# PKU-EPIC/HOTrack

Hardware: AMD Instinct MI355X
Metric: HandTrackNet point-cloud frames/sec (N=1024) (higher is better)
Workload: dtype f32; 1 GPU; HandTrackNet forward, batch=64 synthetic 1024-pt clouds per GPU (BASELINE configs[1]); per_gpu_batch=64, global_batch=64, npoints=1024, parallelism=dp1 (independent batches, no collective), world_size=1, resident_batches_rotated=5, dead_attention_elided=True, fused_sa_kernels=True, launch=hipGraph replay, batches_in_flight=4, hip_hw_queues=4, sa_compute_units=256, weights=deterministic random init (no checkpoint available offline)

## Files before the change

hotrack_amd/csrc/ball_query.hip:

```cpp
#include "pn2_common.h"
#include "fps_tie.h"

namespace pn2 {

constexpr int kBqThreads = 256;
constexpr int kBqWaves = kBqThreads / kWave;
constexpr int kBqTile = 4096;

template <int CPW, bool JOINT>
__device__ __forceinline__ void ball_query_body(const int bx, const int by, int n, int m, float radius2, int nsample,
                                                const float *__restrict__ new_xyz_all, const float *__restrict__ xyz_all,
                                                int *__restrict__ idx_all, const int *__restrict__ picks_all,
                                                float *__restrict__ new_xyz_out_all, float *__restrict__ new_xyz_copy, int copy_ld) {
    extern __shared__ __attribute__((aligned(16))) float smem[];
    const int tile_cap = n < kBqTile ? n : kBqTile;
    float *sx = smem, *sy = smem + tile_cap, *sz = smem + 2 * tile_cap;

    const int b = by;
    const float *__restrict__ xyz = xyz_all + (size_t)b * n * 3;
    const float *__restrict__ new_xyz = picks_all ? nullptr : new_xyz_all + (size_t)b * m * 3;
    const int *__restrict__ picks = picks_all ? picks_all + (size_t)b * m : nullptr;
    int *__restrict__ idx = idx_all + (size_t)b * m * nsample;

    const int tid = threadIdx.x;
    const int lane = tid & 63;
    const int w = tid >> 6;
    const int c_base = bx * (kBqWaves * CPW);

    float cx[CPW], cy[CPW], cz[CPW];
    int cnt[CPW], first[CPW];
#pragma unroll
    for (int c = 0; c < CPW; ++c) {
        const int s = c_base + c * kBqWaves + w;
        const bool ok = s < m;
        const float *__restrict__ src = !ok ? nullptr : (picks ? xyz + 3 * (size_t)picks[s] : new_xyz + 3 * (size_t)s);
        cx[c] = ok ? src[0] : 0.f;
        cy[c] = ok ? src[1] : 0.f;
        cz[c] = ok ? src[2] : 0.f;
        if (ok && picks && lane == 0) {
            float *o = new_xyz_out_all + ((size_t)b * m + s) * 3;
            o[0] = cx[c]; o[1] = cy[c]; o[2] = cz[c];
            if (new_xyz_copy) {
                float *o2 = new_xyz_copy + ((size_t)b * m + s) * copy_ld;
                o2[0] = cx[c]; o2[1] = cy[c]; o2[2] = cz[c];
            }
        }
        cnt[c] = ok ? 0 : nsample;
        first[c] = 0;
    }

    for (int t0 = 0; t0 < n; t0 += kBqTile) {
        const int tn = (n - t0) < kBqTile ? (n - t0) : kBqTile;
        if (t0 > 0) __syncthreads();
        for (int i = tid; i < 3 * tn; i += kBqThreads) {
            const float v = xyz[(size_t)3 * t0 + i];
            const int p = i / 3, comp = i - 3 * p;
            (comp == 0 ? sx : comp == 1 ? sy : sz)[p] = v;
        }
        __syncthreads();
        if constexpr (JOINT) {
            int open = 0;
#pragma unroll
            for (int c = 0; c < CPW; ++c) open += cnt[c] < nsample ? 1 : 0;
            for (int base = 0; base < tn && open > 0; base += kWave) {
                const int p = base + lane;
                const bool in = p < tn;
                const float x = in ? sx[p] : 0.f, y = in ? sy[p] : 0.f, z = in ? sz[p] : 0.f;
                float d2[CPW];
                if constexpr (CPW >= 2) {
#pragma unroll
                    for (int c = 0; c < CPW; c += 2) {
                        const pn2_f32x2 d = sqdist2((pn2_f32x2){cx[c], cx[c + 1]}, (pn2_f32x2){cy[c], cy[c + 1]}, (pn2_f32x2){cz[c], cz[c + 1]}, x, y, z);
                        d2[c] = d.x;
                        d2[c + 1] = d.y;
                    }
                } else {
                    d2[0] = sqdist(cx[0], cy[0], cz[0], x, y, z);
                }
#pragma unroll
                for (int c = 0; c < CPW; ++c) {
                    if (cnt[c] >= nsample) continue;
                    const bool hit = in && (d2[c] < radius2);
                    const uint64_t mask = __ballot(hit);
                    if (mask) {
                        int *__restrict__ row = idx + (size_t)(c_base + c * kBqWaves + w) * nsample;
                        if (cnt[c] == 0) first[c] = t0 + base + __builtin_ctzll(mask);
                        const int pos = cnt[c] + prefix_popc(mask);
                        if (hit && pos < nsample) row[pos] = t0 + p;
                        cnt[c] += __builtin_popcountll(mask);
                        if (cnt[c] >= nsample) --open;
                    }
                }
            }
        } else {
#pragma unroll
            for (int c = 0; c < CPW; ++c) {
                const int s = c_base + c * kBqWaves + w;
                int *__restrict__ row = idx + (size_t)s * nsample;
                int mycnt = cnt[c];
                if (mycnt >= nsample) continue;
                for (int base = 0; base < tn; base += kWave) {
                    const int p = base + lane;
                    const bool in = p < tn;
                    const float x = in ? sx[p] : 0.f, y = in ? sy[p] : 0.f, z = in ? sz[p] : 0.f;
                    const float d2 = sqdist(cx[c], cy[c], cz[c], x, y, z);
                    const bool hit = in && (d2 < radius2);
                    const uint64_t mask = __ballot(hit);
                    if (mask) {
                        if (mycnt == 0) first[c] = t0 + base + __builtin_ctzll(mask);
                        const int pos = mycnt + prefix_popc(mask);
                        if (hit && pos < nsample) row[pos] = t0 + p;
                        mycnt += __builtin_popcountll(mask);
                        if (mycnt >= nsample) break;
                    }
                }
                cnt[c] = mycnt;
            }
        }
    }
#pragma unroll
    for (int c = 0; c < CPW; ++c) {
        const int s = c_base + c * kBqWaves + w;
        if (s >= m) continue;
        int *__restrict__ row = idx + (size_t)s * nsample;
        const int fill = cnt[c] > 0 ? first[c] : 0;
        for (int p = cnt[c] + lane; p < nsample; p += kWave) row[p] = fill;
    }
}

template <int CPW, bool JOINT>
__global__ void __launch_bounds__(kBqThreads)
ball_query_kernel(int n, int m, float radius2, int nsample, const float *__restrict__ new_xyz_all,
                  const float *__restrict__ xyz_all, int *__restrict__ idx_all, const int *__restrict__ picks_all,
                  float *__restrict__ new_xyz_out_all, float *__restrict__ new_xyz_copy, int copy_ld) {
    ball_query_body<CPW, JOINT>((int)blockIdx.x, (int)blockIdx.y, n, m, radius2, nsample, new_xyz_all, xyz_all, idx_all, picks_all,
                                new_xyz_out_all, new_xyz_copy, copy_ld);
}

template <int CPW>
__global__ void __launch_bounds__(kBqThreads)
ball_tie_kernel(int nbx_ball, int nb_ball, int nbx_tie, int n, int m, float radius2, int nsample, const float *__restrict__ xyz_all,
                int *__restrict__ idx_all, const int *__restrict__ picks_all, float *__restrict__ new_xyz_out_all,
                float *__restrict__ new_xyz_copy, int copy_ld, int m2, const float *__restrict__ radii_all, int *__restrict__ flags) {
    const int L = (int)blockIdx.x;
    if (L < nb_ball) {
        const int by = L / nbx_ball;
        ball_query_body<CPW, false>(L - by * nbx_ball, by, n, m, radius2, nsample, xyz_all, xyz_all, idx_all, picks_all, new_xyz_out_all,
                                    new_xyz_copy, copy_ld);
    } else {
        const int T = L - nb_ball, by = T / nbx_tie;
        fps_tie_body(T - by * nbx_tie, by, nbx_tie, n, m2, m, xyz_all, picks_all, radii_all, flags);
    }
}

int ball_query_dispatch(int b, int n, int m, float radius, int nsample, const float *new_xyz,
                        const float *xyz, int *idx, hipStream_t st, const int *picks, float *new_xyz_out, float *new_xyz_copy,
                        int copy_ld) {
    if (b == 0 || m == 0) return PN2_OK;
    const float radius2 = radius * radius;
    const int tile_cap = n < kBqTile ? n : kBqTile;
    const size_t lds = (size_t)3 * tile_cap * sizeof(float);
    const long total = (long)b * m;
    int cpw = 1;
    if (total >= 4L * kBqWaves * 4096) cpw = 4;
    else if (total >= 2L * kBqWaves * 2048) cpw = 2;
    const int per_block = kBqWaves * cpw;
    dim3 grid((m + per_block - 1) / per_block, b);
    const bool joint = cpw >= 2 && n >= 4096;
    if (cpw == 4 && joint)
        hipLaunchKernelGGL((ball_query_kernel<4, true>), grid, dim3(kBqThreads), lds, st, n, m, radius2, nsample, new_xyz, xyz, idx, picks, new_xyz_out, new_xyz_copy, copy_ld);
    else if (cpw == 4)
        hipLaunchKernelGGL((ball_query_kernel<4, false>), grid, dim3(kBqThreads), lds, st, n, m, radius2, nsample, new_xyz, xyz, idx, picks, new_xyz_out, new_xyz_copy, copy_ld);
    else if (cpw == 2 && joint)
        hipLaunchKernelGGL((ball_query_kernel<2, true>), grid, dim3(kBqThreads), lds, st, n, m, radius2, nsample, new_xyz, xyz, idx, picks, new_xyz_out, new_xyz_copy, copy_ld);
    else if (cpw == 2)
        hipLaunchKernelGGL((ball_query_kernel<2, false>), grid, dim3(kBqThreads), lds, st, n, m, radius2, nsample, new_xyz, xyz, idx, picks, new_xyz_out, new_xyz_copy, copy_ld);
    else
        hipLaunchKernelGGL((ball_query_kernel<1, false>), grid, dim3(kBqThreads), lds, st, n, m, radius2, nsample, new_xyz, xyz, idx, picks, new_xyz_out, new_xyz_copy, copy_ld);
    return check_launch();
}

constexpr long kBallTieMaxN = (64 * 1024 - 22 * 1024) / 12 / 64 * 64;
bool ball_tie_supported(long b, long n, long m, long m2) {
    return b >= 1 && m >= 1 && n <= kBallTieMaxN && b * n <= 16384 && b * m < 2L * kBqWaves * 2048 && m2 >= 1 && m2 <= m &&
           m2 <= kTieMaxM;
}

int ball_tie_dispatch(int b, int n, int m, float radius, int nsample, const float *xyz, int *idx, const int *picks, float *new_xyz_out,
                      float *new_xyz_copy, int copy_ld, int m2, const float *radii, int *flags, hipStream_t st) {
    if (!ball_tie_supported(b, n, m, m2)) return PN2_ERANGE;
    const float radius2 = radius * radius;
    const int tile_cap = n < kBqTile ? n : kBqTile;
    const size_t lds = (size_t)3 * tile_cap * sizeof(float);
    const int per_block = kBqWaves;
    const int nbx_ball = (m + per_block - 1) / per_block, nbx_tie = (n + kTiePts - 1) / kTiePts;
    const long grid = (long)b * nbx_ball + (long)b * nbx_tie;
    hipLaunchKernelGGL(ball_tie_kernel<1>, dim3((unsigned)grid), dim3(kBqThreads), lds, st, nbx_ball, b * nbx_ball, nbx_tie, n, m, radius2, nsample,
                       xyz, idx, picks, new_xyz_out, new_xyz_copy, copy_ld, m2, radii, flags);
    return check_launch();
}

}
```

hotrack_amd/csrc/capi.hip:

```cpp
#include <stdlib.h>

#include "pn2_common.h"
#include "../../include/pn2_ext.h"

namespace pn2 {
static thread_local int g_last_hip_error = 0;
void set_last_hip_error(int e) { g_last_hip_error = e; }

int fps_dispatch(int b, int n, int m, const float *xyz, float *temp, int *idx, hipStream_t st, int force_threads,
                 const int *skip_flags, int nflags, float *radii);
int fps_tie_check(int b, int n, int m, int m1, const float *xyz, const int *idx, const float *radii, int *flags, hipStream_t st);
bool fps_knn_supported(int n, int nq, int k);
bool ball_tie_supported(long b, long n, long m, long m2);
int ball_tie_dispatch(int b, int n, int m, float radius, int nsample, const float *xyz, int *idx, const int *picks, float *new_xyz_out,
                      float *new_xyz_copy, int copy_ld, int m2, const float *radii, int *flags, hipStream_t st);
bool three_nn_interp_supported(long b, long n, long m, long c, long ldp, long ldo);
int three_nn_interp_dispatch(int b, int n, int m, int c, const float *unknown, const float *known, const float *points, int ldp,
                             float *out, int ldo, hipStream_t st);
int fps_knn_dispatch(int b, int n, int m, const float *xyz, int *idx, float *radii, int nq, int k, int k2, const float *query,
                     int *kidx, int *kidx2, hipStream_t st);
int ball_query_dispatch(int b, int n, int m, float radius, int nsample, const float *new_xyz, const float *xyz,
                        int *idx, hipStream_t st, const int *picks, float *new_xyz_out, float *new_xyz_copy, int copy_ld);
int three_nn_dispatch(int b, int n, int m, const float *unknown, const float *known, float *dist2, int *idx,
                      hipStream_t st, bool weights);
int interp_pm_dispatch(int b, int c, int m, int n, const float *points, int ldp, const int *idx, const float *weight,
                       float *out, int ldo, hipStream_t st);
int knn_dispatch(int b, int n, int m, int k, const float *unknown, const float *known, float *dist2, int *idx,
                 hipStream_t st, int k2, int *idx2);
int group_fwd_dispatch(int b, int c, int n, int npoints, int nsample, const float *points, const int *idx,
                       float *out, hipStream_t st);
int group_bwd_dispatch(int b, int c, int n, int npoints, int nsample, const float *grad_out, const int *idx,
                       float *grad_points, hipStream_t st);
int interp_fwd_dispatch(int b, int c, int m, int n, const float *points, const int *idx, const float *weight,
                        float *out, hipStream_t st);
int interp_bwd_dispatch(int b, int c, int n, int m, const float *grad_out, const int *idx, const float *weight,
                        float *grad_points, hipStream_t st);
}

using namespace pn2;

#define PN2_REQ(cond, code) \
    do {                    \
        if (!(cond)) return (code); \
    } while (0)

static inline bool fits_int(long v) { return v >= 0 && v <= 2147483647L; }

extern "C" {

int pn2_abi_version(void) { return 2; }

int pn2_last_hip_error(void) { return g_last_hip_error; }

const char *pn2_strerror(int code) {
    switch (code) {
        case PN2_OK: return "ok";
        case PN2_EINVAL: return "invalid dimension or parameter";
        case PN2_ENULL: return "required pointer is NULL";
        case PN2_ERANGE: return "size outside the supported range";
        case PN2_ESCRATCH: return "this size needs the scratch buffer (temp) to be provided";
        case PN2_ELAUNCH: return "HIP kernel launch failed";
        default: return "unknown error";
    }
}

int pn2_furthest_point_sampling(int b, int n, int m, const float *xyz, float *temp, int *idx, void *stream) {
    PN2_REQ(b >= 0 && n >= 1 && m >= 0, PN2_EINVAL);
    if (b == 0 || m == 0) return PN2_OK;
    PN2_REQ(xyz && idx, PN2_ENULL);
    PN2_REQ(b <= 65535 * 32768L, PN2_ERANGE);
    PN2_REQ(fits_int((long)n * 3), PN2_ERANGE);
    int force = 0;
    if (const char *e = getenv("PN2_FPS_THREADS")) force = atoi(e);
    return fps_dispatch(b, n, m, xyz, temp, idx, (hipStream_t)stream, force, nullptr, 0, nullptr);
}

int pn2x_furthest_point_sampling_radii(int b, int n, int m, const float *xyz, int *idx, float *radii, void *stream) {
    PN2_REQ(b >= 0 && n >= 1 && m >= 0, PN2_EINVAL);
    if (b == 0 || m == 0) return PN2_OK;
    PN2_REQ(xyz && idx && radii, PN2_ENULL);
    PN2_REQ(fits_int((long)n * 3), PN2_ERANGE);
    return fps_dispatch(b, n, m, xyz, nullptr, idx, (hipStream_t)stream, 0, nullptr, 0, radii);
}

int pn2x_fps_radii_knn_supported(int n, int nq, int k) { return fps_knn_supported(n, nq, k) ? 1 : 0; }

int pn2x_fps_radii_knn(int b, int n, int m, const float *xyz, int *idx, float *radii, int nq, int k, int k2, const float *query,
                       int *knn_idx, int *knn_idx2, void *stream) {
    PN2_REQ(b >= 0 && n >= 1 && m >= 1 && nq >= 1 && k >= 1 && k2 >= 0 && k2 <= k, PN2_EINVAL);
    if (b == 0) return PN2_OK;
    PN2_REQ(xyz && idx && radii && query && knn_idx && (k2 == 0 || knn_idx2), PN2_ENULL);
    PN2_REQ(m <= n && fits_int((long)n * 3) && fits_int((long)b * nq * k), PN2_ERANGE);
    return fps_knn_dispatch(b, n, m, xyz, idx, radii, nq, k, k2, query, knn_idx, k2 ? knn_idx2 : nullptr, (hipStream_t)stream);
}

int pn2x_fps_prefix_ties(int b, int n, int m1, int m2, const float *xyz, const int *idx1, const float *radii, int *flags, void *stream) {
    PN2_REQ(b >= 0 && n >= 1 && m1 >= 1 && m2 >= 1 && m2 <= m1, PN2_EINVAL);
    if (b == 0) return PN2_OK;
    PN2_REQ(xyz && idx1 && radii && flags, PN2_ENULL);
    PN2_REQ(fits_int((long)n * 3) && b <= 65535, PN2_ERANGE);
    return fps_tie_check(b, n, m2, m1, xyz, idx1, radii, flags, (hipStream_t)stream);
}

int pn2x_fps_prefix_flags(int n) { return n < 1 ? PN2_EINVAL : (n + 63) / 64; }

int pn2x_furthest_point_sampling_prefix(int b, int n, int m, const float *xyz, const int *flags, int nflags, int *idx, void *stream) {
    PN2_REQ(b >= 0 && n >= 1 && m >= 0 && m <= n && nflags >= 1, PN2_EINVAL);
    if (b == 0 || m == 0) return PN2_OK;
    PN2_REQ(xyz && idx && flags, PN2_ENULL);
    PN2_REQ(fits_int((long)n * 3), PN2_ERANGE);
    return fps_dispatch(b, n, m, xyz, nullptr, idx, (hipStream_t)stream, 0, flags, nflags, nullptr);
}

int pn2_ball_query(int b, int n, int m, float radius, int nsample, const float *new_xyz, const float *xyz,
                   int *idx, void *stream) {
    PN2_REQ(b >= 0 && n >= 1 && m >= 0 && nsample >= 1, PN2_EINVAL);
    PN2_REQ(radius == radius, PN2_EINVAL);
    if (b == 0 || m == 0) return PN2_OK;
    PN2_REQ(new_xyz && xyz && idx, PN2_ENULL);
    PN2_REQ(b <= 65535, PN2_ERANGE);
    PN2_REQ(fits_int((long)n * 3) && fits_int((long)m * nsample), PN2_ERANGE);
    if (n >= 4096 && (long)m * n >= (1L << 22) && radius > 0.f) {
        const long words = pn2x_ball_query_grid_scratch_words(b, n);
        if (words > 0 && words < (1L << 30)) {
            StreamScratch own;
            int *scratch = own.acquire((size_t)words + 4, (hipStream_t)stream);
            if (scratch) {
                unsigned *aligned = reinterpret_cast<unsigned *>(((uintptr_t)scratch + 15) & ~(uintptr_t)15);
                const int rc = ball_query_grid_dispatch(b, n, m, radius, nsample, new_xyz, xyz, idx, aligned, (size_t)words, (hipStream_t)stream);
                if (rc != PN2_ERANGE) return rc;
            }
        }
    }
    return ball_query_dispatch(b, n, m, radius, nsample, new_xyz, xyz, idx, (hipStream_t)stream, nullptr, nullptr, nullptr, 0);
}

int pn2x_ball_query_picks(int b, int n, int m, float radius, int nsample, const float *xyz, const int *picks, float *new_xyz,
                           int *idx, float *new_xyz_copy, int copy_ld, void *stream) {
    PN2_REQ(!new_xyz_copy || copy_ld >= 3, PN2_EINVAL);
    PN2_REQ(b >= 0 && n >= 1 && m >= 0 && nsample >= 1, PN2_EINVAL);
    PN2_REQ(radius == radius, PN2_EINVAL);
    if (b == 0 || m == 0) return PN2_OK;
    PN2_REQ(xyz && picks && new_xyz && idx, PN2_ENULL);
    PN2_REQ(b <= 65535, PN2_ERANGE);
    PN2_REQ(fits_int((long)n * 3) && fits_int((long)m * nsample), PN2_ERANGE);
    return ball_query_dispatch(b, n, m, radius, nsample, nullptr, xyz, idx, (hipStream_t)stream, picks, new_xyz, new_xyz_copy, copy_ld);
}

int pn2x_ball_query_picks_ties_supported(int b, int n, int m, int m2) { return ball_tie_supported(b, n, m, m2) ? 1 : 0; }

int pn2x_ball_query_picks_ties(int b, int n, int m, float radius, int nsample, const float *xyz, const int *picks, float *new_xyz,
                               int *idx, float *new_xyz_copy, int copy_ld, int m2, const float *radii, int *flags, void *stream) {
    PN2_REQ(!new_xyz_copy || copy_ld >= 3, PN2_EINVAL);
    PN2_REQ(b >= 0 && n >= 1 && m >= 1 && nsample >= 1 && m2 >= 1 && m2 <= m, PN2_EINVAL);
    PN2_REQ(radius == radius, PN2_EINVAL);
    if (b == 0) return PN2_OK;
    PN2_REQ(xyz && picks && new_xyz && idx && radii && flags, PN2_ENULL);
    PN2_REQ(b <= 65535 && fits_int((long)n * 3) && fits_int((long)m * nsample), PN2_ERANGE);
    return ball_tie_dispatch(b, n, m, radius, nsample, xyz, idx, picks, new_xyz, new_xyz_copy, copy_ld, m2, radii, flags, (hipStream_t)stream);
}

int pn2_group_points(int b, int c, int n, int npoints, int nsample, const float *points, const int *idx,
                     float *out, void *stream) {
    PN2_REQ(b >= 0 && c >= 0 && n >= 1 && npoints >= 0 && nsample >= 0, PN2_EINVAL);
    if (b == 0 || c == 0 || npoints == 0 || nsample == 0) return PN2_OK;
    PN2_REQ(points && idx && out, PN2_ENULL);
    PN2_REQ(b <= 65535 && fits_int((long)npoints * nsample), PN2_ERANGE);
    return group_fwd_dispatch(b, c, n, npoints, nsample, points, idx, out, (hipStream_t)stream);
}

int pn2_group_points_grad(int b, int c, int n, int npoints, int nsample, const float *grad_out, const int *idx,
                          float *grad_points, void *stream) {
    PN2_REQ(b >= 0 && c >= 0 && n >= 1 && npoints >= 0 && nsample >= 0, PN2_EINVAL);
    if (b == 0 || c == 0 || npoints == 0 || nsample == 0) return PN2_OK;
    PN2_REQ(grad_out && idx && grad_points, PN2_ENULL);
    PN2_REQ(b <= 65535 && c <= 65535 * 16 && fits_int((long)npoints * nsample), PN2_ERANGE);
    return group_bwd_dispatch(b, c, n, npoints, nsample, grad_out, idx, grad_points, (hipStream_t)stream);
}

int pn2_gather_points(int b, int c, int n, int npoints, const float *points, const int *idx, float *out,
                      void *stream) {
    return pn2_group_points(b, c, n, npoints, 1, points, idx, out, stream);
}

int pn2_gather_points_grad(int b, int c, int n, int npoints, const float *grad_out, const int *idx,
                           float *grad_points, void *stream) {
    return pn2_group_points_grad(b, c, n, npoints, 1, grad_out, idx, grad_points, stream);
}

int pn2_knn(int b, int n, int m, int k, const float *unknown, const float *known, float *dist2, int *idx,
            void *stream) {
    PN2_REQ(b >= 0 && n >= 0 && m >= 0, PN2_EINVAL);
    PN2_REQ(k >= 1, PN2_EINVAL);
    PN2_REQ(k <= PN2_KNN_MAX_K, PN2_ERANGE);
    if (b == 0 || n == 0) return PN2_OK;
    PN2_REQ(unknown && dist2 && idx && (known || m == 0), PN2_ENULL);
    PN2_REQ(b <= 65535 && fits_int((long)n * k) && fits_int((long)m * 3), PN2_ERANGE);
    return knn_dispatch(b, n, m, k, unknown, known, dist2, idx, (hipStream_t)stream, 0, nullptr);
}

int pn2x_knn_indices(int b, int n, int m, int k, int k2, const float *unknown, const float *known, int *idx, int *idx2, void *stream) {
    PN2_REQ(b >= 0 && n >= 0 && m >= 1 && k >= 1 && k2 >= 0 && k2 <= k, PN2_EINVAL);
    PN2_REQ(k <= PN2_KNN_MAX_K, PN2_ERANGE);
    if (b == 0 || n == 0) return PN2_OK;
    PN2_REQ(unknown && known && idx && (idx2 || k2 == 0), PN2_ENULL);
    PN2_REQ(b <= 65535 && fits_int((long)n * k) && fits_int((long)m * 3), PN2_ERANGE);
    return knn_dispatch(b, n, m, k, unknown, known, nullptr, idx, (hipStream_t)stream, k2, k2 > 0 ? idx2 : nullptr);
}

int pn2_three_nn(int b, int n, int m, const float *unknown, const float *known, float *dist2, int *idx,
                 void *stream) {
    PN2_REQ(b >= 0 && n >= 0 && m >= 0, PN2_EINVAL);
    if (b == 0 || n == 0) return PN2_OK;
    PN2_REQ(unknown && dist2 && idx && (known || m == 0), PN2_ENULL);
    PN2_REQ(b <= 65535 && fits_int((long)n * 3) && fits_int((long)m * 3), PN2_ERANGE);
    return three_nn_dispatch(b, n, m, unknown, known, dist2, idx, (hipStream_t)stream, false);
}

int pn2_three_interpolate(int b, int c, int m, int n, const float *points, const int *idx, const float *weight,
                          float *out, void *stream) {
    PN2_REQ(b >= 0 && c >= 0 && m >= 1 && n >= 0, PN2_EINVAL);
    if (b == 0 || c == 0 || n == 0) return PN2_OK;
    PN2_REQ(points && idx && weight && out, PN2_ENULL);
    PN2_REQ(b <= 65535 && fits_int((long)n * 3), PN2_ERANGE);
    return interp_fwd_dispatch(b, c, m, n, points, idx, weight, out, (hipStream_t)stream);
}

int pn2_three_interpolate_grad(int b, int c, int n, int m, const float *grad_out, const int *idx,
                               const float *weight, float *grad_points, void *stream) {
    PN2_REQ(b >= 0 && c >= 0 && m >= 1 && n >= 0, PN2_EINVAL);
    if (b == 0 || c == 0 || n == 0) return PN2_OK;
    PN2_REQ(grad_out && idx && weight && grad_points, PN2_ENULL);
    PN2_REQ(b <= 65535 && c <= 65535 * 16 && fits_int((long)n * 3), PN2_ERANGE);
    return interp_bwd_dispatch(b, c, n, m, grad_out, idx, weight, grad_points, (hipStream_t)stream);
}

int pn2x_three_nn_weights(int b, int n, int m, const float *unknown, const float *known, float *weight, int *idx,
                          void *stream) {
    PN2_REQ(b >= 0 && n >= 0 && m >= 3, PN2_EINVAL);
    if (b == 0 || n == 0) return PN2_OK;
    PN2_REQ(unknown && known && weight && idx, PN2_ENULL);
    PN2_REQ(b <= 65535 && fits_int((long)n * 3) && fits_int((long)m * 3), PN2_ERANGE);
    return three_nn_dispatch(b, n, m, unknown, known, weight, idx, (hipStream_t)stream, true);
}

int pn2x_three_nn_interpolate_pm_supported(int b, int n, int m, int c, int ldp, int ldo) {
    return three_nn_interp_supported(b, n, m, c, ldp, ldo) ? 1 : 0;
}

int pn2x_three_nn_interpolate_pm(int b, int n, int m, int c, const float *unknown, const float *known, const float *points, int ldp,
                                 float *out, int ldo, void *stream) {
    PN2_REQ(b >= 0 && n >= 0 && m >= 3 && c >= 1 && ldp >= c && ldo >= c, PN2_EINVAL);
    if (b == 0 || n == 0) return PN2_OK;
    PN2_REQ(unknown && known && points && out, PN2_ENULL);
    PN2_REQ(b <= 65535 && fits_int((long)n * 3) && fits_int((long)m * 3), PN2_ERANGE);
    return three_nn_interp_dispatch(b, n, m, c, unknown, known, points, ldp, out, ldo, (hipStream_t)stream);
}

int pn2x_three_interpolate_pm(int b, int c, int m, int n, const float *points, int ldp, const int *idx,
                              const float *weight, float *out, int ldo, void *stream) {
    PN2_REQ(b >= 0 && c >= 0 && m >= 1 && n >= 0 && ldp >= c && ldo >= c, PN2_EINVAL);
    if (b == 0 || c == 0 || n == 0) return PN2_OK;
    PN2_REQ(points && idx && weight && out, PN2_ENULL);
    PN2_REQ(fits_int((long)n * 3), PN2_ERANGE);
    return interp_pm_dispatch(b, c, m, n, points, ldp, idx, weight, out, ldo, (hipStream_t)stream);
}

}
```

hotrack_amd/csrc/sa_fused.hip:

```cpp
#include <stdlib.h>

#include "pn2_common.h"
#include "../../include/pn2_ext.h"

#ifndef SA_PAD
#define SA_PAD 4
#endif

#ifndef SA_DEFER_EPILOGUE
#define SA_DEFER_EPILOGUE 0
#endif
#ifndef SA_OVERLAP_WRITEOUT
#define SA_OVERLAP_WRITEOUT 1
#endif
#ifndef SA_SCALAR_L1
#define SA_SCALAR_L1 0
#endif
#ifndef SA_LOADER_PRIO
#define SA_LOADER_PRIO 0
#endif
#ifndef SA_PROBE
#define SA_PROBE 0
#endif
#ifndef SA_PREFETCH
#define SA_PREFETCH 1
#endif
#if SA_PREFETCH
#define SA_SCHED_FENCE() __builtin_amdgcn_sched_barrier(0)
#else
#define SA_SCHED_FENCE() ((void)0)
#endif

namespace pn2 {

typedef float f32x4 __attribute__((ext_vector_type(4)));
typedef float f32x3 __attribute__((ext_vector_type(3)));
__device__ __forceinline__ f32x3 load_xyz(const float *p) {
    f32x3 v;
    __builtin_memcpy(&v, p, 12);
    return v;
}

typedef __amdgpu_buffer_rsrc_t rsrc_t;
__device__ __forceinline__ rsrc_t make_rsrc(const void *base, unsigned bytes) {
    return __builtin_amdgcn_make_buffer_rsrc(const_cast<void *>(base), 0, (int)bytes, 0x00020000);
}
__device__ __forceinline__ unsigned mad24(int a, unsigned b_uniform, unsigned c) {
    unsigned r;
    asm("v_mad_u32_u24 %0, %1, %2, %3" : "=v"(r) : "v"(a), "s"(b_uniform), "v"(c));
    return r;
}
__device__ __forceinline__ unsigned mul24(int a, unsigned b_uniform) {
    unsigned r;
    asm("v_mul_u32_u24 %0, %1, %2" : "=v"(r) : "s"(b_uniform), "v"(a));
    return r;
}
typedef int i32x4 __attribute__((ext_vector_type(4)));
typedef int i32x2 __attribute__((ext_vector_type(2)));
__device__ __forceinline__ float4 ld_b128(rsrc_t r, unsigned voff, int soff) {
    const f32x4 v = __builtin_bit_cast(f32x4, __builtin_amdgcn_raw_buffer_load_b128(r, (int)voff, soff, 0));
    return make_float4(v.x, v.y, v.z, v.w);
}
typedef float f32x2 __attribute__((ext_vector_type(2)));
__device__ __forceinline__ f32x2 pk_fma_lo(f32x2 w, f32x2 d, f32x2 acc) {
    f32x2 r;
    asm("v_pk_fma_f32 %0, %1, %2, %3 op_sel_hi:[1,0,1]" : "=v"(r) : "v"(w), "v"(d), "v"(acc));
    return r;
}
__device__ __forceinline__ f32x2 pk_fma_hi(f32x2 w, f32x2 d, f32x2 acc) {
    f32x2 r;
    asm("v_pk_fma_f32 %0, %1, %2, %3 op_sel:[0,1,0]" : "=v"(r) : "v"(w), "v"(d), "v"(acc));
    return r;
}

struct SaArgs {
    int B, N, S, K, lgK;
    const float *a1f;
    const float *xyz;
    const float *cxyz;
    const float *wx;
    const float *b1;
    const float *cadd;
    int a1f_ld, cadd_ld;
    const int *idx;
    const float *w2, *b2, *w3, *b3;
    const float *w2e;
    float *out;
    long out_b;
    int out_s, out_c;
    int num_tiles, tiles_per_cloud;
    long long *trace;
};

template <int C1, int C2, int C3, int WC, int RTC, int MINW, int NB1, int K, int MODE>
__device__ __forceinline__ void sa_body(const SaArgs &A, const int wg, const int nwg) {
    static_assert(K == 16 || K == 32 || K == 64, "K");
    constexpr bool ROWS = MODE == 4 || MODE == 5, ROWS_EXTRA = MODE == 5;
    static_assert(!ROWS_EXTRA || SA_PAD >= 4, "the extra input columns live in the LDS row padding");
    constexpr bool has_a1f = MODE >= 1, has_xyz = !ROWS, has_cadd = MODE == 2 || MODE == 3;
    const bool p_a1f = MODE == 3 ? A.a1f != nullptr : has_a1f, p_xyz = MODE == 3 ? A.xyz != nullptr : has_xyz;
    const bool p_cadd = MODE == 3 ? A.cadd != nullptr : has_cadd;
    constexpr int lgK = K == 16 ? 4 : K == 32 ? 5 : 6;
    const int N = A.N, S = A.S;
    const float *__restrict__ W2 = A.w2, *__restrict__ b2 = A.b2, *__restrict__ W3 = A.w3, *__restrict__ b3 = A.b3;
    float *__restrict__ out = A.out;
    const int num_tiles = A.num_tiles, tiles_per_cloud = A.tiles_per_cloud;
    constexpr int WP = 4 / WC;
    constexpr int TM = WP * 64;
    constexpr int LD1 = C1 + SA_PAD, LD2 = C2 + SA_PAD;
    constexpr int NT2 = C2 / (16 * WC), NT3 = C3 / (16 * WC);
    static_assert(C2 % (16 * WC) == 0 && C3 % (16 * WC) == 0 && C1 % 16 == 0, "tile geometry");
    extern __shared__ __attribute__((aligned(16))) float smem[];
    float *H1ring = smem;
    float *H2 = smem + NB1 * TM * LD1;

    const int tid = (int)__builtin_amdgcn_workitem_id_x();
    const int lane = tid & 63;
    const int w = tid >> 6;
    const bool compute = w < 4;
    const int wc = (w & 3) % WC, wp = (w & 3) / WC;
    const int li = lane & 15, g = lane >> 4;
    const int SK = S * K;

    constexpr int Q1 = C1 / 4;
    static_assert(256 % Q1 == 0, "a loader thread keeps its channel quad across rows");
    const int lt = tid & 255;
    const int c4 = lt % Q1;
    float wxr[4][3] = {{0.f}};
    float4 b1r = make_float4(0.f, 0.f, 0.f, 0.f);
    if (!compute) {
        if (p_xyz) {
#pragma unroll
            for (int i = 0; i < 4; ++i)
#pragma unroll
                for (int k = 0; k < 3; ++k) wxr[i][k] = A.wx[(4 * c4 + i) * 3 + k];
        }
        if (A.b1) b1r = *reinterpret_cast<const float4 *>(A.b1 + 4 * c4);
    }

    constexpr int RPT = (TM / 2) / (256 / Q1);
    static_assert((TM / 2) % (256 / Q1) == 0, "half tile rows split evenly over the loader threads");
    static_assert(RPT == 1 || RPT == 2 || RPT == 4, "a thread's neighbour indices are ONE 4/8/16-byte load");
    const int row0 = (lt / Q1) * RPT;
    const int cur_db = nwg / tiles_per_cloud, cur_dt = nwg - cur_db * tiles_per_cloud;
    struct Cursor { int tile, b, t; };
    auto cursor_at = [&](int tile) { Cursor c; c.tile = tile; c.b = tile / tiles_per_cloud; c.t = tile - c.b * tiles_per_cloud; return c; };
    auto cursor_next = [&](Cursor c) {
        c.tile += nwg; c.b += cur_db; c.t += cur_dt;
        if (c.t >= tiles_per_cloud) { c.t -= tiles_per_cloud; ++c.b; }
        return c;
    };
    const unsigned c4x16 = 16u * c4, row0x4 = 4u * row0;
    const unsigned a1f_ldb = 4u * (unsigned)A.a1f_ld, cadd_ldb = 4u * (unsigned)A.cadd_ld;
    const unsigned idx_cloud = 4u * (unsigned)SK, a1f_cloud = (unsigned)N * a1f_ldb, xyz_cloud = 12u * (unsigned)N;
    const unsigned cxyz_cloud = 12u * (unsigned)S, cadd_cloud = (unsigned)S * cadd_ldb;
    const rsrc_t ra_all = make_rsrc(A.a1f, p_a1f ? (unsigned)A.B * a1f_cloud : 0u);
    const rsrc_t rx_all = make_rsrc(A.xyz, p_xyz ? (unsigned)A.B * xyz_cloud : 0u);
    struct HalfIdx { int jj[RPT], ss; };
    struct HalfRows { float4 a[RPT], pj[RPT], c, cs, e; };
    auto load_idx = [&](const Cursor &cu, int h, HalfIdx &I) {
        const int b = cu.b < A.B ? cu.b : A.B - 1;
        const int pos0 = cu.t * TM + h * (TM / 2);
        if constexpr (ROWS) {
#pragma unroll
            for (int r = 0; r < RPT; ++r) I.jj[r] = pos0 + row0 + r;
            I.ss = 0;
            return;
        }
        const rsrc_t ri = make_rsrc(reinterpret_cast<const char *>(A.idx) + (size_t)b * idx_cloud, idx_cloud);
        if constexpr (RPT == 4) {
            const i32x4 v = __builtin_bit_cast(i32x4, __builtin_amdgcn_raw_buffer_load_b128(ri, (int)row0x4, 4 * pos0, 0));
            I.jj[0] = v.x; I.jj[1] = v.y; I.jj[2] = v.z; I.jj[3] = v.w;
        } else if constexpr (RPT == 2) {
            const i32x2 v = __builtin_bit_cast(i32x2, __builtin_amdgcn_raw_buffer_load_b64(ri, (int)row0x4, 4 * pos0, 0));
            I.jj[0] = v.x; I.jj[1] = v.y;
        } else {
            I.jj[0] = (int)__builtin_amdgcn_raw_buffer_load_b32(ri, (int)row0x4, 4 * pos0, 0);
        }
        I.ss = (pos0 + row0) >> lgK;
    };
    auto load_rows = [&](const Cursor &cu, const HalfIdx &I, HalfRows &D) {
        const int b = cu.b < A.B ? cu.b : A.B - 1;
        if (has_a1f) {
            const int so = ROWS ? 0 : (int)((unsigned)b * a1f_cloud);
#pragma unroll
            for (int r = 0; r < RPT; ++r) D.a[r] = ld_b128(ra_all, mad24(I.jj[r], a1f_ldb, c4x16), so);
            if (ROWS_EXTRA && lt < TM / 2) D.e = ld_b128(ra_all, mad24(I.jj[0] - row0 + lt, a1f_ldb, 4u * C1), so);
        }
        if (has_cadd) {
            const rsrc_t rd = make_rsrc(reinterpret_cast<const char *>(A.cadd) + (size_t)b * cadd_cloud, p_cadd ? cadd_cloud : 0u);
            D.c = ld_b128(rd, mad24(I.ss, cadd_ldb, c4x16), 0);
        }
        if (has_xyz) {
            const int so = (int)((unsigned)b * xyz_cloud);
            const rsrc_t rc = make_rsrc(reinterpret_cast<const char *>(A.cxyz) + (size_t)b * cxyz_cloud, p_xyz ? cxyz_cloud : 0u);
#pragma unroll
            for (int r = 0; r < RPT; ++r) D.pj[r] = ld_b128(rx_all, mul24(I.jj[r], 12u), so);
            D.cs = ld_b128(rc, mul24(I.ss, 12u), 0);
        }
    };
    auto finish = [&](const HalfRows &D, float *__restrict__ H1, int h) {
#ifdef SA_FINISH_PRIO
        __builtin_amdgcn_s_setprio(SA_FINISH_PRIO);
#endif
        if constexpr (ROWS) {
#pragma unroll
            for (int r = 0; r < RPT; ++r) *reinterpret_cast<float4 *>(H1 + (h * (TM / 2) + row0 + r) * LD1 + 4 * c4) = D.a[r];
            if (ROWS_EXTRA && lt < TM / 2) *reinterpret_cast<float4 *>(H1 + (h * (TM / 2) + lt) * LD1 + C1) = D.e;
            return;
        }
        const f32x2 w0x = {wxr[0][0], wxr[1][0]}, w0y = {wxr[0][1], wxr[1][1]}, w0z = {wxr[0][2], wxr[1][2]};
        const f32x2 w1x = {wxr[2][0], wxr[3][0]}, w1y = {wxr[2][1], wxr[3][1]}, w1z = {wxr[2][2], wxr[3][2]};
#if SA_SCALAR_L1
        float t[4] = {b1r.x, b1r.y, b1r.z, b1r.w};
        if (has_cadd) { t[0] += D.c.x; t[1] += D.c.y; t[2] += D.c.z; t[3] += D.c.w; }
#pragma unroll
        for (int r = 0; r < RPT; ++r) {
            float v[4] = {t[0], t[1], t[2], t[3]};
            if (has_a1f) { v[0] += D.a[r].x; v[1] += D.a[r].y; v[2] += D.a[r].z; v[3] += D.a[r].w; }
            if (has_xyz) {
                const float dx = D.pj[r].x - D.cs.x, dy = D.pj[r].y - D.cs.y, dz = D.pj[r].z - D.cs.z;
#pragma unroll
                for (int i = 0; i < 4; ++i)
                    v[i] = __builtin_fmaf(wxr[i][0], dx, __builtin_fmaf(wxr[i][1], dy, __builtin_fmaf(wxr[i][2], dz, v[i])));
            }
            *reinterpret_cast<float4 *>(H1 + (h * (TM / 2) + row0 + r) * LD1 + 4 * c4) =
                make_float4(fmax_raw(v[0], 0.f), fmax_raw(v[1], 0.f), fmax_raw(v[2], 0.f), fmax_raw(v[3], 0.f));
        }
#else
        f32x2 t0 = {b1r.x, b1r.y}, t1 = {b1r.z, b1r.w};
        if (has_cadd) { t0 += (f32x2){D.c.x, D.c.y}; t1 += (f32x2){D.c.z, D.c.w}; }
        const f32x2 cxy = {D.cs.x, D.cs.y}, czw = {D.cs.z, D.cs.w};
#pragma unroll
        for (int r = 0; r < RPT; ++r) {
            f32x2 v0 = t0, v1 = t1;
            if (has_a1f) { v0 += (f32x2){D.a[r].x, D.a[r].y}; v1 += (f32x2){D.a[r].z, D.a[r].w}; }
            if (has_xyz) {
                const f32x2 dxy = (f32x2){D.pj[r].x, D.pj[r].y} - cxy, dzw = (f32x2){D.pj[r].z, D.pj[r].w} - czw;
                v0 = pk_fma_lo(w0x, dxy, pk_fma_hi(w0y, dxy, pk_fma_lo(w0z, dzw, v0)));
                v1 = pk_fma_lo(w1x, dxy, pk_fma_hi(w1y, dxy, pk_fma_lo(w1z, dzw, v1)));
            }
            *reinterpret_cast<float4 *>(H1 + (h * (TM / 2) + row0 + r) * LD1 + 4 * c4) =
                make_float4(fmax_raw(v0.x, 0.f), fmax_raw(v0.y, 0.f), fmax_raw(v1.x, 0.f), fmax_raw(v1.y, 0.f));
        }
#endif
#ifdef SA_FINISH_PRIO
        __builtin_amdgcn_s_setprio(SA_LOADER_PRIO);
#endif
    };
    auto gather = [&](const Cursor &cu, float *__restrict__ H1, int h) {
        HalfIdx I;
        HalfRows D;
        load_idx(cu, h, I);
        load_rows(cu, I, D);
        finish(D, H1, h);
    };

    float w2r[NT2][C1 / 4], w3r[NT3][C2 / 4];
    f32x4 bias2v[NT2];
    float bias3[NT3];
    f32x4 bias3v[ROWS ? NT3 : 1];
    float w2e[NT2][4][3] = {{{0.f}}};
    if (compute) {
        if constexpr (ROWS_EXTRA) {
#pragma unroll
            for (int ct = 0; ct < NT2; ++ct)
#pragma unroll
                for (int r = 0; r < 4; ++r)
#pragma unroll
                    for (int k = 0; k < 3; ++k) w2e[ct][r][k] = A.w2e[((wc * NT2 + ct) * 16 + 4 * g + r) * 3 + k];
        }
#pragma unroll
        for (int ct = 0; ct < NT2; ++ct) {
            const int oc = (wc * NT2 + ct) * 16 + li;
            {
                const float *bp = b2 + (wc * NT2 + ct) * 16 + 4 * g;
                bias2v[ct] = (f32x4){bp[0], bp[1], bp[2], bp[3]};
            }
#pragma unroll
            for (int tq = 0; tq < C1 / 16; ++tq) {
                const float4 v = *reinterpret_cast<const float4 *>(W2 + (size_t)oc * C1 + 16 * tq + 4 * g);
                w2r[ct][4 * tq + 0] = v.x; w2r[ct][4 * tq + 1] = v.y; w2r[ct][4 * tq + 2] = v.z; w2r[ct][4 * tq + 3] = v.w;
            }
        }
#pragma unroll
        for (int ct = 0; ct < NT3; ++ct) {
            const int oc = (wc * NT3 + ct) * 16 + li;
            bias3[ct] = b3[oc];
            if constexpr (ROWS) {
                const float *bp = b3 + (wc * NT3 + ct) * 16 + 4 * g;
                bias3v[ct] = (f32x4){bp[0], bp[1], bp[2], bp[3]};
            }
#pragma unroll
            for (int tq = 0; tq < C2 / 16; ++tq) {
                const float4 v = *reinterpret_cast<const float4 *>(W3 + (size_t)oc * C2 + 16 * tq + 4 * g);
                w3r[ct][4 * tq + 0] = v.x; w3r[ct][4 * tq + 1] = v.y; w3r[ct][4 * tq + 2] = v.z; w3r[ct][4 * tq + 3] = v.w;
            }
        }
    } else {
        Cursor cu = cursor_at(wg);
        for (int a = 0; a < NB1 - 1; ++a, cu = cursor_next(cu)) {
            if (cu.tile < num_tiles) {
                gather(cu, H1ring + a * TM * LD1, 0);
                gather(cu, H1ring + a * TM * LD1, 1);
            }
        }
    }
    __syncthreads();

    auto stamp = [&](int it, int slot) {
#if defined(SA_TRACE) && SA_TRACE
        if (A.trace && wg == 0 && lane == 0 && (w == 0 || w == 4) && it < 8)
            A.trace[((w >> 2) * 8 + it) * 8 + slot] = (long long)__builtin_readcyclecounter();
#else
        (void)it; (void)slot;
#endif
    };
    if (!compute) {
        __builtin_amdgcn_s_setprio(SA_LOADER_PRIO);
        HalfIdx I0, I1;
        HalfRows D0, D1;
        Cursor nx = cursor_at(wg + (NB1 - 1) * nwg);
        Cursor af = cursor_next(nx);
        load_idx(nx, 0, I0);
        load_idx(nx, 1, I1);
        load_rows(nx, I0, D0);
        int it = 0;
        for (int tile = wg; tile < num_tiles; tile += nwg, ++it) {
            stamp(it, 0);
            float *H1n = H1ring + ((it + NB1 - 1) % NB1) * TM * LD1;
#if !(SA_PROBE & 1)
            load_rows(nx, I1, D1);
#endif
            stamp(it, 7);
#if !(SA_PROBE & 4)
            load_idx(af, 0, I0);
#endif
            stamp(it, 1);
#if !(SA_PROBE & 2)
            if (nx.tile < num_tiles) finish(D0, H1n, 0);
#endif
            stamp(it, 2);
            __syncthreads();
            stamp(it, 3);
#if !(SA_PROBE & 1)
            load_rows(af, I0, D0);
#endif
#if !(SA_PROBE & 4)
            load_idx(af, 1, I1);
#endif
            stamp(it, 4);
#if !(SA_PROBE & 2)
            if (nx.tile < num_tiles) finish(D1, H1n, 1);
#endif
            stamp(it, 5);
            __syncthreads();
            stamp(it, 6);
            nx = af;
            af = cursor_next(af);
        }
        return;
    }
#ifdef SA_COMPUTE_PRIO
    __builtin_amdgcn_s_setprio(SA_COMPUTE_PRIO);
#endif
    int it = 0;
    Cursor cc = cursor_at(wg);
    constexpr int NP = 4 / RTC, NQ2 = C1 / 16, NQ3 = C2 / 16;
    constexpr int rstep = K >> 4;
    const int oc_lane = (wc * NT3 + g) * 16 + li;
    const unsigned out_cloud = 4u * ((unsigned)(S - 1) * (unsigned)A.out_s + (unsigned)(C3 - 1) * (unsigned)A.out_c + 1u);
    const rsrc_t ro_rows = make_rsrc(out, ROWS ? 4u * (unsigned)N * (unsigned)A.out_s : 0u);
    float m[4][NT3];
#pragma unroll
    for (int rt = 0; rt < 4; ++rt)
#pragma unroll
        for (int ct = 0; ct < NT3; ++ct) m[rt][ct] = 0.f;
    int e_b = 0, e_pos0 = 0;
    bool e_pending = false;
    auto epilogue = [&]() {
        if constexpr (K == 32) {
#pragma unroll
            for (int ct = 0; ct < NT3; ++ct) {
                m[0][ct] = fmax_raw(m[0][ct], m[1][ct]);
                m[2][ct] = fmax_raw(m[2][ct], m[3][ct]);
            }
        }
        if constexpr (K == 64) {
#pragma unroll
            for (int ct = 0; ct < NT3; ++ct) m[0][ct] = fmax_raw(fmax3_raw(m[0][ct], m[1][ct], m[2][ct]), m[3][ct]);
        }
        const rsrc_t ro = make_rsrc(out + (size_t)e_b * A.out_b, e_pending ? out_cloud : 0u);
#pragma unroll
        for (int rt = 0; rt < 4; rt += rstep) {
            const int s = ((e_pos0 + wp * 64) >> lgK) + rt / rstep;
#pragma unroll
            for (int ct0 = 0; ct0 < NT3; ct0 += 4) {
                float v = rows_max4(m[rt][ct0]);
#pragma unroll
                for (int j = 1; j < 4; ++j)
                    if (ct0 + j < NT3) {
                        const float vj = rows_max4(m[rt][ct0 + j]);
                        v = g == j ? vj : v;
                    }
                const unsigned off = 4u * ((unsigned)s * (unsigned)A.out_s + (unsigned)(oc_lane + 16 * ct0) * (unsigned)A.out_c);
                const bool ok = ct0 + g < NT3 && s < S;
                __builtin_amdgcn_raw_buffer_store_b32(__builtin_bit_cast(unsigned, fmaxf(v, 0.f)), ro, (int)(ok ? off : 0xffffffffu), 0, 0);
            }
        }
    };
    auto frag2 = [&](const float *H1, int p, int tq, int rt) {
        return *reinterpret_cast<const float4 *>(H1 + (wp * 64 + (p * RTC + rt) * 16 + li) * LD1 + 4 * g + 16 * tq);
    };
    constexpr bool PREFETCH_NEXT = WP == 1 && RTC * 16 <= TM / 2;
    float4 an2[RTC];
#pragma unroll
    for (int rt = 0; rt < RTC; ++rt) an2[rt] = frag2(H1ring, 0, 0, rt);
    for (int tile = wg; tile < num_tiles; tile += nwg, ++it, cc = cursor_next(cc)) {
        stamp(it, 0);
        const float *H1 = H1ring + (it % NB1) * TM * LD1;
        const float *H1next = H1ring + ((it + 1) % NB1) * TM * LD1;
        {
            f32x4 acc[2][RTC][NT2];
            auto writeout2 = [&](int p) {
#pragma unroll
                for (int rt = 0; rt < RTC; ++rt) {
                    float4 e = make_float4(0.f, 0.f, 0.f, 0.f);
                    if constexpr (ROWS_EXTRA) e = *reinterpret_cast<const float4 *>(H1 + (wp * 64 + (p * RTC + rt) * 16 + li) * LD1 + C1);
#pragma unroll
                    for (int ct = 0; ct < NT2; ++ct) {
                        float *dst = H2 + (wp * 64 + (p * RTC + rt) * 16 + li) * LD2 + (wc * NT2 + ct) * 16 + 4 * g;
                        f32x4 v = acc[p & 1][rt][ct];
                        if constexpr (ROWS_EXTRA) {
#pragma unroll
                            for (int r = 0; r < 4; ++r)
                                v[r] = __builtin_fmaf(w2e[ct][r][0], e.x, __builtin_fmaf(w2e[ct][r][1], e.y, __builtin_fmaf(w2e[ct][r][2], e.z, v[r])));
                        }
                        *reinterpret_cast<float4 *>(dst) = make_float4(fmaxf(v.x, 0.f), fmaxf(v.y, 0.f), fmaxf(v.z, 0.f), fmaxf(v.w, 0.f));
                    }
                }
            };
            float4 an[RTC];
#pragma unroll
            for (int rt = 0; rt < RTC; ++rt) an[rt] = PREFETCH_NEXT ? an2[rt] : frag2(H1, 0, 0, rt);
#pragma unroll
            for (int p = 0; p < NP; ++p) {
#pragma unroll
                for (int rt = 0; rt < RTC; ++rt)
#pragma unroll
                    for (int ct = 0; ct < NT2; ++ct) acc[p & 1][rt][ct] = bias2v[ct];
#pragma unroll
                for (int tq = 0; tq < NQ2; ++tq) {
                    float4 a[RTC];
#pragma unroll
                    for (int rt = 0; rt < RTC; ++rt) a[rt] = an[rt];
                    if (tq + 1 < NQ2 || p + 1 < NP) {
#pragma unroll
                        for (int rt = 0; rt < RTC; ++rt) an[rt] = tq + 1 < NQ2 ? frag2(H1, p, tq + 1, rt) : frag2(H1, p + 1, 0, rt);
                        SA_SCHED_FENCE();
                    }
#pragma unroll
                    for (int j = 0; j < 4; ++j)
#pragma unroll
                        for (int rt = 0; rt < RTC; ++rt) {
                            const float av = j == 0 ? a[rt].x : j == 1 ? a[rt].y : j == 2 ? a[rt].z : a[rt].w;
#pragma unroll
                            for (int ct = 0; ct < NT2; ++ct)
                                acc[p & 1][rt][ct] = __builtin_amdgcn_mfma_f32_16x16x4f32(w2r[ct][4 * tq + j], av, acc[p & 1][rt][ct], 0, 0, 0);
                        }
#if SA_DEFER_EPILOGUE
                    if (!ROWS && tq == 0 && p == 0) epilogue();
#endif
#if SA_OVERLAP_WRITEOUT
                    if (tq == 0 && p > 0) writeout2(p - 1);
#endif
                }
#if !SA_OVERLAP_WRITEOUT
                writeout2(p);
#endif
            }
            stamp(it, 1);
#if SA_OVERLAP_WRITEOUT
            writeout2(NP - 1);
#endif
        }
        stamp(it, 2);
        __syncthreads();
        stamp(it, 3);
        {
            auto frag3 = [&](int p, int tq, int rt) {
                return *reinterpret_cast<const float4 *>(H2 + (wp * 64 + (p * RTC + rt) * 16 + li) * LD2 + 4 * g + 16 * tq);
            };
            float4 an[RTC];
#pragma unroll
            for (int rt = 0; rt < RTC; ++rt) an[rt] = frag3(0, 0, rt);
#pragma unroll
            for (int p = 0; p < NP; ++p) {
                f32x4 acc[RTC][NT3];
#pragma unroll
                for (int rt = 0; rt < RTC; ++rt)
#pragma unroll
                    for (int ct = 0; ct < NT3; ++ct) acc[rt][ct] = ROWS ? bias3v[ct] : (f32x4){bias3[ct], bias3[ct], bias3[ct], bias3[ct]};
#pragma unroll
                for (int tq = 0; tq < NQ3; ++tq) {
                    float4 a[RTC];
#pragma unroll
                    for (int rt = 0; rt < RTC; ++rt) a[rt] = an[rt];
                    if (tq + 1 < NQ3 || p + 1 < NP) {
#pragma unroll
                        for (int rt = 0; rt < RTC; ++rt) an[rt] = tq + 1 < NQ3 ? frag3(p, tq + 1, rt) : frag3(p + 1, 0, rt);
                    } else if (PREFETCH_NEXT) {
#pragma unroll
                        for (int rt = 0; rt < RTC; ++rt) an2[rt] = frag2(H1next, 0, 0, rt);
                    }
                    SA_SCHED_FENCE();
#pragma unroll
                    for (int j = 0; j < 4; ++j)
#pragma unroll
                        for (int rt = 0; rt < RTC; ++rt) {
                            const float av = j == 0 ? a[rt].x : j == 1 ? a[rt].y : j == 2 ? a[rt].z : a[rt].w;
#pragma unroll
                            for (int ct = 0; ct < NT3; ++ct) {
                                if constexpr (ROWS) acc[rt][ct] = __builtin_amdgcn_mfma_f32_16x16x4f32(w3r[ct][4 * tq + j], av, acc[rt][ct], 0, 0, 0);
                                else acc[rt][ct] = __builtin_amdgcn_mfma_f32_16x16x4f32(av, w3r[ct][4 * tq + j], acc[rt][ct], 0, 0, 0);
                            }
                        }
                }
                if constexpr (ROWS) {
#pragma unroll
                    for (int rt = 0; rt < RTC; ++rt)
#pragma unroll
                        for (int ct = 0; ct < NT3; ++ct) {
                            const int row = cc.t * TM + wp * 64 + (p * RTC + rt) * 16 + li;
                            const unsigned off = 4u * ((unsigned)row * (unsigned)A.out_s + (unsigned)((wc * NT3 + ct) * 16 + 4 * g));
                            f32x4 v = acc[rt][ct];
                            v.x = fmaxf(v.x, 0.f); v.y = fmaxf(v.y, 0.f); v.z = fmaxf(v.z, 0.f); v.w = fmaxf(v.w, 0.f);
                            typedef unsigned u32x4 __attribute__((ext_vector_type(4)));
                            __builtin_amdgcn_raw_buffer_store_b128(__builtin_bit_cast(u32x4, v), ro_rows, (int)off, 0, 0);
                        }
                } else {
#pragma unroll
                    for (int rt = 0; rt < RTC; ++rt)
#pragma unroll
                        for (int ct = 0; ct < NT3; ++ct)
                            m[p * RTC + rt][ct] = fmax_raw(fmax3_raw(acc[rt][ct][0], acc[rt][ct][1], acc[rt][ct][2]), acc[rt][ct][3]);
                }
            }
            stamp(it, 4);
            if constexpr (!ROWS) {
                e_b = cc.b;
                e_pos0 = cc.t * TM;
                e_pending = true;
#if !SA_DEFER_EPILOGUE
                epilogue();
#endif
            }
        }
        stamp(it, 5);
        __syncthreads();
        stamp(it, 6);
    }
#if SA_DEFER_EPILOGUE
    if (!ROWS) epilogue();
#endif
}

template <int C1, int C2, int C3, int WC, int RTC, int MINW, int NB1, int K, int MODE>
__global__ void __launch_bounds__(512, MINW)
sa_mlp_max_kernel(const SaArgs A, const int grid) {
    sa_body<C1, C2, C3, WC, RTC, MINW, NB1, K, MODE>(A, (int)__builtin_amdgcn_workgroup_id_x(), grid);
}

template <int C1, int C2, int C3, int WC, int RTC, int MINW, int NB1, int K0, int K1, int MODE>
__global__ void __launch_bounds__(512, MINW)
sa_mlp_max_pair_kernel(const SaArgs A0, const SaArgs A1, const int n0, const int n1) {
    const int wg = (int)__builtin_amdgcn_workgroup_id_x();
    if (wg < n0)
        sa_body<C1, C2, C3, WC, RTC, MINW, NB1, K0, MODE>(A0, wg, n0);
    else
        sa_body<C1, C2, C3, WC, RTC, MINW, NB1, K1, MODE>(A1, wg - n0, n1);
}

static int g_sa_cus = -1;
static int sa_compute_units() {
    if (g_sa_cus < 0) {
        const char *e = getenv("PN2_SA_CUS");
        g_sa_cus = e ? atoi(e) : 0;
    }
    const int all = num_compute_units();
    return (g_sa_cus > 0 && g_sa_cus < all) ? g_sa_cus : all;
}

template <int C1, int C2, int C3, int WC, int RTC, int MINW, int NB1, int K, int MODE>
static int launch_sa_km(int b, SaArgs a, hipStream_t st) {
    constexpr int WP = 4 / WC, TM = WP * 64;
    const int sk = a.S * a.K;
    a.tiles_per_cloud = (sk + TM - 1) / TM;
    const long num_tiles_l = (long)b * a.tiles_per_cloud;
    if (num_tiles_l > 2147483647L) return PN2_ERANGE;
    a.num_tiles = (int)num_tiles_l;
    a.B = b;
    a.lgK = 0;
    while ((1 << a.lgK) < a.K) ++a.lgK;
    const size_t lds = (size_t)TM * (NB1 * (C1 + SA_PAD) + C2 + SA_PAD) * sizeof(float);
    auto kfn = sa_mlp_max_kernel<C1, C2, C3, WC, RTC, MINW, NB1, K, MODE>;
    static PerDeviceOnce raised;
    if (lds > 64 * 1024 && raised.first_use())
        (void)hipFuncSetAttribute((const void *)kfn, hipFuncAttributeMaxDynamicSharedMemorySize, (int)lds);
    const int wg_per_cu = (int)((160 * 1024) / lds) < MINW / 2 ? (int)((160 * 1024) / lds) : MINW / 2;
    const int max_wg = sa_compute_units() * (wg_per_cu < 1 ? 1 : wg_per_cu);
    const int rounds = (a.num_tiles + max_wg - 1) / max_wg;
    const int grid = (a.num_tiles + rounds - 1) / rounds;
    hipLaunchKernelGGL(kfn, dim3(grid), dim3(512), lds, st, a, grid);
    return check_launch();
}

template <int C1, int C2, int C3, int WC, int RTC, int MINW, int NB1>
static void sa_tiles(int b, SaArgs &a) {
    constexpr int WP = 4 / WC, TM = WP * 64;
    a.tiles_per_cloud = (a.S * a.K + TM - 1) / TM;
    a.num_tiles = b * a.tiles_per_cloud;
    a.B = b;
    a.lgK = 0;
    while ((1 << a.lgK) < a.K) ++a.lgK;
}

template <int C1, int C2, int C3, int WC, int RTC, int MINW, int NB1, int K0, int K1, int MODE>
static int launch_sa_pair(int b, SaArgs a0, SaArgs a1, hipStream_t st) {
    constexpr int WP = 4 / WC, TM = WP * 64;
    if ((long)b * ((a0.S * a0.K + TM - 1) / TM) + (long)b * ((a1.S * a1.K + TM - 1) / TM) > 2147483647L) return PN2_ERANGE;
    sa_tiles<C1, C2, C3, WC, RTC, MINW, NB1>(b, a0);
    sa_tiles<C1, C2, C3, WC, RTC, MINW, NB1>(b, a1);
    const size_t lds = (size_t)TM * (NB1 * (C1 + SA_PAD) + C2 + SA_PAD) * sizeof(float);
    auto kfn = sa_mlp_max_pair_kernel<C1, C2, C3, WC, RTC, MINW, NB1, K0, K1, MODE>;
    static PerDeviceOnce raised;
    if (lds > 64 * 1024 && raised.first_use())
        (void)hipFuncSetAttribute((const void *)kfn, hipFuncAttributeMaxDynamicSharedMemorySize, (int)lds);
    const int wg_per_cu = (int)((160 * 1024) / lds) < MINW / 2 ? (int)((160 * 1024) / lds) : MINW / 2;
    const int max_wg = sa_compute_units() * (wg_per_cu < 1 ? 1 : wg_per_cu);
    const int total = a0.num_tiles + a1.num_tiles;
    int rounds = (total + max_wg - 1) / max_wg;
    int n0, n1;
    for (;; ++rounds) {
        n0 = (a0.num_tiles + rounds - 1) / rounds;
        n1 = (a1.num_tiles + rounds - 1) / rounds;
        if (n0 + n1 <= max_wg || rounds > total) break;
    }
    hipLaunchKernelGGL(kfn, dim3(n0 + n1), dim3(512), lds, st, a0, a1, n0, n1);
    return check_launch();
}

template <int C1, int C2, int C3, int WC, int RTC, int MINW, int NB1, int K>
static int launch_sa_k(int b, const SaArgs &a, hipStream_t st) {
    const bool fa = a.a1f != nullptr, fx = a.xyz != nullptr, fc = a.cadd != nullptr;
    if (!fa && fx && !fc) return launch_sa_km<C1, C2, C3, WC, RTC, MINW, NB1, K, 0>(b, a, st);
    if (fa && fx && !fc) return launch_sa_km<C1, C2, C3, WC, RTC, MINW, NB1, K, 1>(b, a, st);
    if (fa && fx && fc) return launch_sa_km<C1, C2, C3, WC, RTC, MINW, NB1, K, 2>(b, a, st);
    return launch_sa_km<C1, C2, C3, WC, RTC, MINW, NB1, K, 3>(b, a, st);
}

template <int C1, int C2, int C3, int WC, int RTC, int MINW, int NB1>
static int launch_sa(int b, const SaArgs &a, hipStream_t st) {
    switch (a.K) {
        case 16: return launch_sa_k<C1, C2, C3, WC, RTC, MINW, NB1, 16>(b, a, st);
        case 32: return launch_sa_k<C1, C2, C3, WC, RTC, MINW, NB1, 32>(b, a, st);
        case 64: return launch_sa_k<C1, C2, C3, WC, RTC, MINW, NB1, 64>(b, a, st);
    }
    return PN2_ERANGE;
}

#ifndef SA_RTC128
#define SA_RTC128 2
#endif
#ifndef SA_NB1
#define SA_NB1 2
#endif
static long long *g_sa_trace = nullptr;
static bool sa_ranges_ok(long b, long n, long s, long k, long a1f_ld, long cadd_ld, long c3, long out_s, long out_c) {
    const long lim = 0xffffffffL;
    if (out_s < 0 || out_c < 0 || 4 * ((s - 1) * out_s + (c3 - 1) * out_c + 1) >= lim) return false;
    return n < (1L << 24) && s < (1L << 24) && 4 * a1f_ld < (1L << 24) && 4 * cadd_ld < (1L << 24) &&
           4 * b * n * (a1f_ld > 3 ? a1f_ld : 3) <= lim && 4 * s * (cadd_ld > 3 ? cadd_ld : 3) <= lim && 4 * s * k <= lim;
}
}

extern "C" int pn2x_sa_set_compute_units(int n) {
    if (n < 0) return PN2_EINVAL;
    pn2::g_sa_cus = n;
    return PN2_OK;
}

extern "C" void pn2x_debug_set_sa_trace(void *device_buffer_2x8x8_int64) { pn2::g_sa_trace = (long long *)device_buffer_2x8x8_int64; }

extern "C" int pn2x_sa_mlp_max(int b, int n, int s, int k, int c1, int c2, int c3, const float *a1f, int a1f_ld,
                               const float *xyz, const float *cxyz, const float *wx, const float *b1, const float *cadd,
                               int cadd_ld, const int *idx,
                               const float *w2, const float *b2, const float *w3, const float *b3, float *out,
                               long out_b, int out_s, int out_c, void *stream) {
    using namespace pn2;
    if (b < 0 || n < 1 || s < 0 || k < 1) return PN2_EINVAL;
    if (b == 0 || s == 0) return PN2_OK;
    if (!idx || !w2 || !b2 || !w3 || !b3 || !out) return PN2_ENULL;
    if (!a1f && !xyz) return PN2_ENULL;
    if (xyz && (!cxyz || !wx)) return PN2_ENULL;
    if ((a1f && (a1f_ld < c1 || a1f_ld % 4)) || (cadd && (cadd_ld < c1 || cadd_ld % 4))) return PN2_EINVAL;
    if (!(k == 16 || k == 32 || k == 64)) return PN2_ERANGE;
    if (!sa_ranges_ok(b, n, s, k, a1f ? a1f_ld : 0, cadd ? cadd_ld : 0, c3, out_s, out_c)) return PN2_ERANGE;
    if (((uintptr_t)a1f | (uintptr_t)cadd | (uintptr_t)b1 | (uintptr_t)w2 | (uintptr_t)w3) % 16 != 0) return PN2_EINVAL;
    SaArgs a;
    a.B = b; a.N = n; a.S = s; a.K = k; a.lgK = 0;
    a.a1f = a1f; a.a1f_ld = a1f_ld; a.cadd_ld = cadd_ld; a.xyz = xyz; a.cxyz = cxyz; a.wx = wx; a.b1 = b1; a.cadd = cadd; a.idx = idx;
    a.w2 = w2; a.b2 = b2; a.w3 = w3; a.b3 = b3; a.w2e = nullptr; a.out = out; a.out_b = out_b; a.out_s = out_s; a.out_c = out_c;
    a.num_tiles = 0; a.tiles_per_cloud = 0; a.trace = g_sa_trace;
    hipStream_t st = (hipStream_t)stream;
    if (c1 == 32 && c2 == 32 && c3 == 64) return launch_sa<32, 32, 64, 2, 4, 4, SA_NB1>(b, a, st);
    if (c1 == 64 && c2 == 64 && c3 == 128) return launch_sa<64, 64, 128, 4, 2, 4, SA_NB1>(b, a, st);
    if (c1 == 128 && c2 == 128 && c3 == 192) return launch_sa<128, 128, 192, 4, SA_RTC128, 2, SA_NB1>(b, a, st);
    return PN2_ERANGE;
}

namespace pn2 {
static int fill_sa_args(int b, const pn2x_sa_problem &p, int c1, int c3, SaArgs &a) {
    if (p.n < 1 || p.s < 1 || p.k < 1) return PN2_EINVAL;
    if (!p.idx || !p.w2 || !p.b2 || !p.w3 || !p.b3 || !p.out) return PN2_ENULL;
    if (!p.a1f && !p.xyz) return PN2_ENULL;
    if (p.xyz && (!p.cxyz || !p.wx)) return PN2_ENULL;
    if ((p.a1f && (p.a1f_ld < c1 || p.a1f_ld % 4)) || (p.cadd && (p.cadd_ld < c1 || p.cadd_ld % 4))) return PN2_EINVAL;
    if (((uintptr_t)p.a1f | (uintptr_t)p.cadd | (uintptr_t)p.b1 | (uintptr_t)p.w2 | (uintptr_t)p.w3) % 16 != 0) return PN2_EINVAL;
    if (!sa_ranges_ok(b, p.n, p.s, p.k, p.a1f ? p.a1f_ld : 0, p.cadd ? p.cadd_ld : 0, c3, p.out_s, p.out_c)) return PN2_ERANGE;
    a.B = 0; a.N = p.n; a.S = p.s; a.K = p.k; a.lgK = 0;
    a.a1f = p.a1f; a.a1f_ld = p.a1f_ld; a.cadd_ld = p.cadd_ld; a.xyz = p.xyz; a.cxyz = p.cxyz; a.wx = p.wx; a.b1 = p.b1;
    a.cadd = p.cadd; a.idx = p.idx; a.w2 = p.w2; a.b2 = p.b2; a.w3 = p.w3; a.b3 = p.b3; a.w2e = nullptr; a.out = p.out; a.out_b = p.out_b;
    a.out_s = p.out_s; a.out_c = p.out_c; a.num_tiles = 0; a.tiles_per_cloud = 0; a.trace = nullptr;
    return PN2_OK;
}
}

extern "C" int pn2x_sa_mlp_max_pair_supported(int k0, int k1, int c1, int c2, int c3) {
    return (c1 == 128 && c2 == 128 && c3 == 192 && ((k0 == 16 && k1 == 64) || (k0 == 64 && k1 == 16))) ? 1 : 0;
}

extern "C" int pn2x_sa_mlp_max_pair(int b, int c1, int c2, int c3, const pn2x_sa_problem *p0, const pn2x_sa_problem *p1, void *stream) {
    using namespace pn2;
    if (b < 0 || !p0 || !p1) return b < 0 ? PN2_EINVAL : PN2_ENULL;
    if (b == 0) return PN2_OK;
    if (!pn2x_sa_mlp_max_pair_supported(p0->k, p1->k, c1, c2, c3)) return PN2_ERANGE;
    if (p0->k > p1->k) { const pn2x_sa_problem *t = p0; p0 = p1; p1 = t; }
    SaArgs a0, a1;
    int rc = fill_sa_args(b, *p0, c1, c3, a0);
    if (rc != PN2_OK) return rc;
    rc = fill_sa_args(b, *p1, c1, c3, a1);
    if (rc != PN2_OK) return rc;
    const bool fa = a0.a1f && a1.a1f, fx = a0.xyz && a1.xyz, fc0 = a0.cadd != nullptr, fc1 = a1.cadd != nullptr;
    if (!fa || !fx || fc0 != fc1 || (a0.a1f == nullptr) != (a1.a1f == nullptr)) return PN2_ERANGE;
    hipStream_t st = (hipStream_t)stream;
    if (fc0) return launch_sa_pair<128, 128, 192, 4, SA_RTC128, 2, SA_NB1, 16, 64, 2>(b, a0, a1, st);
    return launch_sa_pair<128, 128, 192, 4, SA_RTC128, 2, SA_NB1, 16, 64, 1>(b, a0, a1, st);
}

extern "C" int pn2x_mlp2_rows_supported(int c1, int c2, int c3) { return (c1 == 128 && c2 == 128 && c3 == 128) ? 1 : 0; }

extern "C" int pn2x_mlp2_rows(long rows, int c1, int c2, int c3, const float *x, int ldx, const float *w2, const float *w2e, const float *b2,
                              const float *w3, const float *b3, float *out, int ldo, void *stream) {
    using namespace pn2;
    if (rows < 0 || ldx < c1 + (w2e ? 4 : 0) || ldo < c3 || ldx % 4 || ldo % 4) return PN2_EINVAL;
    if (rows == 0) return PN2_OK;
    if (!x || !w2 || !b2 || !w3 || !b3 || !out) return PN2_ENULL;
    if (!pn2x_mlp2_rows_supported(c1, c2, c3)) return PN2_ERANGE;
    if (((uintptr_t)x | (uintptr_t)w2 | (uintptr_t)w3 | (uintptr_t)out) % 16 != 0) return PN2_EINVAL;
    if (rows >= (1L << 24) - 64 || 4L * ldx >= (1L << 24) || 4L * rows * ldx > 0xffffffffL || 4L * rows * ldo > 0xffffffffL) return PN2_ERANGE;
    SaArgs a;
    a.B = 1; a.N = (int)rows; a.K = 16; a.S = (int)((rows + 15) / 16); a.lgK = 4;
    a.a1f = x; a.a1f_ld = ldx; a.cadd_ld = 0; a.xyz = nullptr; a.cxyz = nullptr; a.wx = nullptr; a.b1 = nullptr; a.cadd = nullptr; a.idx = nullptr;
    a.w2 = w2; a.b2 = b2; a.w3 = w3; a.b3 = b3; a.w2e = w2e; a.out = out; a.out_b = 0; a.out_s = ldo; a.out_c = 1;
    a.num_tiles = 0; a.tiles_per_cloud = 0; a.trace = nullptr;
    if (w2e) return launch_sa_km<128, 128, 128, 4, 2, 2, SA_NB1, 16, 5>(1, a, (hipStream_t)stream);
    return launch_sa_km<128, 128, 128, 4, 2, 2, SA_NB1, 16, 4>(1, a, (hipStream_t)stream);
}

extern "C" int pn2x_sa_mlp_max_supported(int k, int c1, int c2, int c3) {
    const bool kk = (k == 16 || k == 32 || k == 64);
    const bool cc = (c1 == 32 && c2 == 32 && c3 == 64) || (c1 == 64 && c2 == 64 && c3 == 128) ||
                    (c1 == 128 && c2 == 128 && c3 == 192);
    return (kk && cc) ? 1 : 0;
}
```

hotrack_amd/ext.py:

```python
from __future__ import annotations

import ctypes
import os

import torch

from . import pointnet2_hip as _native

_lib = _native._lib
_vp, _ci = ctypes.c_void_p, ctypes.c_int
_lib.pn2x_kabsch.argtypes = [_ci, _ci, _ci, _vp, _vp, _vp, _vp, _vp]
_lib.pn2x_kabsch.restype = _ci


def kabsch(x: torch.Tensor, y: torch.Tensor):
    x = x.float().contiguous()
    y = y.float().contiguous()
    if x.dim() == 2:
        x = x.unsqueeze(0)
    B, num, _ = y.shape
    xb = x.shape[0]
    if xb not in (1, B) or x.shape[1] != num:
        raise ValueError(f"kabsch: x {tuple(x.shape)} does not match y {tuple(y.shape)}")
    px = _native._ptr(x, "x", torch.float32, xb * num * 3)
    py = _native._ptr(y, "y", torch.float32, B * num * 3)
    R = torch.empty((B, 3, 3), dtype=torch.float32, device=y.device)
    t = torch.empty((B, 3, 1), dtype=torch.float32, device=y.device)
    with torch.cuda.device(y.device):
        _native._check(_lib.pn2x_kabsch(B, xb, num, px, py, R.data_ptr(), t.data_ptr(), _native._stream(y)), "kabsch")
    return R, t


_lib.pn2x_kabsch_backward.argtypes = [_ci, _ci, _ci, _vp, _vp, _vp, _vp, _vp, _vp, _vp]
_lib.pn2x_kabsch_backward.restype = _ci


def kabsch_backward(x: torch.Tensor, y: torch.Tensor, R: torch.Tensor, grad_R, grad_t) -> torch.Tensor:
    x = x.float().contiguous()
    y = y.float().contiguous()
    if x.dim() == 2:
        x = x.unsqueeze(0)
    B, num, _ = y.shape
    f32 = torch.float32
    gR = None if grad_R is None else _native._ptr(grad_R.contiguous(), "grad_R", f32, B * 9)
    gt = None if grad_t is None else _native._ptr(grad_t.contiguous(), "grad_t", f32, B * 3)
    dy = torch.empty_like(y)
    with torch.cuda.device(y.device):
        _native._check(_lib.pn2x_kabsch_backward(B, x.shape[0], num, _native._ptr(x, "x", f32, x.shape[0] * num * 3),
                                                 _native._ptr(y, "y", f32, B * num * 3), _native._ptr(R.contiguous(), "R", f32, B * 9),
                                                 gR, gt, dy.data_ptr(), _native._stream(y)), "kabsch_backward")
    return dy


class KabschFit(torch.autograd.Function):

    @staticmethod
    def forward(ctx, x, y):
        R, t = kabsch(x, y)
        ctx.save_for_backward(x, y, R)
        return R, t

    @staticmethod
    def backward(ctx, grad_R, grad_t):
        x, y, R = ctx.saved_tensors
        return None, kabsch_backward(x, y, R, grad_R, grad_t)


_cl = ctypes.c_long
_lib.pn2x_sa_mlp_max.argtypes = [_ci] * 7 + [_vp, _ci, _vp, _vp, _vp, _vp, _vp, _ci, _vp, _vp, _vp, _vp, _vp, _vp, _cl, _ci, _ci, _vp]
_lib.pn2x_sa_mlp_max.restype = _ci
_lib.pn2x_sa_mlp_max_supported.argtypes = [_ci] * 4
_lib.pn2x_sa_mlp_max_supported.restype = _ci
_lib.pn2x_three_nn_weights.argtypes = [_ci, _ci, _ci, _vp, _vp, _vp, _vp, _vp]
_lib.pn2x_three_nn_weights.restype = _ci
_lib.pn2x_three_interpolate_pm.argtypes = [_ci, _ci, _ci, _ci, _vp, _ci, _vp, _vp, _vp, _ci, _vp]
_lib.pn2x_three_interpolate_pm.restype = _ci
_lib.pn2x_gather_rows.argtypes = [_ci, _ci, _ci, _ci, _vp, _vp, _vp, _vp]
_lib.pn2x_gather_rows.restype = _ci
_lib.pn2x_bias_act_pm.argtypes = [_cl, _ci, _vp, _ci, _vp, _cl, _ci, _vp]
_lib.pn2x_bias_act_pm.restype = _ci


def sa_mlp_max_supported(k: int, c1: int, c2: int, c3: int) -> bool:
    return bool(_lib.pn2x_sa_mlp_max_supported(k, c1, c2, c3))


def _rows(t: torch.Tensor, name: str, cols: int):
    if not t.is_cuda or t.dtype != torch.float32 or t.dim() != 3:
        raise TypeError(f"{name}: expected a 3-D float32 GPU tensor")
    B, R, C = t.shape
    if C < cols or t.stride(2) != 1 or (R > 1 and B > 1 and t.stride(0) != R * t.stride(1)):
        raise ValueError(f"{name}: unsupported layout shape={tuple(t.shape)} strides={t.stride()}")
    return t.data_ptr(), t.stride(1)


def sa_mlp_max(idx: torch.Tensor, w2, b2, w3, b3, *, a1f=None, xyz=None, cxyz=None, wx=None, b1=None, cadd=None,
               out=None, point_major=False) -> torch.Tensor:
    B, S, K = idx.shape
    C1, C2, C3 = w2.shape[1], w2.shape[0], w3.shape[0]
    f32 = torch.float32
    N = a1f.shape[1] if a1f is not None else xyz.shape[1]
    pa, lda = (None, 0) if a1f is None else _rows(a1f, "a1f", C1)
    pc, ldc = (None, 0) if cadd is None else _rows(cadd, "cadd", C1)
    px = None if xyz is None else _native._ptr(xyz, "xyz", f32, B * N * 3)
    pcx = None if cxyz is None else _native._ptr(cxyz, "cxyz", f32, B * S * 3)
    pwx = None if wx is None else _native._ptr(wx, "wx", f32, C1 * 3)
    pb1 = None if b1 is None else _native._ptr(b1, "b1", f32, C1)
    pi = _native._ptr(idx, "idx", torch.int32, B * S * K)
    pw2, pb2 = _native._ptr(w2, "w2", f32, C2 * C1), _native._ptr(b2, "b2", f32, C2)
    pw3, pb3 = _native._ptr(w3, "w3", f32, C3 * C2), _native._ptr(b3, "b3", f32, C3)
    if out is None:
        out = torch.empty((B, S, C3) if point_major else (B, C3, S), dtype=f32, device=idx.device)
        ob, os_, oc = (S * C3, C3, 1) if point_major else (C3 * S, 1, S)
        po = out.data_ptr()
    else:
        po, ld = _rows(out, "out", C3)
        ob, os_, oc = out.stride(0), ld, 1
    with torch.cuda.device(idx.device):
        _native._check(_native._call(_lib.pn2x_sa_mlp_max, "sa_mlp_max_kernel", None, B, N, S, K, C1, C2, C3, pa, lda, px, pcx,
                                     pwx, pb1, pc, ldc, pi, pw2, pb2, pw3, pb3, po, ob, os_, oc, _native._stream(idx)),
                       "sa_mlp_max")
    return out


class _SaProblem(ctypes.Structure):
    _fields_ = [("n", _ci), ("s", _ci), ("k", _ci), ("a1f", _vp), ("a1f_ld", _ci), ("xyz", _vp), ("cxyz", _vp), ("wx", _vp),
                ("b1", _vp), ("cadd", _vp), ("cadd_ld", _ci), ("idx", _vp), ("w2", _vp), ("b2", _vp), ("w3", _vp), ("b3", _vp),
                ("out", _vp), ("out_b", _cl), ("out_s", _ci), ("out_c", _ci)]


_lib.pn2x_sa_mlp_max_pair.argtypes = [_ci] * 4 + [ctypes.POINTER(_SaProblem)] * 2 + [_vp]
_lib.pn2x_sa_mlp_max_pair.restype = _ci
_lib.pn2x_sa_mlp_max_pair_supported.argtypes = [_ci] * 5
_lib.pn2x_sa_mlp_max_pair_supported.restype = _ci


def _sa_problem(idx, w2, b2, w3, b3, a1f, xyz, cxyz, wx, b1, cadd, out) -> _SaProblem:
    B, S, K = idx.shape
    C1, C2, C3 = w2.shape[1], w2.shape[0], w3.shape[0]
    f32 = torch.float32
    N = a1f.shape[1] if a1f is not None else xyz.shape[1]
    pa, lda = (None, 0) if a1f is None else _rows(a1f, "a1f", C1)
    pc, ldc = (None, 0) if cadd is None else _rows(cadd, "cadd", C1)
    po, ld = _rows(out, "out", C3)
    return _SaProblem(
        N, S, K, pa, lda, None if xyz is None else _native._ptr(xyz, "xyz", f32, B * N * 3),
        None if cxyz is None else _native._ptr(cxyz, "cxyz", f32, B * S * 3), None if wx is None else _native._ptr(wx, "wx", f32, C1 * 3),
        None if b1 is None else _native._ptr(b1, "b1", f32, C1), pc, ldc, _native._ptr(idx, "idx", torch.int32, B * S * K),
        _native._ptr(w2, "w2", f32, C2 * C1), _native._ptr(b2, "b2", f32, C2), _native._ptr(w3, "w3", f32, C3 * C2),
        _native._ptr(b3, "b3", f32, C3), po, out.stride(0), ld, 1)


def sa_mlp_max_pair(p0: dict, p1: dict) -> None:
    keys = ("idx", "w2", "b2", "w3", "b3", "a1f", "xyz", "cxyz", "wx", "b1", "cadd", "out")
    a = [{k: p.get(k) for k in keys} for p in (p0, p1)]
    C1, C2, C3 = a[0]["w2"].shape[1], a[0]["w2"].shape[0], a[0]["w3"].shape[0]
    same = all(tuple(a[1][k].shape) == tuple(a[0][k].shape) for k in ("w2", "w3"))
    modes = [(p["a1f"] is not None, p["xyz"] is not None, p["cadd"] is not None) for p in a]
    if not (same and modes[0] == modes[1] and modes[0][0] and modes[0][1]
            and _lib.pn2x_sa_mlp_max_pair_supported(a[0]["idx"].shape[2], a[1]["idx"].shape[2], C1, C2, C3)):
        for p in a:
            sa_mlp_max(p["idx"], p["w2"], p["b2"], p["w3"], p["b3"], a1f=p["a1f"], xyz=p["xyz"], cxyz=p["cxyz"], wx=p["wx"], b1=p["b1"],
                       cadd=p["cadd"], out=p["out"])
        return
    B = a[0]["idx"].shape[0]
    q0, q1 = (_sa_problem(**p) for p in a)
    with torch.cuda.device(a[0]["idx"].device):
        _native._check(_native._call(_lib.pn2x_sa_mlp_max_pair, "sa_mlp_max_pair_kernel", None, B, C1, C2, C3, ctypes.byref(q0),
                                     ctypes.byref(q1), _native._stream(a[0]["idx"])), "sa_mlp_max_pair")


_lib.pn2x_mlp2_rows.argtypes = [_cl] + [_ci] * 3 + [_vp, _ci, _vp, _vp, _vp, _vp, _vp, _vp, _ci, _vp]
_lib.pn2x_mlp2_rows.restype = _ci
_lib.pn2x_mlp2_rows_supported.argtypes = [_ci] * 3
_lib.pn2x_mlp2_rows_supported.restype = _ci


_lib.pn2x_sa_set_compute_units.argtypes = [_ci]
_lib.pn2x_sa_set_compute_units.restype = _ci


def sa_set_compute_units(n: int) -> None:
    _native._check(_lib.pn2x_sa_set_compute_units(int(n)), "sa_set_compute_units")


def mlp2_rows_supported(c1: int, c2: int, c3: int) -> bool:
    return bool(_lib.pn2x_mlp2_rows_supported(c1, c2, c3))


def mlp2_rows(x: torch.Tensor, w2, b2, w3, b3, out: torch.Tensor = None, w2e=None) -> torch.Tensor:
    if x.dim() != 2 or not x.is_cuda or x.dtype != torch.float32 or x.stride(1) != 1:
        raise TypeError("mlp2_rows: x must be a 2-D float32 GPU tensor with a contiguous last dimension")
    R = x.shape[0]
    C1, C2, C3 = w2.shape[1], w2.shape[0], w3.shape[0]
    f32 = torch.float32
    ldx = x.stride(0) if R > 1 else x.shape[1]
    if x.shape[1] < C1 + (3 if w2e is not None else 0) or (w2e is not None and ldx < C1 + 4):
        raise ValueError("mlp2_rows: x has too few columns")
    if out is None:
        out = torch.empty((R, C3), dtype=f32, device=x.device)
    if out.dim() != 2 or out.shape[0] != R or out.shape[1] < C3 or out.stride(1) != 1 or out.dtype != f32 or out.device != x.device:
        raise ValueError("mlp2_rows: out must be (rows, >= c3) float32 on the same device")
    if (R > 1 and out.stride(0) % 4) or out.data_ptr() % 16:
        raise ValueError("mlp2_rows: out needs a row stride that is a multiple of 4 floats and a 16-byte aligned first element")
    with torch.cuda.device(x.device):
        _native._check(_native._call(_lib.pn2x_mlp2_rows, "mlp2_rows_kernel", None, R, C1, C2, C3, x.data_ptr(), ldx,
                                     _native._ptr(w2, "w2", f32, C2 * C1), None if w2e is None else _native._ptr(w2e, "w2e", f32, C2 * 3),
                                     _native._ptr(b2, "b2", f32, C2), _native._ptr(w3, "w3", f32, C3 * C2),
                                     _native._ptr(b3, "b3", f32, C3), out.data_ptr(), out.stride(0) if R > 1 else out.shape[1], _native._stream(x)),
                       "mlp2_rows")
    return out


def three_nn_weights(unknown: torch.Tensor, known: torch.Tensor):
    B, n, _ = unknown.shape
    m = known.shape[1]
    f32 = torch.float32
    w = torch.empty((B, n, 3), dtype=f32, device=unknown.device)
    idx = torch.empty((B, n, 3), dtype=torch.int32, device=unknown.device)
    with torch.cuda.device(unknown.device):
        _native._check(_lib.pn2x_three_nn_weights(B, n, m, _native._ptr(unknown, "unknown", f32, B * n * 3),
                                                  _native._ptr(known, "known", f32, B * m * 3), w.data_ptr(), idx.data_ptr(),
                                                  _native._stream(unknown)), "three_nn_weights")
    return w, idx


def three_interpolate_pm(points: torch.Tensor, idx: torch.Tensor, weight: torch.Tensor, out: torch.Tensor) -> torch.Tensor:
    B, M, C = points.shape
    n = idx.shape[1]
    pp, ldp = _rows(points, "points", C)
    po, ldo = _rows(out, "out", C)
    with torch.cuda.device(points.device):
        _native._check(_lib.pn2x_three_interpolate_pm(B, C, M, n, pp, ldp, _native._ptr(idx, "idx", torch.int32, B * n * 3),
                                                      _native._ptr(weight, "weight", torch.float32, B * n * 3), po, ldo,
                                                      _native._stream(points)), "three_interpolate_pm")
    return out


_lib.pn2x_three_nn_interpolate_pm.argtypes = [_ci, _ci, _ci, _ci, _vp, _vp, _vp, _ci, _vp, _ci, _vp]
_lib.pn2x_three_nn_interpolate_pm.restype = _ci
_lib.pn2x_three_nn_interpolate_pm_supported.argtypes = [_ci] * 6
_lib.pn2x_three_nn_interpolate_pm_supported.restype = _ci


def three_nn_interpolate_pm(unknown: torch.Tensor, known: torch.Tensor, points: torch.Tensor, out: torch.Tensor) -> torch.Tensor:
    B, n, _ = unknown.shape
    m, C = known.shape[1], points.shape[2]
    pp, ldp = _rows(points, "points", C)
    po, ldo = _rows(out, "out", C)
    f32 = torch.float32
    if _lib.pn2x_three_nn_interpolate_pm_supported(B, n, m, C, ldp, ldo) and pp % 16 == 0 and po % 16 == 0:
        with torch.cuda.device(points.device):
            _native._check(_native._call(_lib.pn2x_three_nn_interpolate_pm, "three_nn_interp_kernel", None, B, n, m, C,
                                         _native._ptr(unknown, "unknown", f32, B * n * 3), _native._ptr(known, "known", f32, B * m * 3),
                                         pp, ldp, po, ldo, _native._stream(points)), "three_nn_interpolate_pm")
        return out
    w, i3 = three_nn_weights(unknown, known)
    return three_interpolate_pm(points, i3, w, out)


def gather_rows(src: torch.Tensor, idx: torch.Tensor) -> torch.Tensor:
    B, N, C = src.shape
    M = idx.shape[1]
    out = torch.empty((B, M, C), dtype=torch.float32, device=src.device)
    with torch.cuda.device(src.device):
        _native._check(_lib.pn2x_gather_rows(B, N, M, C, _native._ptr(src, "src", torch.float32, B * N * C),
                                             _native._ptr(idx, "idx", torch.int32, B * M), out.data_ptr(),
                                             _native._stream(src)), "gather_rows")
    return out

# ... 50 lines not shown
        palm_template = palm_template.unsqueeze(0)
    palm_template, kp, points = palm_template.float().contiguous(), kp.float().contiguous(), points.float().contiguous()
    B, N, _ = points.shape
    J = kp.shape[1]
    xb, num = palm_template.shape[0], palm_template.shape[1]
    f32 = torch.float32
    R = torch.empty((B, 3, 3), dtype=f32, device=points.device)
    t = torch.empty((B, 3, 1), dtype=f32, device=points.device)
    xyz2 = torch.empty((B, N, 3), dtype=f32, device=points.device)
    xyz1 = torch.empty((B, J, 3), dtype=f32, device=points.device)
    pc, ldc = (None, 0) if xyz2_copy is None else _xyz_cols(xyz2_copy, "xyz2_copy", B, N)
    with torch.cuda.device(points.device):
        _native._check(_lib.pn2x_hand_frame(B, xb, num, N, J, _native._ptr(palm_template, "palm_template", f32, xb * num * 3),
                                             _native._ptr(kp, "kp", f32, B * J * 3), _native._ptr(palm_idx, "palm_idx", torch.int32, num),
                                             _native._ptr(points, "points", f32, B * N * 3), float(scale), R.data_ptr(), t.data_ptr(),
                                             xyz2.data_ptr(), xyz1.data_ptr(), pc, ldc,
                                             None if nonfinite is None else _native._ptr(nonfinite, "nonfinite", torch.int32, B),
                                             _native._stream(points)), "hand_frame")
    return R, t, xyz2, xyz1


_cf = ctypes.c_float
_lib.pn2x_add_layernorm.argtypes = [_cl, _ci, _vp, _vp, _vp, _vp, _vp, _cf, _vp, _vp, _cf, _vp, _vp]
_lib.pn2x_add_layernorm.restype = _ci
_lib.pn2x_pose_head.argtypes = [_ci, _ci, _ci, _vp, _vp, _vp, _vp, _vp, _vp, _cf, _vp, _vp, _vp, _vp]
_lib.pn2x_pose_head.restype = _ci


def add_layernorm(x: torch.Tensor, ln1, y: torch.Tensor = None, bias: torch.Tensor = None, ln2=None) -> torch.Tensor:
    rows, C = x.shape
    f32 = torch.float32
    px = _native._ptr(x, "x", f32, rows * C)
    py = None if y is None else _native._ptr(y, "y", f32, rows * C)
    pb = None if bias is None else _native._ptr(bias, "bias", f32, C)
    for ln in (ln1, ln2):
        if ln is not None and (tuple(ln.normalized_shape) != (C,) or ln.weight is None or ln.bias is None):
            raise ValueError("add_layernorm: LayerNorm over the last dimension with affine parameters expected")
    g1, b1 = _native._ptr(ln1.weight, "ln1.weight", f32, C), _native._ptr(ln1.bias, "ln1.bias", f32, C)
    g2 = b2 = None
    eps2 = 0.0
    if ln2 is not None:
        g2, b2, eps2 = _native._ptr(ln2.weight, "ln2.weight", f32, C), _native._ptr(ln2.bias, "ln2.bias", f32, C), ln2.eps
    out = torch.empty_like(x)
    with torch.cuda.device(x.device):
        _native._check(_lib.pn2x_add_layernorm(rows, C, px, py, pb, g1, b1, ln1.eps, g2, b2, eps2, out.data_ptr(), _native._stream(x)),
                       "add_layernorm")
    return out


def pose_head(h: torch.Tensor, w: torch.Tensor, bias: torch.Tensor, xyz1: torch.Tensor, R: torch.Tensor, t: torch.Tensor, scale: float,
              nonfinite: torch.Tensor = None):
    B, J, _ = xyz1.shape
    C = h.shape[1]
    f32 = torch.float32
    ptrs = (_native._ptr(h, "h", f32, B * J * C), _native._ptr(w, "w", f32, 3 * C), _native._ptr(bias, "bias", f32, 3),
            _native._ptr(xyz1, "xyz1", f32, B * J * 3), _native._ptr(R, "R", f32, B * 9), _native._ptr(t, "t", f32, B * 3))
    kp_hand = torch.empty((B, J, 3), dtype=f32, device=h.device)
    kp_cam = torch.empty((B, J, 3), dtype=f32, device=h.device)
    with torch.cuda.device(h.device):
        _native._check(_lib.pn2x_pose_head(B, J, C, *ptrs, float(scale), kp_hand.data_ptr(), kp_cam.data_ptr(),
                                            None if nonfinite is None else _native._ptr(nonfinite, "nonfinite", torch.int32, B),
                                            _native._stream(h)), "pose_head")
    return kp_hand, kp_cam


_lib.pn2x_linear_small.argtypes = [_ci, _ci, _ci, _vp, _ci, _vp, _ci, _vp, _ci, _vp, _ci, _vp]
_lib.pn2x_linear_small.restype = _ci
LINEAR_SMALL_MAX_ROWS = 512
LINEAR_SMALL_MAX_K, LINEAR_SMALL_MAX_N = 384, 512


def linear(x: torch.Tensor, w: torch.Tensor, bias: torch.Tensor = None, relu: bool = False) -> torch.Tensor:
    M, K = x.shape
    N = w.shape[0]
    if (M > LINEAR_SMALL_MAX_ROWS or M < 2 or K > LINEAR_SMALL_MAX_K or N > LINEAR_SMALL_MAX_N or not x.is_cuda or x.dtype != torch.float32 or w.dtype != torch.float32 or x.stride(1) != 1
            or w.stride(1) != 1 or (bias is not None and not bias.is_contiguous()) or torch.is_grad_enabled() and (x.requires_grad or w.requires_grad)):
        if relu and bias is not None:
            return torch._addmm_activation(bias, x, w.t())
        y = torch.nn.functional.linear(x, w, bias)
        return torch.relu_(y) if relu else y
    y = torch.empty((M, N), dtype=torch.float32, device=x.device)
    with torch.cuda.device(x.device):
        _native._check(_lib.pn2x_linear_small(M, K, N, x.data_ptr(), x.stride(0), w.data_ptr(), w.stride(0),
                                              None if bias is None else bias.data_ptr(), 1 if relu else 0, y.data_ptr(), N,
                                              _native._stream(x)), "linear_small")
    return y


_lib.pn2x_ln_linear_small.argtypes = [_ci, _ci, _ci, _vp, _vp, _vp, _vp, _vp, _cf, _vp, _vp, _cf, _vp, _vp, _ci, _vp, _ci, _vp, _ci, _vp]
_lib.pn2x_ln_linear_small.restype = _ci
LN_LINEAR_MAX_ROWS = 256


def ln_linear_supported(rows: int, c: int) -> bool:
    return 0 < rows <= LN_LINEAR_MAX_ROWS and c <= 384


def ln_linear(x: torch.Tensor, ln1, w: torch.Tensor, bias: torch.Tensor = None, relu: bool = False, y: torch.Tensor = None,
              ybias: torch.Tensor = None, ln2=None):
    rows, C = x.shape
    N = w.shape[0]
    f32 = torch.float32
    for ln in (ln1, ln2):
        if ln is not None and (tuple(ln.normalized_shape) != (C,) or ln.weight is None or ln.bias is None):
            raise ValueError("ln_linear: LayerNorm over the last dimension with affine parameters expected")
    if x.dtype != f32 or not x.is_cuda or not x.is_contiguous() or w.dtype != f32 or w.stride(1) != 1 or w.shape[1] != C:
        raise TypeError("ln_linear: contiguous float32 GPU rows and a (N, C) float32 weight expected")
    if y is not None and (y.shape != x.shape or not y.is_contiguous() or y.dtype != f32):
        raise TypeError("ln_linear: y must match x")
    xn = torch.empty_like(x)
    out = torch.empty((rows, N), dtype=f32, device=x.device)
    with torch.cuda.device(x.device):
        _native._check(_lib.pn2x_ln_linear_small(
            rows, C, N, x.data_ptr(), None if y is None else y.data_ptr(), None if ybias is None else _native._ptr(ybias, "ybias", f32, C),
            _native._ptr(ln1.weight, "ln1.weight", f32, C), _native._ptr(ln1.bias, "ln1.bias", f32, C), ln1.eps,
            None if ln2 is None else _native._ptr(ln2.weight, "ln2.weight", f32, C), None if ln2 is None else _native._ptr(ln2.bias, "ln2.bias", f32, C),
            0.0 if ln2 is None else ln2.eps, xn.data_ptr(), w.data_ptr(), w.stride(0), None if bias is None else _native._ptr(bias, "bias", f32, N),
            1 if relu else 0, out.data_ptr(), N, _native._stream(x)), "ln_linear_small")
    return xn, out


_lib.pn2x_knn_indices.argtypes = [_ci, _ci, _ci, _ci, _ci, _vp, _vp, _vp, _vp, _vp]
_lib.pn2x_knn_indices.restype = _ci


def knn_indices(k: int, unknown: torch.Tensor, known: torch.Tensor, k2: int = 0):
    B, n, _ = unknown.shape
    m = known.shape[1]
    pu, pk = _native._ptr(unknown, "unknown", torch.float32, B * n * 3), _native._ptr(known, "known", torch.float32, B * m * 3)
    idx = torch.empty((B, n, k), dtype=torch.int32, device=unknown.device)
    idx2 = torch.empty((B, n, k2), dtype=torch.int32, device=unknown.device) if k2 else None
    with torch.cuda.device(unknown.device):
        _native._check(_lib.pn2x_knn_indices(B, n, m, k, k2, pu, pk, idx.data_ptr(), None if idx2 is None else idx2.data_ptr(),
                                             _native._stream(unknown)), "knn_indices")
    return (idx, idx2) if k2 else idx


_lib.pn2x_furthest_point_sampling_radii.argtypes = [_ci, _ci, _ci, _vp, _vp, _vp, _vp]
_lib.pn2x_furthest_point_sampling_radii.restype = _ci
_lib.pn2x_fps_radii_knn.argtypes = [_ci, _ci, _ci, _vp, _vp, _vp, _ci, _ci, _ci, _vp, _vp, _vp, _vp]
_lib.pn2x_fps_radii_knn.restype = _ci
_lib.pn2x_fps_radii_knn_supported.argtypes = [_ci, _ci, _ci]
_lib.pn2x_fps_radii_knn_supported.restype = _ci
_lib.pn2x_fps_prefix_ties.argtypes = [_ci, _ci, _ci, _ci, _vp, _vp, _vp, _vp, _vp]
_lib.pn2x_fps_prefix_ties.restype = _ci
_lib.pn2x_fps_prefix_flags.argtypes = [_ci]
_lib.pn2x_fps_prefix_flags.restype = _ci
_lib.pn2x_furthest_point_sampling_prefix.argtypes = [_ci, _ci, _ci, _vp, _vp, _ci, _vp, _vp]
_lib.pn2x_furthest_point_sampling_prefix.restype = _ci


_lib.pn2x_ball_query_picks.argtypes = [_ci, _ci, _ci, ctypes.c_float, _ci, _vp, _vp, _vp, _vp, _vp, _ci, _vp]
_lib.pn2x_ball_query_picks.restype = _ci


def ball_query_picks(radius: float, nsample: int, xyz: torch.Tensor, picks: torch.Tensor, xyz_copy: torch.Tensor = None):
    B, N, _ = xyz.shape
    S = picks.shape[1]
    px = _native._ptr(xyz, "xyz", torch.float32, B * N * 3)
    pp = _native._ptr(picks, "picks", torch.int32, B * S)
    idx = torch.empty((B, S, nsample), dtype=torch.int32, device=xyz.device)
    new_xyz = torch.empty((B, S, 3), dtype=torch.float32, device=xyz.device)
    pc, ldc = (None, 0) if xyz_copy is None else _xyz_cols(xyz_copy, "xyz_copy", B, S)
    with torch.cuda.device(xyz.device):
        _native._check(_lib.pn2x_ball_query_picks(B, N, S, float(radius), nsample, px, pp, new_xyz.data_ptr(), idx.data_ptr(),
                                                   pc, ldc, _native._stream(xyz)), "ball_query_picks")
    return idx, new_xyz


FPS_KNN_COLAUNCH = True
BALL_TIE_COLAUNCH = True
_lib.pn2x_ball_query_picks_ties.argtypes = [_ci, _ci, _ci, ctypes.c_float, _ci, _vp, _vp, _vp, _vp, _vp, _ci, _ci, _vp, _vp, _vp]
_lib.pn2x_ball_query_picks_ties.restype = _ci
_lib.pn2x_ball_query_picks_ties_supported.argtypes = [_ci] * 4
_lib.pn2x_ball_query_picks_ties_supported.restype = _ci


def fps_two_level(xyz: torch.Tensor, m1: int, m2: int, query=None, knn=None):
    from . import pointnet2_utils as ops
    B, N, _ = xyz.shape
    if not 1 <= m2 <= m1:
        raise ValueError("fps_two_level: need 1 <= m2 <= m1")
    xyz = xyz.contiguous()

    def knn_alone():
        r = knn_indices(knn[1], knn[0], xyz, k2=knn[2])
        return r if knn[2] else (r, None)
    if m2 > 1024 or N > 16384:
        i1 = ops.furthest_point_sample(xyz, m1)
        l1 = gather_rows(xyz, i1)
        i2 = ops.furthest_point_sample(l1, m2)
        res = (i1, l1, i2) if query is None else (i1, l1, i2, ops.ball_query(query[0], query[1], xyz, l1))
        return res if knn is None else res + (knn_alone(),)
    px = _native._ptr(xyz, "xyz", torch.float32, B * N * 3)
    nf = _lib.pn2x_fps_prefix_flags(N)
    i1 = torch.empty((B, m1), dtype=torch.int32, device=xyz.device)
    radii = torch.empty((B, m1), dtype=torch.float32, device=xyz.device)
    flags = torch.empty((B, nf), dtype=torch.int32, device=xyz.device)
    i2 = torch.empty((B, m2), dtype=torch.int32, device=xyz.device)
    with torch.cuda.device(xyz.device):
        st = _native._stream(xyz)
        lists = None
        if knn is not None and FPS_KNN_COLAUNCH and _lib.pn2x_fps_radii_knn_supported(N, knn[0].shape[1], knn[1]):
            pts, k, k2 = knn
            nq = pts.shape[1]
            gi = torch.empty((B, nq, k), dtype=torch.int32, device=xyz.device)
            gi2 = torch.empty((B, nq, k2), dtype=torch.int32, device=xyz.device) if k2 else None
            _native._check(_native._call(_lib.pn2x_fps_radii_knn, "fps_knn_kernel", None, B, N, m1, px, i1.data_ptr(), radii.data_ptr(),
                                         nq, k, k2, _native._ptr(pts, "knn points", torch.float32, B * nq * 3), gi.data_ptr(),
                                         None if gi2 is None else gi2.data_ptr(), st), "fps_two_level/1+knn")
            lists = (gi, gi2)
        else:
            _native._check(_native._call(_lib.pn2x_furthest_point_sampling_radii, "fps_kernel", None, B, N, m1, px, i1.data_ptr(),
                                         radii.data_ptr(), st), "fps_two_level/1")
        if query is not None and BALL_TIE_COLAUNCH and _lib.pn2x_ball_query_picks_ties_supported(B, N, m1, m2):
            idx1 = torch.empty((B, m1, query[1]), dtype=torch.int32, device=xyz.device)
            l1 = torch.empty((B, m1, 3), dtype=torch.float32, device=xyz.device)
            _native._check(_native._call(_lib.pn2x_ball_query_picks_ties, "ball_tie_kernel", None, B, N, m1, float(query[0]), query[1], px,
                                         i1.data_ptr(), l1.data_ptr(), idx1.data_ptr(), None, 0, m2, radii.data_ptr(), flags.data_ptr(), st),
                           "fps_two_level/query+ties")
        else:
            if query is None:
                l1 = gather_rows(xyz, i1)
            else:
                idx1, l1 = ball_query_picks(query[0], query[1], xyz, i1)
            _native._check(_lib.pn2x_fps_prefix_ties(B, N, m1, m2, px, i1.data_ptr(), radii.data_ptr(), flags.data_ptr(), st), "fps_two_level/ties")
        _native._check(_native._call(_lib.pn2x_furthest_point_sampling_prefix, "fps_prefix_kernel", None, B, m1, m2, l1.data_ptr(),
                                     flags.data_ptr(), nf, i2.data_ptr(), st), "fps_two_level/2")
    res = (i1, l1, i2) if query is None else (i1, l1, i2, idx1)
    if knn is None:
        return res
    return res + (lists if lists is not None else knn_alone(),)


_lib.pn2x_hand_losses.argtypes = [_ci, _ci, _vp, _vp, _vp, _vp, _vp, _vp, ctypes.c_float, _vp, _vp, _vp, _vp, _vp]
_lib.pn2x_hand_losses.restype = _ci
_lib.pn2x_hand_losses_backward.argtypes = [_ci, _ci, _vp, ctypes.c_float, _vp, _vp, _vp, _vp, _vp, _vp, _vp]
_lib.pn2x_hand_losses_backward.restype = _ci
HAND_LOSS_NAMES = ("hand_pred_kp_loss", "hand_pred_r_loss", "hand_pred_t_loss", "hand_pred_kp_diff", "hand_init_kp_diff",
                   "hand_init_r_diff", "hand_init_t_diff", "hand_pred_r_diff", "hand_pred_t_diff")


class HandLosses(torch.autograd.Function):

    @staticmethod
    def forward(ctx, pred_hf, init_hf, gt_kp, pred_kp, R, t, scale, palm, weights=None):
        f32 = torch.float32
        B = pred_hf.shape[0]
        ctx.set_materialize_grads(False)
        pred_hf = pred_hf.contiguous()
        palm = palm.contiguous().float()
        if palm.dim() == 2:
            palm = palm.unsqueeze(0)
        args = [x.detach().contiguous().float() for x in (init_hf, gt_kp, pred_kp, R, t)]
        out = torch.empty(10, dtype=f32, device=pred_hf.device)
        saved = torch.empty((B, 87), dtype=f32, device=pred_hf.device)
        wptr = None if weights is None else _native._ptr(weights, "weights", f32, 9)
        with torch.cuda.device(pred_hf.device):
            _native._check(_lib.pn2x_hand_losses(B, palm.shape[0], _native._ptr(pred_hf, "pred_hf", f32, B * 63), _native._ptr(args[0], "init_hf", f32, B * 63),
                                                  _native._ptr(args[1], "gt_kp", f32, B * 63), _native._ptr(args[2], "pred_kp", f32, B * 63),
                                                  _native._ptr(args[3], "R", f32, B * 9), _native._ptr(args[4], "t", f32, B * 3), float(scale),
                                                  _native._ptr(palm, "palm", f32, palm.shape[0] * 18), out.data_ptr(), saved.data_ptr(), wptr,
                                                  _native._stream(pred_hf)), "hand_losses")
        ctx.save_for_backward(pred_hf, palm, saved, *([weights] if weights is not None else []))
        ctx.scale = float(scale)
        ctx.set_materialize_grads(False)
        if weights is None:
            return out[:9]
        return out[:9], out[9]

    @staticmethod
    def backward(ctx, grad, grad_total=None):
        pred_hf, palm, saved = ctx.saved_tensors[:3]
        weights = ctx.saved_tensors[3] if len(ctx.saved_tensors) > 3 else None
        B = pred_hf.shape[0]
        if grad is None and grad_total is None:
            return (None,) * 9
        g3 = None if grad is None else grad[:3].contiguous().float()
        gt = None if grad_total is None else grad_total.contiguous().float()
        d = torch.empty_like(pred_hf)
        with torch.cuda.device(pred_hf.device):
            _native._check(_lib.pn2x_hand_losses_backward(B, palm.shape[0], pred_hf.data_ptr(), ctx.scale, palm.data_ptr(), saved.data_ptr(),
                                                           None if g3 is None else g3.data_ptr(), None if gt is None else gt.data_ptr(),
                                                           None if weights is None else weights.data_ptr(), d.data_ptr(),
                                                           _native._stream(pred_hf)), "hand_losses_backward")
        return d, None, None, None, None, None, None, None, None


_lib.pn2x_copy_multi_max.argtypes = []
_lib.pn2x_copy_multi_max.restype = _ci
_lib.pn2x_copy_multi.argtypes = [_ci, ctypes.POINTER(_vp), ctypes.POINTER(_vp), ctypes.POINTER(ctypes.c_long), _vp]
_lib.pn2x_copy_multi.restype = _ci


def copy_multi(dsts, srcs) -> None:
    n = len(dsts)
    if n == 0:
        return
    cap = int(_lib.pn2x_copy_multi_max())
    dev = dsts[0].device
    for d, s_ in zip(dsts, srcs):
        if (not d.is_cuda or d.device != dev or s_.device != dev or d.dtype != s_.dtype or d.shape != s_.shape
                or not d.is_contiguous() or not s_.is_contiguous()):
            raise ValueError("copy_multi: same-shaped contiguous tensors of one dtype on one GPU")
    with torch.cuda.device(dev):
        for i0 in range(0, n, cap):
            k = min(cap, n - i0)
            D, S, Bn = (_vp * k)(), (_vp * k)(), (ctypes.c_long * k)()
            for j in range(k):
                D[j], S[j], Bn[j] = dsts[i0 + j].data_ptr(), srcs[i0 + j].data_ptr(), dsts[i0 + j].numel() * dsts[i0 + j].element_size()
            _native._check(_lib.pn2x_copy_multi(k, D, S, Bn, _native._stream(dsts[0])), "copy_multi")


_lib.pn2x_row_lists.argtypes = [_ci] * 5 + [_vp] * 5
_lib.pn2x_row_lists.restype = _ci
_lib.pn2x_row_chain_supported.argtypes = [_ci] * 4
_lib.pn2x_row_chain_supported.restype = _ci
_lib.pn2x_row_chain.argtypes = [_ci, _ci, _vp, _ci, _vp, _vp] + [_vp] * 7 + [_vp, _ci, _ci, _vp]
_lib.pn2x_row_chain.restype = _ci
ROW_CHAIN_MAX_B = 1024


def row_lists(gi: torch.Tensor, gi_small, n: int):
    if gi.dim() != 3 or gi.dtype != torch.int32 or not gi.is_cuda:
        raise TypeError("row_lists: gi must be a (B,J,K) int32 GPU tensor")
    gi = gi.contiguous()
    B, J, KL = gi.shape
    if gi_small is not None:
        if gi_small.dim() != 3 or gi_small.shape[:2] != (B, J) or gi_small.dtype != torch.int32 or gi_small.device != gi.device:
            raise ValueError("row_lists: gi_small must be (B,J,K2) int32 on gi's device")
        gi_small = gi_small.contiguous()
    KS = gi_small.shape[2] if gi_small is not None else KL
    lst = torch.empty((B, n), dtype=torch.int32, device=gi.device)
    counts = torch.empty((B, 2), dtype=torch.int32, device=gi.device)
    with torch.cuda.device(gi.device):
        _native._check(_native._call(_lib.pn2x_row_lists, "row_lists_kernel", None, B, n, J, KL, KS, gi.data_ptr(),
                                     None if gi_small is None else gi_small.data_ptr(), lst.data_ptr(), counts.data_ptr(),
                                     _native._stream(gi)), "row_lists")
    return lst, counts


def row_chain_supported(c_in: int, c_h: int, c_conv: int, c_q: int) -> bool:
    return bool(_lib.pn2x_row_chain_supported(c_in, c_h, c_conv, c_q))


def row_chain_pack(W: torch.Tensor) -> torch.Tensor:
    n_out, k = W.shape
    kp = (k + 15) // 16 * 16
    Wp = torch.zeros((n_out, kp), dtype=torch.float32, device=W.device)
    Wp[:, :k] = W
    return Wp.view(n_out // 16, 16, kp // 16, 4, 4).permute(0, 2, 3, 1, 4).contiguous()


def row_chain(x: torch.Tensor, lst: torch.Tensor, counts: torch.Tensor, wa, ba, wb, bb, wc, bc, wq, out: torch.Tensor = None,
              grid: int = 0) -> torch.Tensor:
    if x.dim() != 3 or not x.is_cuda or x.dtype != torch.float32 or x.stride(2) != 1 or x.stride(0) != x.shape[1] * x.stride(1):
        raise TypeError("row_chain: x must be a (B,N,C) float32 GPU tensor with contiguous rows")
    B, N, _ = x.shape
    f32 = torch.float32
    if out is None:
        out = torch.empty((B, N, 512), dtype=f32, device=x.device)
    if out.shape[:2] != (B, N) or out.shape[2] < 512 or out.stride(2) != 1 or out.stride(0) != N * out.stride(1) or out.dtype != f32:
        raise ValueError("row_chain: out must be (B,N,>=512) float32 with contiguous rows")
    if lst.shape != (B, N) or counts.shape != (B, 2) or lst.dtype != torch.int32 or counts.dtype != torch.int32:
        raise ValueError("row_chain: list (B,N) / counts (B,2) int32 from row_lists")
    with torch.cuda.device(x.device):
        _native._check(_native._call(_lib.pn2x_row_chain, "row_chain_kernel", None, B, N, x.data_ptr(), x.stride(1), lst.data_ptr(),
                                     counts.data_ptr(), _native._ptr(wa, "wa", f32, 128 * 144), _native._ptr(ba, "ba", f32, 128),
                                     _native._ptr(wb, "wb", f32, 128 * 128), _native._ptr(bb, "bb", f32, 128),
                                     _native._ptr(wc, "wc", f32, 384 * 128), _native._ptr(bc, "bc", f32, 384),
                                     _native._ptr(wq, "wq", f32, 512 * 384), out.data_ptr(), out.stride(1), int(grid),
                                     _native._stream(x)), "row_chain")
    return out


_lib.pn2x_sa3_chain_supported.argtypes = [_ci] * 5
_lib.pn2x_sa3_chain_supported.restype = _ci
_lib.pn2x_sa3_chain.argtypes = [_ci, _ci, _vp, _ci] + [_vp] * 7 + [_vp]
_lib.pn2x_sa3_chain.restype = _ci
_lib.pn2x_fp3_chain_supported.argtypes = [_ci] * 5
_lib.pn2x_fp3_chain_supported.restype = _ci
_lib.pn2x_fp3_chain.argtypes = [_ci, _ci, _vp, _ci] + [_vp] * 6 + [_vp, _ci, _vp]
# ... 268 lines not shown
```

include/pn2_ext.h:

```cpp
#ifndef PN2_EXT_H
#define PN2_EXT_H

#include "pn2_hip.h"

#ifdef __cplusplus
extern "C" {
#endif

int pn2x_kabsch(int b, int xb, int num, const float *x, const float *y, float *R, float *t, void *stream);
int pn2x_kabsch_backward(int b, int xb, int num, const float *x, const float *y, const float *R, const float *grad_R,
                         const float *grad_t, float *grad_y, void *stream);

int pn2x_hand_frame(int b, int xb, int num, int n, int j, const float *palm_template, const float *kp,
                    const int *palm_idx, const float *points, float scale, float *R, float *t, float *xyz2,
                    float *xyz1, float *xyz2_copy, int copy_ld, int *nonfinite, void *stream);

int pn2x_sa_mlp_max(int b, int n, int s, int k, int c1, int c2, int c3, const float *a1f, int a1f_ld,
                    const float *xyz, const float *cxyz, const float *wx, const float *b1, const float *cadd,
                    int cadd_ld, const int *idx,
                    const float *w2, const float *b2, const float *w3, const float *b3, float *out,
                    long out_b, int out_s, int out_c, void *stream);
int pn2x_sa_mlp_max_supported(int k, int c1, int c2, int c3);

int pn2x_bias_act(int b, int c, int n, float *y, const float *bias, int relu, void *stream);

int pn2x_three_nn_weights(int b, int n, int m, const float *unknown, const float *known, float *weight, int *idx,
                          void *stream);

int pn2x_three_nn_interpolate_pm_supported(int b, int n, int m, int c, int ldp, int ldo);
int pn2x_three_nn_interpolate_pm(int b, int n, int m, int c, const float *unknown, const float *known, const float *points, int ldp,
                                 float *out, int ldo, void *stream);
int pn2x_three_interpolate_pm(int b, int c, int m, int n, const float *points, int ldp, const int *idx,
                              const float *weight, float *out, int ldo, void *stream);

int pn2x_furthest_point_sampling_radii(int b, int n, int m, const float *xyz, int *idx, float *radii, void *stream);
int pn2x_fps_radii_knn_supported(int n, int nq, int k);
int pn2x_fps_radii_knn(int b, int n, int m, const float *xyz, int *idx, float *radii, int nq, int k, int k2, const float *query,
                       int *knn_idx, int *knn_idx2, void *stream);
int pn2x_fps_prefix_ties(int b, int n, int m1, int m2, const float *xyz, const int *idx1, const float *radii, int *flags, void *stream);
int pn2x_ball_query_picks_ties_supported(int b, int n, int m, int m2);
int pn2x_ball_query_picks_ties(int b, int n, int m, float radius, int nsample, const float *xyz, const int *picks, float *new_xyz,
                               int *idx, float *new_xyz_copy, int copy_ld, int m2, const float *radii, int *flags, void *stream);
int pn2x_fps_prefix_flags(int n);
int pn2x_furthest_point_sampling_prefix(int b, int n, int m, const float *xyz, const int *flags, int nflags, int *idx, void *stream);

int pn2x_knn_indices(int b, int n, int m, int k, int k2, const float *unknown, const float *known, int *idx, int *idx2, void *stream);

int pn2x_ball_query_picks(int b, int n, int m, float radius, int nsample, const float *xyz, const int *picks, float *new_xyz,
                          int *idx, float *new_xyz_copy, int copy_ld, void *stream);

long pn2x_ball_query_grid_scratch_words(int b, int n);
int pn2x_ball_query_grid(int b, int n, int m, float radius, int nsample, const float *new_xyz, const float *xyz, int *idx,
                         void *scratch, long scratch_words, void *stream);

int pn2x_gather_rows(int b, int n, int m, int c, const float *src, const int *idx, float *out, void *stream);

int pn2x_bias_act_pm(long rows, int c, float *y, int ldy, const float *bias, long rows_per_bias, int relu, void *stream);

int pn2x_max_rows(int b, int r, int c, const float *x, float *out, void *stream);

int pn2x_copy_multi_max(void);
int pn2x_copy_multi(int n, void *const *dst, const void *const *src, const long *bytes, void *stream);

int pn2x_add_layernorm(long rows, int c, const float *x, const float *y, const float *bias, const float *g1,
                       const float *b1, float eps1, const float *g2, const float *b2, float eps2, float *out, void *stream);

int pn2x_pose_head(int b, int j, int c, const float *h, const float *w, const float *bias, const float *xyz1,
                   const float *R, const float *t, float scale, float *kp_hand, float *kp_cam, const int *nonfinite,
                   void *stream);

typedef struct pn2x_sa_problem {
    int n, s, k;
    const float *a1f;
    int a1f_ld;
    const float *xyz, *cxyz, *wx, *b1, *cadd;
    int cadd_ld;
    const int *idx;
    const float *w2, *b2, *w3, *b3;
    float *out;
    long out_b;
    int out_s, out_c;
} pn2x_sa_problem;
int pn2x_sa_set_compute_units(int n);
int pn2x_mlp2_rows_supported(int c1, int c2, int c3);
int pn2x_mlp2_rows(long rows, int c1, int c2, int c3, const float *x, int ldx, const float *w2, const float *w2e, const float *b2,
                   const float *w3, const float *b3, float *out, int ldo, void *stream);
int pn2x_sa_mlp_max_pair_supported(int k0, int k1, int c1, int c2, int c3);
int pn2x_sa_mlp_max_pair(int b, int c1, int c2, int c3, const pn2x_sa_problem *p0, const pn2x_sa_problem *p1, void *stream);

int pn2x_row_lists(int b, int n, int j, int k_large, int k_small, const int *gi, const int *gi_small, int *list, int *counts,
                   void *stream);
int pn2x_row_chain_supported(int c_in, int c_h, int c_conv, int c_q);
int pn2x_row_chain(int b, int n, const float *x, int ldx, const int *list, const int *counts, const float *wa, const float *ba,
                   const float *wb, const float *bb, const float *wc, const float *bc, const float *wq, float *out, int ldo,
                   int grid, void *stream);

int pn2x_sa3_chain_supported(int s, int c_in, int c1, int c2, int c3);
int pn2x_sa3_chain(int b, int s, const float *x, int ldx, const float *w1, const float *b1, const float *w2, const float *b2,
                   const float *w3, const float *b3, float *part, void *stream);
int pn2x_fp3_chain_supported(int s, int c_l2, int c_l3, int c1, int c2);
int pn2x_fp3_chain(int b, int s, const float *x, int ldx, const float *part, const float *wgt, const float *bg, const float *wa,
                   const float *wf, const float *bf, float *out, int ldo, void *stream);

int pn2x_hand_shape_opt_supported(int p, int d, int t);
int pn2x_hand_shape_opt(int p, int d, int t, int iterations, const float *k0, const float *k, const float *pre,
                        const float *targets, const float *initial_scale, double scaling_coefficient2, double beta, float *out,
                        float *trace, void *stream);

int pn2x_hand_pose_opt_supported(int p, int v, int j, int k, int d_pose, int res);
long pn2x_hand_pose_opt_work_floats(int p);
int pn2x_hand_pose_energy(int p, int v, int j, int k, const int *parents, const int *pose_block, const float *rest_joints,
                          const float *rest_verts, const int *skin_pack, const float *skin_w, const float *comps, float theta_scale,
                          const float *pre, const float *pred_kp, const float *last_kp, const unsigned char *vis_mask,
                          const float *obj_r, const float *obj_t, const void *vol, int vol_f16, int res, float voxel_scale,
                          const unsigned char *mask, int h, int w, float fx, float fy, float cx, float cy, float w_sil, float w_pen,
                          float w_vis, float w_invis, float w_temporal, float w_attr, const float *state, float *work, float *energy,
                          float *out_verts, float *out_kp, void *stream);
int pn2x_hand_pose_opt(int p, int v, int j, int k, const int *parents, const int *pose_block, const float *rest_joints,
                       const float *rest_verts, const int *skin_pack, const float *skin_w, const float *comps, float theta_scale,
                       const float *pre, const float *pred_kp, const float *last_kp, const unsigned char *vis_mask,
                       const float *obj_r, const float *obj_t, const void *vol, int vol_f16, int res, float voxel_scale,
                       const unsigned char *mask, int h, int w, float fx, float fy, float cx, float cy, float w_sil, float w_pen,
                       float w_vis, float w_invis, float w_temporal, float w_attr, int iterations, double scaling_coefficient2,
                       double beta, float *state, float *work, float *trace, void *stream);

int pn2x_iknet_supported(int m, int k_in, int hidden, int layers, int n_out);
long pn2x_iknet_work_floats(void);
int pn2x_iknet_forward(int m, int frame, const float *kp, const float *R, const float *t, const float *w1, const float *b1,
                       const float *wh, const float *bh, const float *wo, const float *bo, float *work, float *kp_hf,
                       float *raw_quat, float *theta, void *stream);

int pn2x_bn_sums_doubles(int c);
int pn2x_bn_stats(long rows, int c, const float *y, int ldy, double *sums, void *stream);
int pn2x_bn_relu_apply(long rows, int c, const float *y, int ldy, const double *sums, const float *gamma, const float *beta,
                       const float *conv_bias, float eps, float momentum, float *running_mean, float *running_var,
                       long long *num_batches_tracked, float *save_mean, float *save_invstd, float *h, int ldh, int relu,
                       void *stream);
int pn2x_bn_relu_bwd(long rows, int c, const float *dh, int ldd, const float *y, int ldy, const float *mean,
                     const float *invstd, const float *gamma, const float *beta, int relu, double *sums, float *dy, int ldo,
                     float *dgamma, float *dbeta, float *dbias, void *stream);
int pn2x_sa_layer1(int b, int n, int s, int k, int c1, const float *a1f, int a1f_ld, const float *xyz, const float *cxyz,
                   const float *wx, int wx_ld, const float *cadd, int cadd_ld, const int *idx, float *out, float *rel_out,
                   void *stream);
int pn2x_sa_layer1_stats(int b, int n, int s, int k, int c1, const float *a1f, int a1f_ld, const float *xyz, const float *cxyz,
                         const float *wx, int wx_ld, const float *cadd, int cadd_ld, const int *idx, float *out, float *rel_out,
                         double *sums, void *stream);
int pn2x_sa_layer1_stats_pair(int b, int n, int s, const float *xyz, const float *cxyz, int k_a, int c1_a, const float *a1f_a, int a1f_ld_a,
                              const float *wx_a, int wx_ld_a, const float *cadd_a, int cadd_ld_a, const int *idx_a, float *out_a,
                              float *rel_out_a, double *sums_a, int k_b, int c1_b, const float *a1f_b, int a1f_ld_b, const float *wx_b,
                              int wx_ld_b, const float *cadd_b, int cadd_ld_b, const int *idx_b, float *out_b, float *rel_out_b,
                              double *sums_b, void *stream);
int pn2x_scatter_add_rows(int b, int n, int m, int c, const float *dout, int ldo, const int *idx, float *din, int ldi,
                          void *stream);
int pn2x_three_interpolate_pm_grad(int b, int c, int m, int n, const float *dout, int ldo, const int *idx,
                                   const float *weight, float *dpoints, int ldp, void *stream);

int pn2x_inverse_index(int b, int n_dst, int l, const int *idx, int *offsets, int *order, void *stream);
int pn2x_rows_segment_sum(int b, int n_dst, int m_src, int t, int c, const float *dout, int ldo, const int *offsets,
                          const int *order, const float *weight, float *din, int ldi, int accumulate, void *stream);
int pn2x_rows_segment_sum_pair(int b, int n_dst, int m_a, int c_a, const float *dout_a, int ldo_a, const int *offsets_a, const int *order_a,
                               float *din_a, int ldi_a, int m_b, int c_b, const float *dout_b, int ldo_b, const int *offsets_b,
                               const int *order_b, float *din_b, int ldi_b, int accumulate, void *stream);

long pn2x_scatter_cm_scratch_ints(int t, int b, int n_dst, int m_src);
int pn2x_scatter_cm(int t, int b, int c, int n_dst, int m_src, const float *grad_out, const int *idx, const float *weight,
                    float *grad_points, int *scratch, long scratch_ints, void *stream);

int pn2x_bn_relu_max(long groups, int k, int c, const float *y, int ldy, const double *sums, const float *gamma, const float *beta,
                     const float *conv_bias, float eps, float momentum, float *running_mean, float *running_var,
                     long long *num_batches_tracked, float *save_mean, float *save_invstd, float *out, int *arg, void *stream);
int pn2x_bn_relu_max_ld(long groups, int k, int c, const float *y, int ldy, const double *sums, const float *gamma, const float *beta,
                        const float *conv_bias, float eps, float momentum, float *running_mean, float *running_var,
                        long long *num_batches_tracked, float *save_mean, float *save_invstd, float *out, int ldo, int *arg, void *stream);
int pn2x_bn_relu_max_pair(long groups_a, int k_a, int c_a, const float *y_a, int ldy_a, const double *sums_a, const float *gamma_a,
                          const float *beta_a, const float *conv_bias_a, float eps_a, float momentum_a, float *running_mean_a,
                          float *running_var_a, long long *nbt_a, float *save_mean_a, float *save_invstd_a, float *out_a, int ldo_a,
                          int *arg_a, long groups_b, int k_b, int c_b, const float *y_b, int ldy_b, const double *sums_b,
                          const float *gamma_b, const float *beta_b, const float *conv_bias_b, float eps_b, float momentum_b,
                          float *running_mean_b, float *running_var_b, long long *nbt_b, float *save_mean_b, float *save_invstd_b,
                          float *out_b, int ldo_b, int *arg_b, void *stream);
int pn2x_bn_relu_max_bwd(long groups, int k, int c, const float *dout, const int *arg, const float *y, int ldy, const float *mean,
                         const float *invstd, const float *gamma, const float *beta, double *sums, float *dy, int ldo, float *dgamma,
                         float *dbeta, float *dbias, void *stream);

int pn2x_bn_bwd_reduce(long rows, int c, const float *dh, int ldd, const int *arg, int k, const float *y, int ldy, const float *mean,
                       const float *invstd, const float *gamma, const float *beta, int relu, double *sums, float *g_out, int ldg,
                       void *stream);
int pn2x_bn_bwd_reduce_routed(long groups, int k, int c, const float *dout, int ldd, const int *arg, int lda, const float *y, int ldy,
                              const float *mean, const float *invstd, const float *gamma, const float *beta, double *sums, void *stream);
int pn2x_bn_bwd_reduce_routed_pair(long groups_a, int k_a, int c_a, const float *dout_a, int ldd_a, const int *arg_a, int lda_a,
                                   const float *y_a, int ldy_a, const float *mean_a, const float *invstd_a, const float *gamma_a,
                                   const float *beta_a, double *sums_a, long groups_b, int k_b, int c_b, const float *dout_b, int ldd_b,
                                   const int *arg_b, int lda_b, const float *y_b, int ldy_b, const float *mean_b, const float *invstd_b,
                                   const float *gamma_b, const float *beta_b, double *sums_b, void *stream);
long pn2x_rows_outer3_scratch_floats(long rows, int c);
int pn2x_rows_outer3(long rows, int c, const float *dy, int ldy, const float *rel, float *out, float *scratch, long scratch_floats,
                     void *stream);
int pn2x_bn_bwd_apply(long rows, int c, const float *g, int ldg, const float *y, int ldy, const float *mean, const float *invstd,
                      const float *gamma, const float *beta, int relu, const double *sums, float *dy, int ldo, float *dgamma,
                      float *dbeta, float *dbias, void *stream);

long pn2x_bn_bwd_apply_rel_scratch_floats(long rows, int c);
// ... 113 lines not shown
```

network/models/fast_eval.py:

```python
from __future__ import annotations

import torch
import torch.nn.functional as F



def _lin_relu(x2d: torch.Tensor, W: torch.Tensor, b: torch.Tensor) -> torch.Tensor:
    from hotrack_amd import ext
    return ext.linear(x2d, W, b, relu=True)


def _lin(x2d: torch.Tensor, W: torch.Tensor, b: torch.Tensor = None) -> torch.Tensor:
    from hotrack_amd import ext
    return ext.linear(x2d, W, b)


class FastEval:
    MAX_POINTS = 16384

    def __init__(self, net):
        self.net = net
        self._shapes_seen = set()
        self._key = None
        self.P = None
        self._consts = {}
        self._idents = {}
        self.row_chain = True

    def _palm_idx(self, device):
        key = ("palm", str(device))
        if key not in self._consts:
            self._consts[key] = torch.tensor([0, 1, 5, 9, 13, 17], dtype=torch.int32, device=device)
        return self._consts[key]

    def _scale(self, device):
        key = ("scale", str(device))
        if key not in self._consts:
            self._consts[key] = 0.2 * torch.ones(1, dtype=torch.float32, device=device)
        return self._consts[key]

    def _versions(self):
        return tuple((t._version, t.data_ptr(), t.device) for t in list(self.net.parameters()) + list(self.net.buffers()))

    @staticmethod
    def supported(net) -> bool:
        from hotrack_amd import ext
        bh = net.bhand
        if net.handframe != "kp" or not net.elide_dead_attention:
            return False

        def scales_ok(mod, n_scales):
            if len(mod.conv_blocks) != n_scales or len(mod.nsample_list) != n_scales:
                return False
            for convs, K in zip(mod.conv_blocks, mod.nsample_list):
                if len(convs) != 3 or not ext.sa_mlp_max_supported(int(K), *(int(c.weight.shape[0]) for c in convs)):
                    return False
            return True

        if not (scales_ok(bh.sa1, 1) and scales_ok(bh.sa2, 1) and scales_ok(net.q1, 2) and scales_ok(net.q2, 2)):
            return False
        if getattr(bh.sa1, "knn", False) or getattr(bh.sa2, "knn", False) or not (net.q1.knn and net.q2.knn):
            return False
        if bh.in_dim != 0 or not bh.sa3.group_all:
            return False
        if list(net.q1.nsample_list) != list(net.q2.nsample_list):
            return False
        w = [tuple(int(c.weight.shape[0]) for c in convs) for mod in (net.q1, net.q2) for convs in mod.conv_blocks]
        return len(set(w)) == 1

    def prepare(self, force: bool = False):
        key = self._versions()
        if not force and self._key == key:
            return self.P
        with torch.no_grad():
            ts = [t for t in list(self.net.parameters()) + list(self.net.buffers()) if t.is_floating_point()]
            self.finite_weights = bool(torch.stack([torch.isfinite(t).all() for t in ts]).all().item()) if ts else True
        if not self.finite_weights:
            self.P, self._key = None, key
            return None
        from hotrack_amd import gemm_tuning
        from hotrack_amd.fused import fold_conv_bn as fold
        gemm_tuning.enable()
        net, bh = self.net, self.net.bhand
        P = {}

        def msg(mod, i):
            return [fold(c, n) for c, n in zip(mod.conv_blocks[i], mod.bn_blocks[i])]

        (W1, b1), l2, l3 = msg(bh.sa1, 0)
        P["sa1"] = dict(wx=W1.contiguous(), b1=b1, l2=l2, l3=l3)
        (W1, b1), l2, l3 = msg(bh.sa2, 0)
        D = W1.shape[1] - 3
        P["sa2"] = dict(w1f=W1[:, :D].contiguous(), wx=W1[:, D:].contiguous(), b1=b1, l2=l2, l3=l3)
        sa3 = [fold(c, n) for c, n in zip(bh.sa3.mlp_convs, bh.sa3.mlp_bns)]
        W = sa3[0][0]
        sa3[0] = (torch.cat([W[:, 3:], W[:, :3]], dim=1).contiguous(), sa3[0][1])
        P["sa3"] = sa3
        fp3 = [fold(c, n) for c, n in zip(bh.fp3.mlp_convs, bh.fp3.mlp_bns)]
        c_l2 = bh.sa2.out_channel
        P["fp3"] = dict(wa=fp3[0][0][:, :c_l2].contiguous(), wb=fp3[0][0][:, c_l2:].contiguous(), b=fp3[0][1], rest=fp3[1:])
        P["fp2"] = [fold(c, n) for c, n in zip(bh.fp2.mlp_convs, bh.fp2.mlp_bns)]
        fp1 = [fold(c, n) for c, n in zip(bh.fp1.mlp_convs, bh.fp1.mlp_bns)]
        W = fp1[0][0]
        fp1[0] = (torch.cat([W[:, 3:], W[:, :3]], dim=1).contiguous(), fp1[0][1])
        P["fp1"] = fp1
        import os
        from hotrack_amd import ext
        P["fp1_fused"] = None
        c_in = fp1[0][0].shape[1] - 3
        if os.environ.get("HOTRACK_MLP2", "1") != "0" and len(fp1) == 2 and c_in == P["fp2"][-1][0].shape[0] and ext.mlp2_rows_supported(c_in, fp1[0][0].shape[0], fp1[1][0].shape[0]):
            P["fp1_fused"] = dict(w2=fp1[0][0][:, :c_in].contiguous(), w2e=fp1[0][0][:, c_in:].contiguous(), b2=fp1[0][1],
                                  w3=fp1[1][0].contiguous(), b3=fp1[1][1])
        P["conv1"] = fold(bh.conv1, bh.bn1)
        C = bh.out_dim
        wq, q = [], {}
        for name, mod in (("q1", net.q1), ("q2", net.q2)):
            for i in range(2):
                (W1, b1), l2, l3 = msg(mod, i)
                wq.append(W1[:, :C])
                q[(name, i)] = dict(wx=W1[:, C:C + 3].contiguous(), b1=b1, l2=l2, l3=l3, K=mod.nsample_list[i],
                                    wc=W1[:, C + 3:] if W1.shape[1] > C + 3 else None)
        P["q"] = q
        Ks = [q[("q1", i)]["K"] for i in range(2)]
        i_s = Ks.index(min(Ks))
        P["wq_order"] = (i_s, 1 - i_s)
        P["wq"] = torch.cat([torch.cat([wq[i], wq[2 + i]], dim=0) for i in P["wq_order"]], dim=0)
        P["row_chain"] = None
        Wc = P["conv1"][0]
        if (len(fp1) == 2 and c_in == P["fp2"][-1][0].shape[0] and Ks[0] != Ks[1] and fp1[0][0].shape[1] == c_in + 3
                and ext.row_chain_supported(c_in, fp1[0][0].shape[0], Wc.shape[0], 4 * wq[0].shape[0])
                and fp1[1][0].shape == (c_in, c_in) and Wc.shape[1] == c_in and C == Wc.shape[0]):
            P["row_chain"] = dict(wa=ext.row_chain_pack(fp1[0][0]), ba=fp1[0][1].contiguous(),
                                  wb=ext.row_chain_pack(fp1[1][0]), bb=fp1[1][1].contiguous(),
                                  wc=ext.row_chain_pack(Wc), bc=P["conv1"][1].contiguous(), wq=ext.row_chain_pack(P["wq"]))
        P["mid_chain"] = None
        S2 = bh.sa2.npoint
        pf = P["fp3"]
        if (len(sa3) == 3 and len(pf["rest"]) == 1 and sa3[0][0].shape[1] == c_l2 + 3
                and ext.sa3_chain_supported(S2, c_l2, sa3[0][0].shape[0], sa3[1][0].shape[0], sa3[2][0].shape[0])
                and sa3[1][0].shape[1] == sa3[0][0].shape[0] and sa3[2][0].shape[1] == sa3[1][0].shape[0]
                and ext.fp3_chain_supported(S2, pf["wa"].shape[1], pf["wb"].shape[1], pf["wa"].shape[0], pf["rest"][0][0].shape[0])
                and pf["wb"].shape[1] == sa3[2][0].shape[0] and pf["rest"][0][0].shape[1] == pf["wa"].shape[0]):
            P["mid_chain"] = dict(sa3=[t for W, b in sa3 for t in (ext.row_chain_pack(W), b.contiguous())],
                                  wgt=pf["wb"].t().contiguous(), bg=pf["b"].contiguous(), wa=ext.row_chain_pack(pf["wa"]),
                                  wf=ext.row_chain_pack(pf["rest"][0][0]), bf=pf["rest"][0][1].contiguous())
        P["wc2"] = torch.cat([q[("q2", 0)]["wc"], q[("q2", 1)]["wc"]], dim=0).contiguous()
        P["head_w"] = net.final_mlp[2].weight.detach().squeeze(-1).contiguous()
        P["r1"] = (net.r1.linear.weight.detach().squeeze(-1), net.r1.linear.bias.detach(), net.r1._perm.t().contiguous())
        P["r2"] = (net.r2.linear.weight.detach().squeeze(-1), net.r2.linear.bias.detach(), net.r2._perm.t().contiguous())
        self.P, self._key = P, key
        return P

    def _large_batch(self, B, N) -> bool:
        from hotrack_amd import ext
        return self.row_chain and B * N >= 32768 and B <= ext.ROW_CHAIN_MAX_B

    def _perm_idx(self, perm, B):
        key = ("perm", B, str(perm.device))
        if key not in self._idents:
            self._idents[key] = perm.reshape(1, -1).to(torch.int32).expand(B, -1).contiguous()
        return self._idents[key]

    @staticmethod
    def _q_scales(ext, name, plan, q, xyz1, c1q, a_col, cadd, out, c_q):
        probs = []
        for i, (idx, a, nb_xyz) in enumerate(plan):
            p = q[(name, i)]
            probs.append(dict(idx=idx, w2=p["l2"][0], b2=p["l2"][1], w3=p["l3"][0], b3=p["l3"][1], a1f=a[:, :, a_col:a_col + c1q],
                              xyz=nb_xyz, cxyz=xyz1, wx=p["wx"], b1=p["b1"],
                              cadd=None if cadd is None else cadd[:, :, i * c1q:(i + 1) * c1q], out=out[:, :, i * c_q:(i + 1) * c_q]))
        if len(probs) == 2:
            ext.sa_mlp_max_pair(*probs)
        else:
            for p in probs:
                ext.sa_mlp_max(p.pop("idx"), p.pop("w2"), p.pop("b2"), p.pop("w3"), p.pop("b3"), **p)

    def forward(self, input, flag_dict):
        from hotrack_amd import gemm_tuning
        shape = tuple(input["hand_points"].shape[:2])
        first = shape not in self._shapes_seen
        self._shapes_seen.add(shape)
        with gemm_tuning.scope(tune=first):
            return self._forward(input, flag_dict)

    def _forward(self, input, flag_dict):
        G = self._geometry(input, flag_dict)
        return None if G is None else self._dense(G, flag_dict)

    def _geometry(self, input, flag_dict):
        from hotrack_amd import ext
        net = self.net
        P = self.prepare()
        if P is None:
            return None
        dev = net.device
        if flag_dict["track_flag"]:
            palm = input["pred_palm_template"]
        else:
            palm = input["gt_hand_pose"]["palm_template"]
        palm = palm.to(dev).float()
        kp = input["jittered_hand_kp"].to(dev).float()
        pts = input["hand_points"].to(dev).float()
        B, N, _ = pts.shape
        J = kp.shape[1]
        f32 = dict(dtype=torch.float32, device=pts.device)

        if net.handframe != "kp":
            raise NotImplementedError("fast path covers handframe='kp' (HandTrackNet's configuration)")
        if kp.shape[1] != 21:
            raise NotImplementedError("fast path covers the 21-keypoint hand")
        palm_idx = self._palm_idx(pts.device)
        c_i = P["fp2"][-1][0].shape[0]
        fp1_in = torch.empty((B, N, c_i + 4), **f32)
        nonfinite = torch.empty(B, dtype=torch.int32, device=pts.device)
        R, t, xyz2, xyz1 = ext.hand_frame(palm.contiguous(), kp.contiguous(), palm_idx, pts.contiguous(), 0.2,
                                          xyz2_copy=fp1_in[:, :, c_i:c_i + 3], nonfinite=nonfinite)
        scale = self._scale(pts.device)
        canon = {"scale": scale, "rotation": R, "translation": t}
        tt = t.transpose(1, 2)

        bh = net.bhand
        p = P["sa1"]
        S1, K1 = bh.sa1.npoint, bh.sa1.nsample_list[0]
        qK = [P["q"][("q1", i)]["K"] for i in range(2)]
        knn_req = (xyz1, max(qK), min(qK) if min(qK) < max(qK) else 0)
        _, l1_xyz, i_l2, idx1, knn_lists = ext.fps_two_level(xyz2, S1, bh.sa2.npoint, query=(bh.sa1.radius_list[0], K1), knn=knn_req)
        return dict(P=P, pts=pts, B=B, N=N, J=J, c_i=c_i, fp1_in=fp1_in, nonfinite=nonfinite, R=R, t=t, xyz2=xyz2, xyz1=xyz1,
                    canon=canon, S1=S1, K1=K1, l1_xyz=l1_xyz, i_l2=i_l2, idx1=idx1, knn_lists=knn_lists)

    def _dense(self, G, flag_dict):
        from hotrack_amd import ext
        from hotrack_amd import pointnet2_utils as ops
        net, bh = self.net, self.net.bhand
        P, pts, B, N, J, c_i, fp1_in, nonfinite = G["P"], G["pts"], G["B"], G["N"], G["J"], G["c_i"], G["fp1_in"], G["nonfinite"]
        R, t, xyz2, xyz1, canon, S1, K1 = G["R"], G["t"], G["xyz2"], G["xyz1"], G["canon"], G["S1"], G["K1"]
        l1_xyz, i_l2, idx1, knn_lists = G["l1_xyz"], G["i_l2"], G["idx1"], G["knn_lists"]
        f32 = dict(dtype=torch.float32, device=pts.device)
        dev = net.device
        p = P["sa1"]
        c_l1 = p["l3"][0].shape[0]
        fp2_w = P["fp2"][0][0].shape[1]
        fp2_in = torch.empty((B, S1, fp2_w), **f32)
        l1_feat = fp2_in[:, :, :c_l1]
        ext.sa_mlp_max(idx1, *p["l2"], *p["l3"], xyz=xyz2, cxyz=l1_xyz, wx=p["wx"], b1=p["b1"], out=l1_feat)

        p = P["sa2"]
        S2, K2 = bh.sa2.npoint, bh.sa2.nsample_list[0]
        c_l2 = p["l3"][0].shape[0]
        sa3_in = torch.empty((B, S2, c_l2 + 4), **f32)
        idx2, l2_xyz = ext.ball_query_picks(bh.sa2.radius_list[0], K2, l1_xyz, i_l2, xyz_copy=sa3_in[:, :, c_l2:c_l2 + 3])
        a1f = _lin(l1_feat.reshape(B * S1, c_l1), p["w1f"]).view(B, S1, -1)
        l2_feat = sa3_in[:, :, :c_l2]
        ext.sa_mlp_max(idx2, *p["l2"], *p["l3"], a1f=a1f, xyz=l1_xyz, cxyz=l2_xyz, wx=p["wx"], b1=p["b1"], out=l2_feat)

        large = self._large_batch(B, N)
        mc = P["mid_chain"]
        if large and mc is not None:
            part = ext.sa3_chain(sa3_in, *mc["sa3"])
            l2_out = ext.fp3_chain(sa3_in, part, mc["wgt"], mc["bg"], mc["wa"], mc["wf"], mc["bf"])
        else:
            x = sa3_in.view(B * S2, c_l2 + 4)[:, :c_l2 + 3]
            for W, b in P["sa3"]:
                x = _lin_relu(x, W, b)
            l3 = ext.max_rows(x.view(B, S2, -1))

            p = P["fp3"]
            g = _lin(l3, p["wb"], p["b"])
            if B == 1:
                h = _lin_relu(sa3_in.view(S2, c_l2 + 4)[:, :c_l2], p["wa"], g.view(-1)).view(B, S2, -1)
            else:
                h = _lin(sa3_in.view(B * S2, c_l2 + 4)[:, :c_l2], p["wa"]).view(B, S2, -1)
                ext.bias_act_pm_(h, g, rows_per_bias=S2, relu=True)
            x = h.view(B * S2, -1)
            for W, b in p["rest"]:
                x = _lin_relu(x, W, b)
            l2_out = x.view(B, S2, -1)

        ext.three_nn_interpolate_pm(l1_xyz, l2_xyz, l2_out, fp2_in[:, :, c_l1:])
        x = fp2_in.view(B * S1, fp2_w)
        for W, b in P["fp2"]:
            x = _lin_relu(x, W, b)
        l1_out = x.view(B, S1, -1)

        assert c_i == l1_out.shape[2]
        ext.three_nn_interpolate_pm(xyz2, l1_xyz, l1_out, fp1_in[:, :, :c_i])
        q = P["q"]
        Ks = [q[("q1", i)]["K"] for i in range(2)]
        kmin, kmax = min(Ks), max(Ks)
        gi, gi_small = knn_lists
        c_q = q[("q1", 0)]["l3"][0].shape[0]
        c1q = q[("q1", 0)]["l2"][0].shape[1]
        rc = P["row_chain"]
        if large and rc is not None and gi_small is not None:
            lst, counts = ext.row_lists(gi, gi_small, N)
            a_all = torch.empty((B, N, 4 * c1q), **f32)
            ext.row_chain(fp1_in, lst, counts, rc["wa"], rc["ba"], rc["wb"], rc["bb"], rc["wc"], rc["bc"], rc["wq"], out=a_all)
        else:
            f = P["fp1_fused"]
            if f is not None:
                x = ext.mlp2_rows(fp1_in.view(B * N, c_i + 4), f["w2"], f["b2"], f["w3"], f["b3"], w2e=f["w2e"])
            else:
                x = fp1_in.view(B * N, c_i + 4)[:, :c_i + 3]
                for W, b in P["fp1"]:
                    x = _lin_relu(x, W, b)
            src2 = _lin_relu(x, *P["conv1"])
            a_all = _lin(src2, P["wq"]).view(B, N, -1)
        plan = []
        for i, K in enumerate(Ks):
            j = P["wq_order"].index(i)
            idx = gi if K == kmax else (gi_small if K == kmin and gi_small is not None else gi[:, :, :K].contiguous())
            plan.append((idx, a_all[:, :, 2 * c1q * j:2 * c1q * (j + 1)], xyz2))
        f11 = torch.empty((B, J, 2 * c_q), **f32)
        self._q_scales(ext, "q1", plan, q, xyz1, c1q, 0, None, f11, c_q)
        Wr, br, perm = P["r1"]
        f12 = _lin(ext.gather_rows(f11, self._perm_idx(perm, B)).view(B * J, -1), Wr, br)
        cadd = _lin(f12, P["wc2"]).view(B, J, -1)
        f13 = torch.empty((B, J, 2 * c_q), **f32)
        self._q_scales(ext, "q2", plan, q, xyz1, c1q, c1q, cadd, f13, c_q)
        Wr, br, perm = P["r2"]
        f14 = _lin(ext.gather_rows(f13, self._perm_idx(perm, B)).view(B * J, -1), Wr, br)

        s11, c11, c3 = net.transt.s11, net.transt.c11, net.c3
        wf, bf = net.final_mlp[0].weight.squeeze(-1), net.final_mlp[0].bias
        if ext.ln_linear_supported(f14.shape[0], f14.shape[1]):
            x, hdn = ext.ln_linear(f14, s11.norm1, c11.linear1.weight, c11.linear1.bias, relu=True, ln2=c11.norm1)
            y = _lin(hdn, c11.linear2.weight)
            x, hdn = ext.ln_linear(x, c11.norm2, c3.linear1.weight, c3.linear1.bias, relu=True, y=y, ybias=c11.linear2.bias, ln2=c3.norm1)
            y = _lin(hdn, c3.linear2.weight)
            x, hdn = ext.ln_linear(x, c3.norm2, wf, bf, relu=True, y=y, ybias=c3.linear2.bias)
        else:
            x = ext.add_layernorm(f14, s11.norm1, ln2=c11.norm1)
            for blk, nxt in ((c11, c3.norm1), (c3, None)):
                hdn = _lin_relu(x, blk.linear1.weight, blk.linear1.bias)
                x = ext.add_layernorm(x, blk.norm2, y=_lin(hdn, blk.linear2.weight), bias=blk.linear2.bias, ln2=nxt)
            hdn = _lin_relu(x, wf, bf)
        pred_hf, pred_kp = ext.pose_head(hdn, P["head_w"], net.final_mlp[2].bias, xyz1, R, t, 0.2, nonfinite=nonfinite)

        ret = {"canon_pose": canon}
        ret["pred_kp_handframe"] = pred_hf.transpose(1, 2)
        ret["init_kp_handframe"] = xyz1.transpose(1, 2)
        ret["points_handframe"] = xyz2.transpose(1, 2)
        ret["pred_kp"] = pred_kp
        if flag_dict.get("IKNet_flag", False):
            d4, _ = ops.knn(4, ret["pred_kp"].contiguous(), pts.contiguous())
            d4 = d4.mean(dim=-1)
            d4[:, 0] -= 0.01
            d4[:, 1] -= 0.01
            ret["pred_kp_vis_mask"] = (d4 < 0.02).bool()
        return ret
```

Baseline: 87980 frames/s.

## Group SA centroids by neighbour count so fused MLP skips duplicate padded rows

Ball query now optionally writes each centroid's distinct-neighbour count. A class-list kernel buckets centroids into classes of 32/16/8 effective rows. A new class-walk mode of the fused SA MLP+max kernel processes only those rows instead of always K padded neighbours, since padding duplicates the first hit and cannot change the max. This aims to cut MLP work for sparse neighbourhoods, at the cost of an extra list-building launch and more complex tile scheduling.

```diff
diff --git a/hotrack_amd/csrc/ball_query.hip b/hotrack_amd/csrc/ball_query.hip
--- a/hotrack_amd/csrc/ball_query.hip
+++ b/hotrack_amd/csrc/ball_query.hip
@@ -11,7 +11,8 @@
 __device__ __forceinline__ void ball_query_body(const int bx, const int by, int n, int m, float radius2, int nsample,
                                                 const float *__restrict__ new_xyz_all, const float *__restrict__ xyz_all,
                                                 int *__restrict__ idx_all, const int *__restrict__ picks_all,
-                                                float *__restrict__ new_xyz_out_all, float *__restrict__ new_xyz_copy, int copy_ld) {
+                                                float *__restrict__ new_xyz_out_all, float *__restrict__ new_xyz_copy, int copy_ld,
+                                                int *__restrict__ counts_all) {
     extern __shared__ __attribute__((aligned(16))) float smem[];
     const int tile_cap = n < kBqTile ? n : kBqTile;
     float *sx = smem, *sy = smem + tile_cap, *sz = smem + 2 * tile_cap;
@@ -125,6 +126,7 @@
         int *__restrict__ row = idx + (size_t)s * nsample;
         const int fill = cnt[c] > 0 ? first[c] : 0;
         for (int p = cnt[c] + lane; p < nsample; p += kWave) row[p] = fill;
+        if (counts_all && lane == 0) counts_all[(size_t)b * m + s] = cnt[c] < 1 ? 1 : (cnt[c] < nsample ? cnt[c] : nsample);
     }
 }
 
@@ -132,21 +134,22 @@
 __global__ void __launch_bounds__(kBqThreads)
 ball_query_kernel(int n, int m, float radius2, int nsample, const float *__restrict__ new_xyz_all,
                   const float *__restrict__ xyz_all, int *__restrict__ idx_all, const int *__restrict__ picks_all,
-                  float *__restrict__ new_xyz_out_all, float *__restrict__ new_xyz_copy, int copy_ld) {
+                  float *__restrict__ new_xyz_out_all, float *__restrict__ new_xyz_copy, int copy_ld, int *__restrict__ counts_all) {
     ball_query_body<CPW, JOINT>((int)blockIdx.x, (int)blockIdx.y, n, m, radius2, nsample, new_xyz_all, xyz_all, idx_all, picks_all,
-                                new_xyz_out_all, new_xyz_copy, copy_ld);
+                                new_xyz_out_all, new_xyz_copy, copy_ld, counts_all);
 }
 
 template <int CPW>
 __global__ void __launch_bounds__(kBqThreads)
 ball_tie_kernel(int nbx_ball, int nb_ball, int nbx_tie, int n, int m, float radius2, int nsample, const float *__restrict__ xyz_all,
                 int *__restrict__ idx_all, const int *__restrict__ picks_all, float *__restrict__ new_xyz_out_all,
-                float *__restrict__ new_xyz_copy, int copy_ld, int m2, const float *__restrict__ radii_all, int *__restrict__ flags) {
+                float *__restrict__ new_xyz_copy, int copy_ld, int m2, const float *__restrict__ radii_all, int *__restrict__ flags,
+                int *__restrict__ counts_all) {
     const int L = (int)blockIdx.x;
     if (L < nb_ball) {
         const int by = L / nbx_ball;
         ball_query_body<CPW, false>(L - by * nbx_ball, by, n, m, radius2, nsample, xyz_all, xyz_all, idx_all, picks_all, new_xyz_out_all,
-                                    new_xyz_copy, copy_ld);
+                                    new_xyz_copy, copy_ld, counts_all);
     } else {
         const int T = L - nb_ball, by = T / nbx_tie;
         fps_tie_body(T - by * nbx_tie, by, nbx_tie, n, m2, m, xyz_all, picks_all, radii_all, flags);
@@ -155,7 +158,7 @@
 
 int ball_query_dispatch(int b, int n, int m, float radius, int nsample, const float *new_xyz,
                         const float *xyz, int *idx, hipStream_t st, const int *picks, float *new_xyz_out, float *new_xyz_copy,
-                        int copy_ld) {
+                        int copy_ld, int *counts) {
     if (b == 0 || m == 0) return PN2_OK;
     const float radius2 = radius * radius;
     const int tile_cap = n < kBqTile ? n : kBqTile;
@@ -168,15 +171,15 @@
     dim3 grid((m + per_block - 1) / per_block, b);
     const bool joint = cpw >= 2 && n >= 4096;
     if (cpw == 4 && joint)
-        hipLaunchKernelGGL((ball_query_kernel<4, true>), grid, dim3(kBqThreads), lds, st, n, m, radius2, nsample, new_xyz, xyz, idx, picks, new_xyz_out, new_xyz_copy, copy_ld);
+        hipLaunchKernelGGL((ball_query_kernel<4, true>), grid, dim3(kBqThreads), lds, st, n, m, radius2, nsample, new_xyz, xyz, idx, picks, new_xyz_out, new_xyz_copy, copy_ld, counts);
     else if (cpw == 4)
-        hipLaunchKernelGGL((ball_query_kernel<4, false>), grid, dim3(kBqThreads), lds, st, n, m, radius2, nsample, new_xyz, xyz, idx, picks, new_xyz_out, new_xyz_copy, copy_ld);
+        hipLaunchKernelGGL((ball_query_kernel<4, false>), grid, dim3(kBqThreads), lds, st, n, m, radius2, nsample, new_xyz, xyz, idx, picks, new_xyz_out, new_xyz_copy, copy_ld, counts);
     else if (cpw == 2 && joint)
-        hipLaunchKernelGGL((ball_query_kernel<2, true>), grid, dim3(kBqThreads), lds, st, n, m, radius2, nsample, new_xyz, xyz, idx, picks, new_xyz_out, new_xyz_copy, copy_ld);
+        hipLaunchKernelGGL((ball_query_kernel<2, true>), grid, dim3(kBqThreads), lds, st, n, m, radius2, nsample, new_xyz, xyz, idx, picks, new_xyz_out, new_xyz_copy, copy_ld, counts);
     else if (cpw == 2)
-        hipLaunchKernelGGL((ball_query_kernel<2, false>), grid, dim3(kBqThreads), lds, st, n, m, radius2, nsample, new_xyz, xyz, idx, picks, new_xyz_out, new_xyz_copy, copy_ld);
+        hipLaunchKernelGGL((ball_query_kernel<2, false>), grid, dim3(kBqThreads), lds, st, n, m, radius2, nsample, new_xyz, xyz, idx, picks, new_xyz_out, new_xyz_copy, copy_ld, counts);
     else
-        hipLaunchKernelGGL((ball_query_kernel<1, false>), grid, dim3(kBqThreads), lds, st, n, m, radius2, nsample, new_xyz, xyz, idx, picks, new_xyz_out, new_xyz_copy, copy_ld);
+        hipLaunchKernelGGL((ball_query_kernel<1, false>), grid, dim3(kBqThreads), lds, st, n, m, radius2, nsample, new_xyz, xyz, idx, picks, new_xyz_out, new_xyz_copy, copy_ld, counts);
     return check_launch();
 }
 
@@ -187,7 +190,7 @@
 }
 
 int ball_tie_dispatch(int b, int n, int m, float radius, int nsample, const float *xyz, int *idx, const int *picks, float *new_xyz_out,
-                      float *new_xyz_copy, int copy_ld, int m2, const float *radii, int *flags, hipStream_t st) {
+                      float *new_xyz_copy, int copy_ld, int m2, const float *radii, int *flags, hipStream_t st, int *counts) {
     if (!ball_tie_supported(b, n, m, m2)) return PN2_ERANGE;
     const float radius2 = radius * radius;
     const int tile_cap = n < kBqTile ? n : kBqTile;
@@ -196,7 +199,7 @@
     const int nbx_ball = (m + per_block - 1) / per_block, nbx_tie = (n + kTiePts - 1) / kTiePts;
     const long grid = (long)b * nbx_ball + (long)b * nbx_tie;
     hipLaunchKernelGGL(ball_tie_kernel<1>, dim3((unsigned)grid), dim3(kBqThreads), lds, st, nbx_ball, b * nbx_ball, nbx_tie, n, m, radius2, nsample,
-                       xyz, idx, picks, new_xyz_out, new_xyz_copy, copy_ld, m2, radii, flags);
+                       xyz, idx, picks, new_xyz_out, new_xyz_copy, copy_ld, m2, radii, flags, counts);
     return check_launch();
 }
 
diff --git a/hotrack_amd/csrc/capi.hip b/hotrack_amd/csrc/capi.hip
--- a/hotrack_amd/csrc/capi.hip
+++ b/hotrack_amd/csrc/capi.hip
@@ -13,14 +13,14 @@
 bool fps_knn_supported(int n, int nq, int k);
 bool ball_tie_supported(long b, long n, long m, long m2);
 int ball_tie_dispatch(int b, int n, int m, float radius, int nsample, const float *xyz, int *idx, const int *picks, float *new_xyz_out,
-                      float *new_xyz_copy, int copy_ld, int m2, const float *radii, int *flags, hipStream_t st);
+                      float *new_xyz_copy, int copy_ld, int m2, const float *radii, int *flags, hipStream_t st, int *counts);
 bool three_nn_interp_supported(long b, long n, long m, long c, long ldp, long ldo);
 int three_nn_interp_dispatch(int b, int n, int m, int c, const float *unknown, const float *known, const float *points, int ldp,
                              float *out, int ldo, hipStream_t st);
 int fps_knn_dispatch(int b, int n, int m, const float *xyz, int *idx, float *radii, int nq, int k, int k2, const float *query,
                      int *kidx, int *kidx2, hipStream_t st);
 int ball_query_dispatch(int b, int n, int m, float radius, int nsample, const float *new_xyz, const float *xyz,
-                        int *idx, hipStream_t st, const int *picks, float *new_xyz_out, float *new_xyz_copy, int copy_ld);
+                        int *idx, hipStream_t st, const int *picks, float *new_xyz_out, float *new_xyz_copy, int copy_ld, int *counts);
 int three_nn_dispatch(int b, int n, int m, const float *unknown, const float *known, float *dist2, int *idx,
                       hipStream_t st, bool weights);
 int interp_pm_dispatch(int b, int c, int m, int n, const float *points, int ldp, const int *idx, const float *weight,
@@ -132,11 +132,16 @@
             }
         }
     }
-    return ball_query_dispatch(b, n, m, radius, nsample, new_xyz, xyz, idx, (hipStream_t)stream, nullptr, nullptr, nullptr, 0);
+    return ball_query_dispatch(b, n, m, radius, nsample, new_xyz, xyz, idx, (hipStream_t)stream, nullptr, nullptr, nullptr, 0, nullptr);
 }
 
 int pn2x_ball_query_picks(int b, int n, int m, float radius, int nsample, const float *xyz, const int *picks, float *new_xyz,
                            int *idx, float *new_xyz_copy, int copy_ld, void *stream) {
+    return pn2x_ball_query_picks_counts(b, n, m, radius, nsample, xyz, picks, new_xyz, idx, new_xyz_copy, copy_ld, nullptr, stream);
+}
+
+int pn2x_ball_query_picks_counts(int b, int n, int m, float radius, int nsample, const float *xyz, const int *picks, float *new_xyz,
+                                  int *idx, float *new_xyz_copy, int copy_ld, int *counts, void *stream) {
     PN2_REQ(!new_xyz_copy || copy_ld >= 3, PN2_EINVAL);
     PN2_REQ(b >= 0 && n >= 1 && m >= 0 && nsample >= 1, PN2_EINVAL);
     PN2_REQ(radius == radius, PN2_EINVAL);
@@ -144,20 +149,27 @@
     PN2_REQ(xyz && picks && new_xyz && idx, PN2_ENULL);
     PN2_REQ(b <= 65535, PN2_ERANGE);
     PN2_REQ(fits_int((long)n * 3) && fits_int((long)m * nsample), PN2_ERANGE);
-    return ball_query_dispatch(b, n, m, radius, nsample, nullptr, xyz, idx, (hipStream_t)stream, picks, new_xyz, new_xyz_copy, copy_ld);
+    return ball_query_dispatch(b, n, m, radius, nsample, nullptr, xyz, idx, (hipStream_t)stream, picks, new_xyz, new_xyz_copy, copy_ld, counts);
 }
 
 int pn2x_ball_query_picks_ties_supported(int b, int n, int m, int m2) { return ball_tie_supported(b, n, m, m2) ? 1 : 0; }
 
 int pn2x_ball_query_picks_ties(int b, int n, int m, float radius, int nsample, const float *xyz, const int *picks, float *new_xyz,
                                int *idx, float *new_xyz_copy, int copy_ld, int m2, const float *radii, int *flags, void *stream) {
+    return pn2x_ball_query_picks_ties_counts(b, n, m, radius, nsample, xyz, picks, new_xyz, idx, new_xyz_copy, copy_ld, m2, radii, flags,
+                                             nullptr, stream);
+}
+
+int pn2x_ball_query_picks_ties_counts(int b, int n, int m, float radius, int nsample, const float *xyz, const int *picks, float *new_xyz,
+                                      int *idx, float *new_xyz_copy, int copy_ld, int m2, const float *radii, int *flags, int *counts,
+                                      void *stream) {
     PN2_REQ(!new_xyz_copy || copy_ld >= 3, PN2_EINVAL);
     PN2_REQ(b >= 0 && n >= 1 && m >= 1 && nsample >= 1 && m2 >= 1 && m2 <= m, PN2_EINVAL);
     PN2_REQ(radius == radius, PN2_EINVAL);
     if (b == 0) return PN2_OK;
     PN2_REQ(xyz && picks && new_xyz && idx && radii && flags, PN2_ENULL);
     PN2_REQ(b <= 65535 && fits_int((long)n * 3) && fits_int((long)m * nsample), PN2_ERANGE);
-    return ball_tie_dispatch(b, n, m, radius, nsample, xyz, idx, picks, new_xyz, new_xyz_copy, copy_ld, m2, radii, flags, (hipStream_t)stream);
+    return ball_tie_dispatch(b, n, m, radius, nsample, xyz, idx, picks, new_xyz, new_xyz_copy, copy_ld, m2, radii, flags, (hipStream_t)stream, counts);
 }
 
 int pn2_group_points(int b, int c, int n, int npoints, int nsample, const float *points, const int *idx,
diff --git a/hotrack_amd/csrc/sa_fused.hip b/hotrack_amd/csrc/sa_fused.hip
--- a/hotrack_amd/csrc/sa_fused.hip
+++ b/hotrack_amd/csrc/sa_fused.hip
@@ -71,6 +71,12 @@
     f32x2 r;
     asm("v_pk_fma_f32 %0, %1, %2, %3 op_sel:[0,1,0]" : "=v"(r) : "v"(w), "v"(d), "v"(acc));
     return r;
+}
+
+__device__ __forceinline__ float rows_max2(float v) {
+    const unsigned u = __builtin_bit_cast(unsigned, v);
+    auto a = __builtin_amdgcn_permlane16_swap(u, u, false, false);
+    return fmax_raw(__builtin_bit_cast(float, (unsigned)a[0]), __builtin_bit_cast(float, (unsigned)a[1]));
 }
 
 struct SaArgs {
@@ -90,11 +96,14 @@
     int out_s, out_c;
     int num_tiles, tiles_per_cloud;
     long long *trace;
+    const int *cls_list;
+    const int *cls_sizes;
 };
 
 template <int C1, int C2, int C3, int WC, int RTC, int MINW, int NB1, int K, int MODE>
 __device__ __forceinline__ void sa_body(const SaArgs &A, const int wg, const int nwg) {
-    static_assert(K == 16 || K == 32 || K == 64, "K");
+    static_assert(K == 0 || K == 16 || K == 32 || K == 64, "K");
+    constexpr bool CLS = K == 0;
     constexpr bool ROWS = MODE == 4 || MODE == 5, ROWS_EXTRA = MODE == 5;
     static_assert(!ROWS_EXTRA || SA_PAD >= 4, "the extra input columns live in the LDS row padding");
     constexpr bool has_a1f = MODE >= 1, has_xyz = !ROWS, has_cadd = MODE == 2 || MODE == 3;
@@ -142,10 +151,39 @@
     static_assert((TM / 2) % (256 / Q1) == 0, "half tile rows split evenly over the loader threads");
     static_assert(RPT == 1 || RPT == 2 || RPT == 4, "a thread's neighbour indices are ONE 4/8/16-byte load");
     const int row0 = (lt / Q1) * RPT;
-    const int cur_db = nwg / tiles_per_cloud, cur_dt = nwg - cur_db * tiles_per_cloud;
+    int first = wg, step = nwg, end = num_tiles;
+    int cls_n0 = 0, cls_n1 = 0, cls_n2 = 0, cls_t0 = 0, cls_t1 = 0;
+    if constexpr (CLS) {
+        constexpr int lgTM = TM == 64 ? 6 : 7;
+        static_assert(TM == 64 || TM == 128, "class walk: tile of 64 or 128 positions");
+        cls_n0 = A.cls_sizes[0]; cls_n1 = A.cls_sizes[1]; cls_n2 = A.cls_sizes[2];
+        cls_t0 = (int)(((unsigned)cls_n0 * 32u + (TM - 1)) >> lgTM);
+        cls_t1 = (int)(((unsigned)cls_n1 * 16u + (TM - 1)) >> lgTM);
+        const unsigned total = (unsigned)cls_t0 + (unsigned)cls_t1 + (((unsigned)cls_n2 * 8u + (TM - 1)) >> lgTM);
+        const unsigned q = total / (unsigned)nwg, r = total - q * (unsigned)nwg;
+        first = (int)((unsigned)wg * q + ((unsigned)wg < r ? (unsigned)wg : r));
+        end = first + (int)q + ((unsigned)wg < r ? 1 : 0);
+        step = 1;
+    }
+    auto sel3 = [](int c, int v0, int v1, int v2) { return c == 0 ? v0 : c == 1 ? v1 : v2; };
+    const int cur_db = CLS ? 0 : nwg / tiles_per_cloud, cur_dt = CLS ? 0 : nwg - cur_db * tiles_per_cloud;
     struct Cursor { int tile, b, t; };
-    auto cursor_at = [&](int tile) { Cursor c; c.tile = tile; c.b = tile / tiles_per_cloud; c.t = tile - c.b * tiles_per_cloud; return c; };
+    auto cursor_at = [&](int tile) {
+        Cursor c;
+        c.tile = tile;
+        if constexpr (CLS) {
+            c.b = 0; c.t = tile;
+            if (c.t >= cls_t0) {
+                c.t -= cls_t0; c.b = 1;
+                if (c.t >= cls_t1) { c.t -= cls_t1; c.b = 2; }
+            }
+        } else {
+            c.b = tile / tiles_per_cloud; c.t = tile - c.b * tiles_per_cloud;
+        }
+        return c;
+    };
     auto cursor_next = [&](Cursor c) {
+        if constexpr (CLS) return cursor_at(c.tile + 1);
         c.tile += nwg; c.b += cur_db; c.t += cur_dt;
         if (c.t >= tiles_per_cloud) { c.t -= tiles_per_cloud; ++c.b; }
         return c;
@@ -156,7 +194,8 @@
     const unsigned cxyz_cloud = 12u * (unsigned)S, cadd_cloud = (unsigned)S * cadd_ldb;
     const rsrc_t ra_all = make_rsrc(A.a1f, p_a1f ? (unsigned)A.B * a1f_cloud : 0u);
     const rsrc_t rx_all = make_rsrc(A.xyz, p_xyz ? (unsigned)A.B * xyz_cloud : 0u);
-    struct HalfIdx { int jj[RPT], ss; };
+    struct HalfIdx { int jj[RPT], ss, bn; };
+    struct HalfCid { int cid, bn; };
     struct HalfRows { float4 a[RPT], pj[RPT], c, cs, e; };
     auto load_idx = [&](const Cursor &cu, int h, HalfIdx &I) {
         const int b = cu.b < A.B ? cu.b : A.B - 1;
@@ -179,7 +218,49 @@
         }
         I.ss = (pos0 + row0) >> lgK;
     };
+    const rsrc_t ri_all = make_rsrc(A.idx, CLS ? 128u * (unsigned)A.B * (unsigned)S : 0u);
+    auto load_cid = [&](const Cursor &cu, int h, HalfCid &C) {
+        const int lgk = 5 - cu.b;
+        const int n_c = sel3(cu.b, cls_n0, cls_n1, cls_n2), off = sel3(cu.b, 0, cls_n0, cls_n0 + cls_n1);
+        const rsrc_t rl = make_rsrc(A.cls_list + 4 * (size_t)off, 16u * (unsigned)n_c);
+        const unsigned slot = (unsigned)(cu.t * TM + h * (TM / 2) + row0) >> lgk;
+        const i32x2 v = __builtin_bit_cast(i32x2, __builtin_amdgcn_raw_buffer_load_b64(rl, (int)(16u * slot), 0, 0));
+        C.cid = v.x; C.bn = v.y;
+    };
+    auto load_idx_cls = [&](const Cursor &cu, int h, const HalfCid &C, HalfIdx &I) {
+        const int lgk = 5 - cu.b;
+        const unsigned k0 = (unsigned)(cu.t * TM + h * (TM / 2) + row0) & ((1u << lgk) - 1u);
+        const unsigned voff = mad24(C.cid, 128u, 4u * k0);
+        if constexpr (RPT == 4) {
+            const i32x4 v = __builtin_bit_cast(i32x4, __builtin_amdgcn_raw_buffer_load_b128(ri_all, (int)voff, 0, 0));
+            I.jj[0] = v.x; I.jj[1] = v.y; I.jj[2] = v.z; I.jj[3] = v.w;
+        } else if constexpr (RPT == 2) {
+            const i32x2 v = __builtin_bit_cast(i32x2, __builtin_amdgcn_raw_buffer_load_b64(ri_all, (int)voff, 0, 0));
+            I.jj[0] = v.x; I.jj[1] = v.y;
+        } else {
+            I.jj[0] = (int)__builtin_amdgcn_raw_buffer_load_b32(ri_all, (int)voff, 0, 0);
+        }
+        I.ss = C.cid;
+        I.bn = C.bn;
+    };
     auto load_rows = [&](const Cursor &cu, const HalfIdx &I, HalfRows &D) {
+        if constexpr (CLS) {
+            if (has_a1f) {
+#pragma unroll
+                for (int r = 0; r < RPT; ++r) D.a[r] = ld_b128(ra_all, mad24(I.jj[r] + I.bn, a1f_ldb, c4x16), 0);
+            }
+            if (has_cadd) {
+                const rsrc_t rd = make_rsrc(A.cadd, p_cadd ? (unsigned)A.B * cadd_cloud : 0u);
+                D.c = ld_b128(rd, mad24(I.ss, cadd_ldb, c4x16), 0);
+            }
+            if (has_xyz) {
+                const rsrc_t rc = make_rsrc(A.cxyz, p_xyz ? (unsigned)A.B * cxyz_cloud : 0u);
+#pragma unroll
+                for (int r = 0; r < RPT; ++r) D.pj[r] = ld_b128(rx_all, mul24(I.jj[r] + I.bn, 12u), 0);
+                D.cs = ld_b128(rc, mul24(I.ss, 12u), 0);
+            }
+            return;
+        }
         const int b = cu.b < A.B ? cu.b : A.B - 1;
         if (has_a1f) {
             const int so = ROWS ? 0 : (int)((unsigned)b * a1f_cloud);
@@ -251,7 +332,13 @@
     auto gather = [&](const Cursor &cu, float *__restrict__ H1, int h) {
         HalfIdx I;
         HalfRows D;
-        load_idx(cu, h, I);
+        if constexpr (CLS) {
+            HalfCid C;
+            load_cid(cu, h, C);
+            load_idx_cls(cu, h, C, I);
+        } else {
+            load_idx(cu, h, I);
+        }
         load_rows(cu, I, D);
         finish(D, H1, h);
     };
@@ -298,9 +385,9 @@
             }
         }
     } else {
-        Cursor cu = cursor_at(wg);
+        Cursor cu = cursor_at(first);
         for (int a = 0; a < NB1 - 1; ++a, cu = cursor_next(cu)) {
-            if (cu.tile < num_tiles) {
+            if (cu.tile < end) {
                 gather(cu, H1ring + a * TM * LD1, 0);
                 gather(cu, H1ring + a * TM * LD1, 1);
             }
@@ -320,13 +407,24 @@
         __builtin_amdgcn_s_setprio(SA_LOADER_PRIO);
         HalfIdx I0, I1;
         HalfRows D0, D1;
-        Cursor nx = cursor_at(wg + (NB1 - 1) * nwg);
+        Cursor nx = cursor_at(first + (NB1 - 1) * step);
         Cursor af = cursor_next(nx);
-        load_idx(nx, 0, I0);
-        load_idx(nx, 1, I1);
+        Cursor ag = cursor_next(af);
+        HalfCid G0, G1;
+        if constexpr (CLS) {
+            load_cid(nx, 0, G0);
+            load_cid(nx, 1, G1);
+            load_idx_cls(nx, 0, G0, I0);
+            load_idx_cls(nx, 1, G1, I1);
+            load_cid(af, 0, G0);
+            load_cid(af, 1, G1);
+        } else {
+            load_idx(nx, 0, I0);
+            load_idx(nx, 1, I1);
+        }
         load_rows(nx, I0, D0);
         int it = 0;
-        for (int tile = wg; tile < num_tiles; tile += nwg, ++it) {
+        for (int tile = first; tile < end; tile += step, ++it) {
             stamp(it, 0);
             float *H1n = H1ring + ((it + NB1 - 1) % NB1) * TM * LD1;
 #if !(SA_PROBE & 1)
@@ -334,11 +432,16 @@
 #endif
             stamp(it, 7);
 #if !(SA_PROBE & 4)
-            load_idx(af, 0, I0);
+            if constexpr (CLS) {
+                load_idx_cls(af, 0, G0, I0);
+                load_cid(ag, 0, G0);
+            } else {
+                load_idx(af, 0, I0);
+            }
 #endif
             stamp(it, 1);
 #if !(SA_PROBE & 2)
-            if (nx.tile < num_tiles) finish(D0, H1n, 0);
+            if (nx.tile < end) finish(D0, H1n, 0);
 #endif
             stamp(it, 2);
             __syncthreads();
@@ -347,17 +450,23 @@
             load_rows(af, I0, D0);
 #endif
 #if !(SA_PROBE & 4)
-            load_idx(af, 1, I1);
+            if constexpr (CLS) {
+                load_idx_cls(af, 1, G1, I1);
+                load_cid(ag, 1, G1);
+            } else {
+                load_idx(af, 1, I1);
+            }
 #endif
             stamp(it, 4);
 #if !(SA_PROBE & 2)
-            if (nx.tile < num_tiles) finish(D1, H1n, 1);
+            if (nx.tile < end) finish(D1, H1n, 1);
 #endif
             stamp(it, 5);
             __syncthreads();
             stamp(it, 6);
             nx = af;
-            af = cursor_next(af);
+            af = CLS ? ag : cursor_next(af);
+            if constexpr (CLS) ag = cursor_next(ag);
         }
         return;
     }
@@ -365,9 +474,9 @@
     __builtin_amdgcn_s_setprio(SA_COMPUTE_PRIO);
 #endif
     int it = 0;
-    Cursor cc = cursor_at(wg);
+    Cursor cc = cursor_at(first);
     constexpr int NP = 4 / RTC, NQ2 = C1 / 16, NQ3 = C2 / 16;
-    constexpr int rstep = K >> 4;
+    constexpr int rstep = CLS ? 4 : K >> 4;
     const int oc_lane = (wc * NT3 + g) * 16 + li;
     const unsigned out_cloud = 4u * ((unsigned)(S - 1) * (unsigned)A.out_s + (unsigned)(C3 - 1) * (unsigned)A.out_c + 1u);
     const rsrc_t ro_rows = make_rsrc(out, ROWS ? 4u * (unsigned)N * (unsigned)A.out_s : 0u);
@@ -409,6 +518,48 @@
             }
         }
     };
+    int me_b = 0, me_s = 0;
+    auto load_me = [&](const Cursor &cu) {
+        const int lgk = 5 - cu.b;
+        const int n_c = sel3(cu.b, cls_n0, cls_n1, cls_n2), off = sel3(cu.b, 0, cls_n0, cls_n0 + cls_n1);
+        const rsrc_t rl = make_rsrc(A.cls_list + 4 * (size_t)off, 16u * (unsigned)n_c);
+        const unsigned slot = ((unsigned)(cu.t * TM + wp * 64) >> lgk) + (unsigned)(lane & 7);
+        const i32x2 v = __builtin_bit_cast(i32x2, __builtin_amdgcn_raw_buffer_load_b64(rl, (int)(16u * slot + 8u), 0, 0));
+        me_b = v.x; me_s = v.y;
+    };
+    const unsigned out_all = 4u * ((unsigned)(A.B - 1) * (unsigned)A.out_b + (unsigned)(S - 1) * (unsigned)A.out_s + (unsigned)(C3 - 1) * (unsigned)A.out_c + 1u);
+    auto epilogue_cls = [&](const Cursor &cu) {
+        static_assert(!CLS || NT3 == 2, "class walk: a lane row stores one of two channel tiles");
+        const int lgk = 5 - cu.b;
+        const int n_c = sel3(cu.b, cls_n0, cls_n1, cls_n2);
+        const int slot0 = (int)((unsigned)(cu.t * TM + wp * 64) >> lgk);
+        const rsrc_t ro = make_rsrc(out, out_all);
+        auto store = [&](float v, int src, int ct, bool lane_ok) {
+            const unsigned bb = (unsigned)__builtin_amdgcn_ds_bpermute(4 * src, me_b), ss = (unsigned)__builtin_amdgcn_ds_bpermute(4 * src, me_s);
+            const unsigned off = 4u * (bb * (unsigned)A.out_b + ss * (unsigned)A.out_s + (unsigned)((wc * NT3 + ct) * 16 + li) * (unsigned)A.out_c);
+            const bool ok = lane_ok && slot0 + src < n_c;
+            __builtin_amdgcn_raw_buffer_store_b32(__builtin_bit_cast(unsigned, fmaxf(v, 0.f)), ro, (int)(ok ? off : 0xffffffffu), 0, 0);
+        };
+        if (lgk == 5) {
+#pragma unroll
+            for (int rt = 0; rt < 4; rt += 2) {
+                const float v0 = rows_max4(fmax_raw(m[rt][0], m[rt + 1][0])), v1 = rows_max4(fmax_raw(m[rt][NT3 - 1], m[rt + 1][NT3 - 1]));
+                store(g == 1 ? v1 : v0, rt >> 1, g & 1, g < 2);
+            }
+        } else if (lgk == 4) {
+#pragma unroll
+            for (int rt = 0; rt < 4; ++rt) {
+                const float v0 = rows_max4(m[rt][0]), v1 = rows_max4(m[rt][NT3 - 1]);
+                store(g == 1 ? v1 : v0, rt, g & 1, g < 2);
+            }
+        } else {
+#pragma unroll
+            for (int rt = 0; rt < 4; ++rt) {
+                const float v0 = rows_max2(m[rt][0]), v1 = rows_max2(m[rt][NT3 - 1]);
+                store((g & 1) ? v1 : v0, 2 * rt + (g >> 1), g & 1, true);
+            }
+        }
+    };
     auto frag2 = [&](const float *H1, int p, int tq, int rt) {
         return *reinterpret_cast<const float4 *>(H1 + (wp * 64 + (p * RTC + rt) * 16 + li) * LD1 + 4 * g + 16 * tq);
     };
@@ -416,7 +567,7 @@
     float4 an2[RTC];
 #pragma unroll
     for (int rt = 0; rt < RTC; ++rt) an2[rt] = frag2(H1ring, 0, 0, rt);
-    for (int tile = wg; tile < num_tiles; tile += nwg, ++it, cc = cursor_next(cc)) {
+    for (int tile = first; tile < end; tile += step, ++it, cc = cursor_next(cc)) {
         stamp(it, 0);
         const float *H1 = H1ring + (it % NB1) * TM * LD1;
         const float *H1next = H1ring + ((it + 1) % NB1) * TM * LD1;
@@ -469,7 +620,7 @@
                                 acc[p & 1][rt][ct] = __builtin_amdgcn_mfma_f32_16x16x4f32(w2r[ct][4 * tq + j], av, acc[p & 1][rt][ct], 0, 0, 0);
                         }
 #if SA_DEFER_EPILOGUE
-                    if (!ROWS && tq == 0 && p == 0) epilogue();
+                    if (!ROWS && !CLS && tq == 0 && p == 0) epilogue();
 #endif
 #if SA_OVERLAP_WRITEOUT
                     if (tq == 0 && p > 0) writeout2(p - 1);
@@ -487,6 +638,7 @@
         stamp(it, 2);
         __syncthreads();
         stamp(it, 3);
+        if constexpr (CLS) load_me(cc);
         {
             auto frag3 = [&](int p, int tq, int rt) {
                 return *reinterpret_cast<const float4 *>(H2 + (wp * 64 + (p * RTC + rt) * 16 + li) * LD2 + 4 * g + 16 * tq);
@@ -547,7 +699,9 @@
                 }
             }
             stamp(it, 4);
-            if constexpr (!ROWS) {
+            if constexpr (CLS) {
+                epilogue_cls(cc);
+            } else if constexpr (!ROWS) {
                 e_b = cc.b;
                 e_pos0 = cc.t * TM;
                 e_pending = true;
@@ -561,7 +715,7 @@
         stamp(it, 6);
     }
 #if SA_DEFER_EPILOGUE
-    if (!ROWS) epilogue();
+    if (!ROWS && !CLS) epilogue();
 #endif
 }
 
@@ -569,6 +723,12 @@
 __global__ void __launch_bounds__(512, MINW)
 sa_mlp_max_kernel(const SaArgs A, const int grid) {
     sa_body<C1, C2, C3, WC, RTC, MINW, NB1, K, MODE>(A, (int)__builtin_amdgcn_workgroup_id_x(), grid);
+}
+
+template <int C1, int C2, int C3, int WC, int RTC, int MINW, int NB1, int MODE>
+__global__ void __launch_bounds__(512, MINW)
+sa_mlp_max_classes_kernel(const SaArgs A, const int grid) {
+    sa_body<C1, C2, C3, WC, RTC, MINW, NB1, 0, MODE>(A, (int)__builtin_amdgcn_workgroup_id_x(), grid);
 }
 
 template <int C1, int C2, int C3, int WC, int RTC, int MINW, int NB1, int K0, int K1, int MODE>
@@ -615,6 +775,23 @@
     return check_launch();
 }
 
+template <int C1, int C2, int C3, int WC, int RTC, int MINW, int NB1, int MODE>
+static int launch_sa_classes(int b, SaArgs a, hipStream_t st) {
+    constexpr int WP = 4 / WC, TM = WP * 64;
+    a.B = b; a.K = 32; a.lgK = 5; a.tiles_per_cloud = 1; a.num_tiles = 0;
+    const size_t lds = (size_t)TM * (NB1 * (C1 + SA_PAD) + C2 + SA_PAD) * sizeof(float);
+    auto kfn = sa_mlp_max_classes_kernel<C1, C2, C3, WC, RTC, MINW, NB1, MODE>;
+    static PerDeviceOnce raised;
+    if (lds > 64 * 1024 && raised.first_use())
+        (void)hipFuncSetAttribute((const void *)kfn, hipFuncAttributeMaxDynamicSharedMemorySize, (int)lds);
+    const int wg_per_cu = (int)((160 * 1024) / lds) < MINW / 2 ? (int)((160 * 1024) / lds) : MINW / 2;
+    const long max_wg = (long)sa_compute_units() * (wg_per_cu < 1 ? 1 : wg_per_cu);
+    const long most = ((long)b * a.S * 32 + TM - 1) / TM + 2;
+    const int grid = (int)(most < max_wg ? most : max_wg);
+    hipLaunchKernelGGL(kfn, dim3(grid), dim3(512), lds, st, a, grid);
+    return check_launch();
+}
+
 template <int C1, int C2, int C3, int WC, int RTC, int MINW, int NB1>
 static void sa_tiles(int b, SaArgs &a) {
     constexpr int WP = 4 / WC, TM = WP * 64;
@@ -682,6 +859,94 @@
     return n < (1L << 24) && s < (1L << 24) && 4 * a1f_ld < (1L << 24) && 4 * cadd_ld < (1L << 24) &&
            4 * b * n * (a1f_ld > 3 ? a1f_ld : 3) <= lim && 4 * s * (cadd_ld > 3 ? cadd_ld : 3) <= lim && 4 * s * k <= lim;
 }
+
+constexpr int kClsThreads = 1024;
+__global__ __launch_bounds__(kClsThreads) void sa_class_lists_kernel(int M, int S, int N, const int *__restrict__ counts,
+                                                                      int *__restrict__ list, int *__restrict__ sizes) {
+    __shared__ int scan[3][kClsThreads];
+    const int tid = (int)threadIdx.x;
+    const int per = (M + kClsThreads - 1) / kClsThreads;
+    const long lo = (long)tid * per;
+    const int i0 = (int)(lo < M ? lo : M), i1 = i0 + per < M ? i0 + per : M;
+    int c0 = 0, c1 = 0, c2 = 0;
+    for (int i = i0; i < i1; ++i) {
+        const int k = counts[i];
+        c0 += k > 16 ? 1 : 0;
+        c1 += (k > 8 && k <= 16) ? 1 : 0;
+        c2 += k <= 8 ? 1 : 0;
+    }
+    int s0 = c0, s1 = c1, s2 = c2;
+    for (int d = 1; d < kClsThreads; d <<= 1) {
+        scan[0][tid] = s0; scan[1][tid] = s1; scan[2][tid] = s2;
+        __syncthreads();
+        if (tid >= d) { s0 += scan[0][tid - d]; s1 += scan[1][tid - d]; s2 += scan[2][tid - d]; }
+        __syncthreads();
+    }
+    scan[0][tid] = s0; scan[1][tid] = s1; scan[2][tid] = s2;
+    __syncthreads();
+    const int t0 = scan[0][kClsThreads - 1], t1 = scan[1][kClsThreads - 1], t2 = scan[2][kClsThreads - 1];
+    int p0 = s0 - c0, p1 = t0 + s1 - c1, p2 = t0 + t1 + s2 - c2;
+    int b = i0 / S, s = i0 - b * S;
+    int4 *__restrict__ dst = reinterpret_cast<int4 *>(list);
+    for (int i = i0; i < i1; ++i) {
+        const int k = counts[i];
+        const int4 rec = make_int4(i, b * N, b, s);
+        if (k > 16) dst[p0++] = rec;
+        else if (k > 8) dst[p1++] = rec;
+        else dst[p2++] = rec;
+        if (++s == S) { s = 0; ++b; }
+    }
+    if (tid == 0) { sizes[0] = t0; sizes[1] = t1; sizes[2] = t2; }
+}
+}
+
+extern "C" int pn2x_sa_class_lists(int b, int s, int n, const int *counts, int *list, int *sizes, void *stream) {
+    using namespace pn2;
+    if (b < 0 || s < 1 || n < 1) return PN2_EINVAL;
+    if ((long)b * s >= (1L << 24) || (long)b * n >= (1L << 24)) return PN2_ERANGE;
+    if (!sizes) return PN2_ENULL;
+    if (b > 0 && (!counts || !list)) return PN2_ENULL;
+    if ((uintptr_t)list % 16 != 0) return PN2_EINVAL;
+    hipLaunchKernelGGL(sa_class_lists_kernel, dim3(1), dim3(kClsThreads), 0, (hipStream_t)stream, b * s, s, n, counts, list, sizes);
+    return check_launch();
+}
+
+extern "C" int pn2x_sa_mlp_max_classes_supported(int k, int c1, int c2, int c3) {
+    return (k == 32 && ((c1 == 32 && c2 == 32 && c3 == 64) || (c1 == 64 && c2 == 64 && c3 == 128))) ? 1 : 0;
+}
+
+extern "C" int pn2x_sa_mlp_max_classes(int b, int n, int s, int k, int c1, int c2, int c3, const float *a1f, int a1f_ld,
+                                       const float *xyz, const float *cxyz, const float *wx, const float *b1, const float *cadd,
+                                       int cadd_ld, const int *idx, const int *cls_list, const int *cls_sizes,
+                                       const float *w2, const float *b2, const float *w3, const float *b3, float *out,
+                                       long out_b, int out_s, int out_c, void *stream) {
+    using namespace pn2;
+    if (b < 0 || n < 1 || s < 0 || k < 1) return PN2_EINVAL;
+    if (b == 0 || s == 0) return PN2_OK;
+    if (!idx || !cls_list || !cls_sizes || !w2 || !b2 || !w3 || !b3 || !out) return PN2_ENULL;
+    if (!a1f && !xyz) return PN2_ENULL;
+    if (xyz && (!cxyz || !wx)) return PN2_ENULL;
+    if ((a1f && (a1f_ld < c1 || a1f_ld % 4)) || (cadd && (cadd_ld < c1 || cadd_ld % 4))) return PN2_EINVAL;
+    if (!pn2x_sa_mlp_max_classes_supported(k, c1, c2, c3)) return PN2_ERANGE;
+    if (!sa_ranges_ok(b, n, s, k, a1f ? a1f_ld : 0, cadd ? cadd_ld : 0, c3, out_s, out_c)) return PN2_ERANGE;
+    const long lim = 0xffffffffL;
+    if (out_b < 0 || (long)b * n >= (1L << 24) || (long)b * s >= (1L << 24) || 128L * b * s > lim ||
+        4L * b * s * (cadd && cadd_ld > 3 ? cadd_ld : 3) > lim || 4 * ((b - 1) * out_b + (s - 1L) * out_s + (c3 - 1L) * out_c + 1) >= lim)
+        return PN2_ERANGE;
+    if (((uintptr_t)a1f | (uintptr_t)cadd | (uintptr_t)b1 | (uintptr_t)w2 | (uintptr_t)w3 | (uintptr_t)cls_list) % 16 != 0) return PN2_EINVAL;
+    SaArgs a;
+    a.B = b; a.N = n; a.S = s; a.K = k; a.lgK = 5;
+    a.a1f = a1f; a.a1f_ld = a1f_ld; a.cadd_ld = cadd_ld; a.xyz = xyz; a.cxyz = cxyz; a.wx = wx; a.b1 = b1; a.cadd = cadd; a.idx = idx;
+    a.w2 = w2; a.b2 = b2; a.w3 = w3; a.b3 = b3; a.w2e = nullptr; a.out = out; a.out_b = out_b; a.out_s = out_s; a.out_c = out_c;
+    a.num_tiles = 0; a.tiles_per_cloud = 1; a.trace = nullptr; a.cls_list = cls_list; a.cls_sizes = cls_sizes;
+    hipStream_t st = (hipStream_t)stream;
+    const bool fa = a1f != nullptr, fx = xyz != nullptr, fc = cadd != nullptr;
+    if (c1 == 32) {
+        if (!fa && fx && !fc) return launch_sa_classes<32, 32, 64, 2, 4, 4, SA_NB1, 0>(b, a, st);
+        return launch_sa_classes<32, 32, 64, 2, 4, 4, SA_NB1, 3>(b, a, st);
+    }
+    if (fa && fx && !fc) return launch_sa_classes<64, 64, 128, 4, 2, 4, SA_NB1, 1>(b, a, st);
+    return launch_sa_classes<64, 64, 128, 4, 2, 4, SA_NB1, 3>(b, a, st);
 }
 
 extern "C" int pn2x_sa_set_compute_units(int n) {
@@ -711,7 +976,7 @@
     a.B = b; a.N = n; a.S = s; a.K = k; a.lgK = 0;
     a.a1f = a1f; a.a1f_ld = a1f_ld; a.cadd_ld = cadd_ld; a.xyz = xyz; a.cxyz = cxyz; a.wx = wx; a.b1 = b1; a.cadd = cadd; a.idx = idx;
     a.w2 = w2; a.b2 = b2; a.w3 = w3; a.b3 = b3; a.w2e = nullptr; a.out = out; a.out_b = out_b; a.out_s = out_s; a.out_c = out_c;
-    a.num_tiles = 0; a.tiles_per_cloud = 0; a.trace = g_sa_trace;
+    a.num_tiles = 0; a.tiles_per_cloud = 0; a.trace = g_sa_trace; a.cls_list = nullptr; a.cls_sizes = nullptr;
     hipStream_t st = (hipStream_t)stream;
     if (c1 == 32 && c2 == 32 && c3 == 64) return launch_sa<32, 32, 64, 2, 4, 4, SA_NB1>(b, a, st);
     if (c1 == 64 && c2 == 64 && c3 == 128) return launch_sa<64, 64, 128, 4, 2, 4, SA_NB1>(b, a, st);
@@ -731,7 +996,7 @@
     a.B = 0; a.N = p.n; a.S = p.s; a.K = p.k; a.lgK = 0;
     a.a1f = p.a1f; a.a1f_ld = p.a1f_ld; a.cadd_ld = p.cadd_ld; a.xyz = p.xyz; a.cxyz = p.cxyz; a.wx = p.wx; a.b1 = p.b1;
     a.cadd = p.cadd; a.idx = p.idx; a.w2 = p.w2; a.b2 = p.b2; a.w3 = p.w3; a.b3 = p.b3; a.w2e = nullptr; a.out = p.out; a.out_b = p.out_b;
-    a.out_s = p.out_s; a.out_c = p.out_c; a.num_tiles = 0; a.tiles_per_cloud = 0; a.trace = nullptr;
+    a.out_s = p.out_s; a.out_c = p.out_c; a.num_tiles = 0; a.tiles_per_cloud = 0; a.trace = nullptr; a.cls_list = nullptr; a.cls_sizes = nullptr;
     return PN2_OK;
 }
 }
@@ -773,7 +1038,7 @@
     a.B = 1; a.N = (int)rows; a.K = 16; a.S = (int)((rows + 15) / 16); a.lgK = 4;
     a.a1f = x; a.a1f_ld = ldx; a.cadd_ld = 0; a.xyz = nullptr; a.cxyz = nullptr; a.wx = nullptr; a.b1 = nullptr; a.cadd = nullptr; a.idx = nullptr;
     a.w2 = w2; a.b2 = b2; a.w3 = w3; a.b3 = b3; a.w2e = w2e; a.out = out; a.out_b = 0; a.out_s = ldo; a.out_c = 1;
-    a.num_tiles = 0; a.tiles_per_cloud = 0; a.trace = nullptr;
+    a.num_tiles = 0; a.tiles_per_cloud = 0; a.trace = nullptr; a.cls_list = nullptr; a.cls_sizes = nullptr;
     if (w2e) return launch_sa_km<128, 128, 128, 4, 2, 2, SA_NB1, 16, 5>(1, a, (hipStream_t)stream);
     return launch_sa_km<128, 128, 128, 4, 2, 2, SA_NB1, 16, 4>(1, a, (hipStream_t)stream);
 }
diff --git a/hotrack_amd/ext.py b/hotrack_amd/ext.py
--- a/hotrack_amd/ext.py
+++ b/hotrack_amd/ext.py
@@ -96,6 +96,51 @@
 
 def sa_mlp_max(idx: torch.Tensor, w2, b2, w3, b3, *, a1f=None, xyz=None, cxyz=None, wx=None, b1=None, cadd=None,
                out=None, point_major=False) -> torch.Tensor:
+    return _sa_mlp_max(idx, w2, b2, w3, b3, None, a1f, xyz, cxyz, wx, b1, cadd, out, point_major)
+
+
+_lib.pn2x_sa_mlp_max_classes.argtypes = [_ci] * 7 + [_vp, _ci, _vp, _vp, _vp, _vp, _vp, _ci, _vp, _vp, _vp, _vp, _vp, _vp, _vp, _vp, _cl, _ci, _ci, _vp]
+_lib.pn2x_sa_mlp_max_classes.restype = _ci
+_lib.pn2x_sa_mlp_max_classes_supported.argtypes = [_ci] * 4
+_lib.pn2x_sa_mlp_max_classes_supported.restype = _ci
+_lib.pn2x_sa_class_lists.argtypes = [_ci, _ci, _ci, _vp, _vp, _vp, _vp]
+_lib.pn2x_sa_class_lists.restype = _ci
+
+
+def sa_mlp_max_classes_supported(k: int, c1: int, c2: int, c3: int) -> bool:
+    return bool(_lib.pn2x_sa_mlp_max_classes_supported(k, c1, c2, c3))
+
+
+def sa_class_partition(counts: torch.Tensor):
+    c = counts.reshape(-1)
+    ids = torch.arange(c.numel(), dtype=torch.int32, device=c.device)
+    masks = (c > 16, (c > 8) & (c <= 16), c <= 8)
+    return torch.cat([ids[m] for m in masks]), torch.stack([m.sum() for m in masks]).to(torch.int32)
+
+
+def sa_class_lists(counts: torch.Tensor, n: int):
+    if not isinstance(counts, torch.Tensor) or counts.dim() != 2 or counts.dtype != torch.int32 or not counts.is_cuda:
+        raise TypeError("sa_class_lists: counts must be a (B,S) int32 GPU tensor")
+    if int(n) < 1:
+        raise ValueError("sa_class_lists: n >= 1")
+    B, S = counts.shape
+    pc = _native._ptr(counts, "counts", torch.int32, B * S)
+    lst = torch.empty((B * S, 4), dtype=torch.int32, device=counts.device)
+    sizes = torch.empty(3, dtype=torch.int32, device=counts.device)
+    with torch.cuda.device(counts.device):
+        _native._check(_native._call(_lib.pn2x_sa_class_lists, "sa_class_lists_kernel", None, B, S, int(n), pc, lst.data_ptr(),
+                                     sizes.data_ptr(), _native._stream(counts)), "sa_class_lists")
+    return lst, sizes
+
+
+def sa_mlp_max_classes(idx: torch.Tensor, classes, w2, b2, w3, b3, *, a1f=None, xyz=None, cxyz=None, wx=None, b1=None, cadd=None,
+                       out=None, point_major=False) -> torch.Tensor:
+    if not (isinstance(classes, (tuple, list)) and len(classes) == 2):
+        raise TypeError("sa_mlp_max_classes: classes must be the (list, sizes) pair of sa_class_lists")
+    return _sa_mlp_max(idx, w2, b2, w3, b3, classes, a1f, xyz, cxyz, wx, b1, cadd, out, point_major)
+
+
+def _sa_mlp_max(idx, w2, b2, w3, b3, classes, a1f, xyz, cxyz, wx, b1, cadd, out, point_major):
     B, S, K = idx.shape
     C1, C2, C3 = w2.shape[1], w2.shape[0], w3.shape[0]
     f32 = torch.float32
@@ -116,6 +161,17 @@
     else:
         po, ld = _rows(out, "out", C3)
         ob, os_, oc = out.stride(0), ld, 1
+    if classes is not None:
+        lst, sizes = classes
+        pl = _native._ptr(lst, "classes list", torch.int32, B * S * 4)
+        ps = _native._ptr(sizes, "classes sizes", torch.int32, 3)
+        if lst.device != idx.device or sizes.device != idx.device:
+            raise ValueError("sa_mlp_max_classes: classes on another device than idx")
+        with torch.cuda.device(idx.device):
+            _native._check(_native._call(_lib.pn2x_sa_mlp_max_classes, "sa_mlp_max_classes_kernel", None, B, N, S, K, C1, C2, C3, pa, lda,
+                                         px, pcx, pwx, pb1, pc, ldc, pi, pl, ps, pw2, pb2, pw3, pb3, po, ob, os_, oc,
+                                         _native._stream(idx)), "sa_mlp_max_classes")
+        return out
     with torch.cuda.device(idx.device):
         _native._check(_native._call(_lib.pn2x_sa_mlp_max, "sa_mlp_max_kernel", None, B, N, S, K, C1, C2, C3, pa, lda, px, pcx,
                                      pwx, pb1, pc, ldc, pi, pw2, pb2, pw3, pb3, po, ob, os_, oc, _native._stream(idx)),
@@ -472,9 +528,12 @@
 
 _lib.pn2x_ball_query_picks.argtypes = [_ci, _ci, _ci, ctypes.c_float, _ci, _vp, _vp, _vp, _vp, _vp, _ci, _vp]
 _lib.pn2x_ball_query_picks.restype = _ci
-
-
-def ball_query_picks(radius: float, nsample: int, xyz: torch.Tensor, picks: torch.Tensor, xyz_copy: torch.Tensor = None):
+_lib.pn2x_ball_query_picks_counts.argtypes = [_ci, _ci, _ci, ctypes.c_float, _ci, _vp, _vp, _vp, _vp, _vp, _ci, _vp, _vp]
+_lib.pn2x_ball_query_picks_counts.restype = _ci
+
+
+def ball_query_picks(radius: float, nsample: int, xyz: torch.Tensor, picks: torch.Tensor, xyz_copy: torch.Tensor = None,
+                     counts: bool = False):
     B, N, _ = xyz.shape
     S = picks.shape[1]
     px = _native._ptr(xyz, "xyz", torch.float32, B * N * 3)
@@ -483,6 +542,11 @@
     new_xyz = torch.empty((B, S, 3), dtype=torch.float32, device=xyz.device)
     pc, ldc = (None, 0) if xyz_copy is None else _xyz_cols(xyz_copy, "xyz_copy", B, S)
     with torch.cuda.device(xyz.device):
+        if counts:
+            cnt = torch.empty((B, S), dtype=torch.int32, device=xyz.device)
+            _native._check(_lib.pn2x_ball_query_picks_counts(B, N, S, float(radius), nsample, px, pp, new_xyz.data_ptr(), idx.data_ptr(),
+                                                              pc, ldc, cnt.data_ptr(), _native._stream(xyz)), "ball_query_picks")
+            return idx, new_xyz, cnt
         _native._check(_lib.pn2x_ball_query_picks(B, N, S, float(radius), nsample, px, pp, new_xyz.data_ptr(), idx.data_ptr(),
                                                    pc, ldc, _native._stream(xyz)), "ball_query_picks")
     return idx, new_xyz
@@ -492,11 +556,13 @@
 BALL_TIE_COLAUNCH = True
 _lib.pn2x_ball_query_picks_ties.argtypes = [_ci, _ci, _ci, ctypes.c_float, _ci, _vp, _vp, _vp, _vp, _vp, _ci, _ci, _vp, _vp, _vp]
 _lib.pn2x_ball_query_picks_ties.restype = _ci
+_lib.pn2x_ball_query_picks_ties_counts.argtypes = [_ci, _ci, _ci, ctypes.c_float, _ci, _vp, _vp, _vp, _vp, _vp, _ci, _ci, _vp, _vp, _vp, _vp]
+_lib.pn2x_ball_query_picks_ties_counts.restype = _ci
 _lib.pn2x_ball_query_picks_ties_supported.argtypes = [_ci] * 4
 _lib.pn2x_ball_query_picks_ties_supported.restype = _ci
 
 
-def fps_two_level(xyz: torch.Tensor, m1: int, m2: int, query=None, knn=None):
+def fps_two_level(xyz: torch.Tensor, m1: int, m2: int, query=None, knn=None, query_counts: bool = False):
     from . import pointnet2_utils as ops
     B, N, _ = xyz.shape
     if not 1 <= m2 <= m1:
@@ -510,6 +576,8 @@
         i1 = ops.furthest_point_sample(xyz, m1)
         l1 = gather_rows(xyz, i1)
         i2 = ops.furthest_point_sample(l1, m2)
+        if query is not None and query_counts:
+            raise ValueError("fps_two_level: query_counts needs m2 <= 1024 and N <= 16384")
         res = (i1, l1, i2) if query is None else (i1, l1, i2, ops.ball_query(query[0], query[1], xyz, l1))
         return res if knn is None else res + (knn_alone(),)
     px = _native._ptr(xyz, "xyz", torch.float32, B * N * 3)
@@ -518,6 +586,9 @@
     radii = torch.empty((B, m1), dtype=torch.float32, device=xyz.device)
     flags = torch.empty((B, nf), dtype=torch.int32, device=xyz.device)
     i2 = torch.empty((B, m2), dtype=torch.int32, device=xyz.device)
+    if query_counts and query is None:
+        raise ValueError("fps_two_level: query_counts without query")
+    cnt1 = torch.empty((B, m1), dtype=torch.int32, device=xyz.device) if query_counts else None
     with torch.cuda.device(xyz.device):
         st = _native._stream(xyz)
         lists = None
@@ -536,18 +607,27 @@
         if query is not None and BALL_TIE_COLAUNCH and _lib.pn2x_ball_query_picks_ties_supported(B, N, m1, m2):
             idx1 = torch.empty((B, m1, query[1]), dtype=torch.int32, device=xyz.device)
             l1 = torch.empty((B, m1, 3), dtype=torch.float32, device=xyz.device)
-            _native._check(_native._call(_lib.pn2x_ball_query_picks_ties, "ball_tie_kernel", None, B, N, m1, float(query[0]), query[1], px,
-                                         i1.data_ptr(), l1.data_ptr(), idx1.data_ptr(), None, 0, m2, radii.data_ptr(), flags.data_ptr(), st),
-                           "fps_two_level/query+ties")
+            if query_counts:
+                _native._check(_native._call(_lib.pn2x_ball_query_picks_ties_counts, "ball_tie_kernel", None, B, N, m1, float(query[0]), query[1],
+                                             px, i1.data_ptr(), l1.data_ptr(), idx1.data_ptr(), None, 0, m2, radii.data_ptr(),
+                                             flags.data_ptr(), cnt1.data_ptr(), st), "fps_two_level/query+ties")
+            else:
+                _native._check(_native._call(_lib.pn2x_ball_query_picks_ties, "ball_tie_kernel", None, B, N, m1, float(query[0]), query[1], px,
+                                             i1.data_ptr(), l1.data_ptr(), idx1.data_ptr(), None, 0, m2, radii.data_ptr(), flags.data_ptr(), st),
+                               "fps_two_level/query+ties")
         else:
             if query is None:
                 l1 = gather_rows(xyz, i1)
+            elif query_counts:
+                idx1, l1, cnt1 = ball_query_picks(query[0], query[1], xyz, i1, counts=True)
             else:
                 idx1, l1 = ball_query_picks(query[0], query[1], xyz, i1)
             _native._check(_lib.pn2x_fps_prefix_ties(B, N, m1, m2, px, i1.data_ptr(), radii.data_ptr(), flags.data_ptr(), st), "fps_two_level/ties")
         _native._check(_native._call(_lib.pn2x_furthest_point_sampling_prefix, "fps_prefix_kernel", None, B, m1, m2, l1.data_ptr(),
                                      flags.data_ptr(), nf, i2.data_ptr(), st), "fps_two_level/2")
     res = (i1, l1, i2) if query is None else (i1, l1, i2, idx1)
+    if query_counts:
+        res = res + (cnt1,)
     if knn is None:
         return res
     return res + (lists if lists is not None else knn_alone(),)
diff --git a/include/pn2_ext.h b/include/pn2_ext.h
--- a/include/pn2_ext.h
+++ b/include/pn2_ext.h
@@ -21,6 +21,14 @@
                     const float *w2, const float *b2, const float *w3, const float *b3, float *out,
                     long out_b, int out_s, int out_c, void *stream);
 int pn2x_sa_mlp_max_supported(int k, int c1, int c2, int c3);
+
+int pn2x_sa_class_lists(int b, int s, int n, const int *counts, int *list, int *sizes, void *stream);
+int pn2x_sa_mlp_max_classes_supported(int k, int c1, int c2, int c3);
+int pn2x_sa_mlp_max_classes(int b, int n, int s, int k, int c1, int c2, int c3, const float *a1f, int a1f_ld,
+                            const float *xyz, const float *cxyz, const float *wx, const float *b1, const float *cadd,
+                            int cadd_ld, const int *idx, const int *cls_list, const int *cls_sizes,
+                            const float *w2, const float *b2, const float *w3, const float *b3, float *out,
+                            long out_b, int out_s, int out_c, void *stream);
 
 int pn2x_bias_act(int b, int c, int n, float *y, const float *bias, int relu, void *stream);
 
@@ -48,6 +56,11 @@
 
 int pn2x_ball_query_picks(int b, int n, int m, float radius, int nsample, const float *xyz, const int *picks, float *new_xyz,
                           int *idx, float *new_xyz_copy, int copy_ld, void *stream);
+int pn2x_ball_query_picks_counts(int b, int n, int m, float radius, int nsample, const float *xyz, const int *picks, float *new_xyz,
+                                 int *idx, float *new_xyz_copy, int copy_ld, int *counts, void *stream);
+int pn2x_ball_query_picks_ties_counts(int b, int n, int m, float radius, int nsample, const float *xyz, const int *picks, float *new_xyz,
+                                      int *idx, float *new_xyz_copy, int copy_ld, int m2, const float *radii, int *flags, int *counts,
+                                      void *stream);
 
 long pn2x_ball_query_grid_scratch_words(int b, int n);
 int pn2x_ball_query_grid(int b, int n, int m, float radius, int nsample, const float *new_xyz, const float *xyz, int *idx,
diff --git a/network/models/fast_eval.py b/network/models/fast_eval.py
--- a/network/models/fast_eval.py
+++ b/network/models/fast_eval.py
@@ -26,6 +26,7 @@
         self._consts = {}
         self._idents = {}
         self.row_chain = True
+        self.sa_classes = True
 
     def _palm_idx(self, device):
         key = ("palm", str(device))
@@ -224,8 +225,16 @@
         S1, K1 = bh.sa1.npoint, bh.sa1.nsample_list[0]
         qK = [P["q"][("q1", i)]["K"] for i in range(2)]
         knn_req = (xyz1, max(qK), min(qK) if min(qK) < max(qK) else 0)
-        _, l1_xyz, i_l2, idx1, knn_lists = ext.fps_two_level(xyz2, S1, bh.sa2.npoint, query=(bh.sa1.radius_list[0], K1), knn=knn_req)
-        return dict(P=P, pts=pts, B=B, N=N, J=J, c_i=c_i, fp1_in=fp1_in, nonfinite=nonfinite, R=R, t=t, xyz2=xyz2, xyz1=xyz1,
+        classes = self.sa_classes and self._large_batch(B, N) and all(
+            ext.sa_mlp_max_classes_supported(int(m.nsample_list[0]), *(int(c.weight.shape[0]) for c in m.conv_blocks[0]))
+            for m in (bh.sa1, bh.sa2))
+        cnt1 = None
+        if classes:
+            _, l1_xyz, i_l2, idx1, cnt1, knn_lists = ext.fps_two_level(xyz2, S1, bh.sa2.npoint, query=(bh.sa1.radius_list[0], K1),
+                                                                       knn=knn_req, query_counts=True)
+        else:
+            _, l1_xyz, i_l2, idx1, knn_lists = ext.fps_two_level(xyz2, S1, bh.sa2.npoint, query=(bh.sa1.radius_list[0], K1), knn=knn_req)
+        return dict(cnt1=cnt1, P=P, pts=pts, B=B, N=N, J=J, c_i=c_i, fp1_in=fp1_in, nonfinite=nonfinite, R=R, t=t, xyz2=xyz2, xyz1=xyz1,
                     canon=canon, S1=S1, K1=K1, l1_xyz=l1_xyz, i_l2=i_l2, idx1=idx1, knn_lists=knn_lists)
 
     def _dense(self, G, flag_dict):
@@ -242,16 +251,28 @@
         fp2_w = P["fp2"][0][0].shape[1]
         fp2_in = torch.empty((B, S1, fp2_w), **f32)
         l1_feat = fp2_in[:, :, :c_l1]
-        ext.sa_mlp_max(idx1, *p["l2"], *p["l3"], xyz=xyz2, cxyz=l1_xyz, wx=p["wx"], b1=p["b1"], out=l1_feat)
+        cnt1 = G["cnt1"]
+        if cnt1 is not None:
+            ext.sa_mlp_max_classes(idx1, ext.sa_class_lists(cnt1, N), *p["l2"], *p["l3"], xyz=xyz2, cxyz=l1_xyz, wx=p["wx"], b1=p["b1"],
+                                   out=l1_feat)
+        else:
+            ext.sa_mlp_max(idx1, *p["l2"], *p["l3"], xyz=xyz2, cxyz=l1_xyz, wx=p["wx"], b1=p["b1"], out=l1_feat)
 
         p = P["sa2"]
         S2, K2 = bh.sa2.npoint, bh.sa2.nsample_list[0]
         c_l2 = p["l3"][0].shape[0]
         sa3_in = torch.empty((B, S2, c_l2 + 4), **f32)
-        idx2, l2_xyz = ext.ball_query_picks(bh.sa2.radius_list[0], K2, l1_xyz, i_l2, xyz_copy=sa3_in[:, :, c_l2:c_l2 + 3])
+        if cnt1 is not None:
+            idx2, l2_xyz, cnt2 = ext.ball_query_picks(bh.sa2.radius_list[0], K2, l1_xyz, i_l2, xyz_copy=sa3_in[:, :, c_l2:c_l2 + 3], counts=True)
+        else:
+            idx2, l2_xyz = ext.ball_query_picks(bh.sa2.radius_list[0], K2, l1_xyz, i_l2, xyz_copy=sa3_in[:, :, c_l2:c_l2 + 3])
         a1f = _lin(l1_feat.reshape(B * S1, c_l1), p["w1f"]).view(B, S1, -1)
         l2_feat = sa3_in[:, :, :c_l2]
-        ext.sa_mlp_max(idx2, *p["l2"], *p["l3"], a1f=a1f, xyz=l1_xyz, cxyz=l2_xyz, wx=p["wx"], b1=p["b1"], out=l2_feat)
+        if cnt1 is not None:
+            ext.sa_mlp_max_classes(idx2, ext.sa_class_lists(cnt2, S1), *p["l2"], *p["l3"], a1f=a1f, xyz=l1_xyz, cxyz=l2_xyz, wx=p["wx"],
+                                   b1=p["b1"], out=l2_feat)
+        else:
+            ext.sa_mlp_max(idx2, *p["l2"], *p["l3"], a1f=a1f, xyz=l1_xyz, cxyz=l2_xyz, wx=p["wx"], b1=p["b1"], out=l2_feat)
 
         large = self._large_batch(B, N)
         mc = P["mid_chain"]
```

After: 90900 frames/s (median of 6 runs). 3.3% higher.
